# z430/keyword-spotting

Hardware: AMD Instinct MI355X
Metric: 1s 16kHz clips/sec end-to-end (wav->label) (higher is better)
Workload: dtype f32

## Files before the change

### include/kws_hip.h

```cpp
#ifndef KWS_HIP_H
#define KWS_HIP_H

#include <stddef.h>
#include <stdint.h>

#ifdef __cplusplus
extern "C" {
#endif

typedef struct kws_ctx kws_ctx;

enum {
    KWS_OK = 0,
    KWS_EINVAL = -1,
    KWS_ENOMEM = -2,
    KWS_EHIP = -3,
    KWS_ESTATE = -4,
    KWS_EUNSUPPORTED = -5
};

#define KWS_ABI_VERSION 1
int kws_abi_version(void);


int kws_create(kws_ctx** out, int device_id);
void kws_destroy(kws_ctx* ctx);

int kws_set_stream(kws_ctx* ctx, void* hip_stream, int external);

int kws_sync(kws_ctx* ctx);

const char* kws_last_error(kws_ctx* ctx);


int kws_set_frontend(kws_ctx* ctx, int sample_rate, int n_samples, int frame_len, int frame_step,
                     int nfft, int nfilt, int numcep, float preemph, int ceplifter);

#define KWS_FE_F32 0
#define KWS_FE_F64 1
int kws_set_frontend_math(kws_ctx* ctx, int math);
int kws_frontend_math(kws_ctx* ctx);

#define KWS_FE_REFINE_SPAN_DEFAULT 10.2f
int kws_set_frontend_refine(kws_ctx* ctx, float log_ratio);
int kws_frontend_stats(kws_ctx* ctx, uint64_t* frames_total, uint64_t* frames_refined, int* last_call_refined);

int kws_frontend_shape(kws_ctx* ctx, int* num_frames, int* numcep);

int kws_mfcc_i16(kws_ctx* ctx, const int16_t* d_wav, int B, float* d_out);

int kws_mfcc_f32(kws_ctx* ctx, const float* d_wav, int B, float* d_out);


int kws_load_dscnn(kws_ctx* ctx, const float* blob, size_t n_floats, int num_classes);
int kws_load_dscnn_ex(kws_ctx* ctx, const float* blob, size_t n_floats, int num_classes, int input_channels);
int kws_load_dscnn_device(kws_ctx* ctx, const float* d_blob, size_t n_floats, int num_classes, int input_channels);
int kws_dscnn_image_read(kws_ctx* ctx, uint32_t* out_words, size_t cap_words, size_t* need_words, float* scalars);

int kws_forward_f32(kws_ctx* ctx, const float* d_feat, int B, float* d_logits, int32_t* d_label);

int kws_forward_map_f32(kws_ctx* ctx, const float* d_feat, int B, int T, int F, float* d_logits, int32_t* d_label);
int kws_forward_map_debug_f32(kws_ctx* ctx, const float* d_feat, int B, int T, int F, float* d_logits, int32_t* d_label,
                              float* d_layers);


int kws_dscnn_backward_f32(kws_ctx* ctx, const float* d_feat, int B, int T, int F, const float* d_dlogits, float* d_grad);

int kws_cnn_trad_backward_f32(kws_ctx* ctx, const float* d_feat, int B, const float* d_dlogits, float* d_grad);

int kws_cnn_trad_train_debug_f32(kws_ctx* ctx, const float* d_feat, int B, float* d_conv1, int32_t* d_winner, float* d_conv2,
                                 float* d_hidden);

int kws_dsblock_forward_f32(kws_ctx* ctx, const float* d_x, int B, int C_in, int H, int W, const float* d_dw_w,
                            const float* d_dw_b, const float* d_pw_w, const float* d_pw_b, int C_out, int kernel_size,
                            int stride, int padding, float* d_out);

int kws_infer_i16(kws_ctx* ctx, const int16_t* d_wav, int B, float* d_logits, int32_t* d_label);

int kws_infer_f32(kws_ctx* ctx, const float* d_wav, int B, float* d_logits, int32_t* d_label);

int kws_infer_host_i16(kws_ctx* ctx, const int16_t* h_wav, int B, float* h_logits, int32_t* h_label);
int kws_infer_host_submit_i16(kws_ctx* ctx, const int16_t* h_wav, int B, float* h_logits, int32_t* h_label, uint64_t* ticket);
int kws_infer_host_wait(kws_ctx* ctx, uint64_t ticket);
int kws_ingest_config(kws_ctx* ctx, int chunk_clips, int n_slots, int pack_threads);

int kws_reserve(kws_ctx* ctx, int max_batch);

#define KWS_PW_F32 1
#define KWS_PW_SPLIT_BF16 4
#define KWS_PW_PAIR_F16 5
int kws_set_pointwise_math(kws_ctx* ctx, int math);

#define KWS_ACT_FLOATS_PER_CLIP (64 * (141 + 141 + 245 + 357) + 64 + 64 * 477)
int kws_forward_debug_f32(kws_ctx* ctx, const float* d_feat, int B, float* d_logits, int32_t* d_label,
                          float* d_act, int use_mfma);


int kws_stream_open(kws_ctx* ctx, int n_streams);
int kws_stream_close(kws_ctx* ctx);
int kws_stream_push_i16(kws_ctx* ctx, const int16_t* d_hop, float* d_logits, int32_t* d_label, int use_graph);
int kws_stream_cluster(kws_ctx* ctx, int workgroups_per_stream);
int kws_stream_host_results(kws_ctx* ctx, int enable);
int kws_stream_wait_host(kws_ctx* ctx, const float** h_logits, const int32_t** h_label);
int kws_stream_push_host_i16(kws_ctx* ctx, const int16_t* h_hop, const float** h_logits, const int32_t** h_label);
int kws_stream_state(kws_ctx* ctx, const float** d_feat_ring, int* hops);
int kws_stream_copy_features(kws_ctx* ctx, float* d_out);

int kws_stream_vad_f32(kws_ctx* ctx, float log_energy_threshold, int on_window, int off_window, int32_t* d_state);

int kws_load_cnn_trad(kws_ctx* ctx, const float* blob, size_t n_floats, int num_classes);
int kws_load_cnn_trad_device(kws_ctx* ctx, const float* d_blob, size_t n_floats, int num_classes);
int kws_forward_cnn_trad_f32(kws_ctx* ctx, const float* d_feat, int B, float* d_logits, int32_t* d_label);
#define KWS_CT_F16_PAIR 0
#define KWS_CT_BF16_TRIPLE 1
int kws_set_cnn_trad_math(kws_ctx* ctx, int math);
int kws_forward_cnn_trad_debug_f32(kws_ctx* ctx, const float* d_feat, int B, float* d_logits, int32_t* d_label, float* d_conv2,
                                   float* d_clip_scale);

int kws_infer_cnn_trad_i16(kws_ctx* ctx, const int16_t* d_wav, int B, float* d_logits, int32_t* d_label);


int kws_softmax_f32(kws_ctx* ctx, const float* d_logits, int B, int C, float* d_prob);

int kws_stream_smooth_f32(kws_ctx* ctx, const float* d_logits, int C, int window, float* d_smoothed, int32_t* d_label);


int kws_scan_i16(kws_ctx* ctx, const int16_t* d_pcm, int R, int n_total, int hop_frames, float* d_logits, int32_t* d_label,
                 float* d_feat_out);

int kws_scan_detect_f32(kws_ctx* ctx, const float* d_logits, int R, int W, int C, int smooth_window, int first_keyword,
                        float threshold, int refractory, float* d_smoothed, int32_t* d_event_window, int32_t* d_event_label,
                        float* d_event_score, int max_events, int32_t* d_event_count);


int kws_frames_i16(kws_ctx* ctx, const int16_t* d_pcm, int R, int n_total, float* d_feat_out);

int kws_segment_f32(kws_ctx* ctx, const float* d_feat, int R, int F_total, int n_total, float log_energy_threshold, int on_window,
                    int off_window, int pre_roll, int max_frames, int32_t* d_utt, int max_utts, int32_t* d_count);

int kws_cut_i16(kws_ctx* ctx, const int16_t* d_pcm, int R, int n_total, const int32_t* d_span, int U, int normalize_to,
                int16_t* d_clips, int n_out, int32_t* d_peak);


int kws_host_stream_utt_history(int frame_len, int frame_step, int pre_roll, int max_frames, int slack_hops, int* history_samples);

int kws_stream_utt_open(kws_ctx* ctx, float log_energy_threshold, int on_window, int off_window, int pre_roll, int max_frames,
                        int history_samples, int max_events);
int kws_stream_utt_close(kws_ctx* ctx);
int kws_stream_utt_step_i16(kws_ctx* ctx, const int16_t* d_hop, const float* d_energy);
int kws_stream_utt_flush(kws_ctx* ctx);
int kws_stream_utt_poll(kws_ctx* ctx, uint64_t* total_events, uint64_t* steps);
int kws_stream_utt_read(kws_ctx* ctx, uint64_t first_seq, int n, int64_t* out_records);
int kws_stream_utt_cut_i16(kws_ctx* ctx, uint64_t first_seq, int U, int normalize_to, int16_t* d_clips, int n_out, int32_t* d_peak);


int kws_resample_i16(kws_ctx* ctx, const int16_t* d_in, int R, int n_in, const int32_t* d_len, int rate_in, int rate_out,
                     int16_t* d_out, int n_out);
int kws_resample_f32(kws_ctx* ctx, const float* d_in, int R, int n_in, const int32_t* d_len, int rate_in, int rate_out,
                     float* d_out, int n_out);

int kws_host_stream_resample_plan(int rate_in, int rate_out, int* up, int* down, int* delay_out, int* history);
int kws_host_stream_resample_count(int rate_in, int rate_out, uint64_t samples_before, int n_in, int* n_out);
int kws_stream_resample_open(kws_ctx* ctx, int n_streams, int rate_in, int rate_out, int max_in, uint64_t first_sample);
int kws_stream_resample_close(kws_ctx* ctx);
int kws_stream_resample_i16(kws_ctx* ctx, const int16_t* d_in, int n_in, int16_t* d_out, int out_cap, int* n_out);
int kws_stream_push_rate_i16(kws_ctx* ctx, const int16_t* d_in, int n_in, float* d_logits, int32_t* d_label);
int kws_stream_push_host_rate_i16(kws_ctx* ctx, const int16_t* h_in, int n_in, const float** h_logits, const int32_t** h_label);


int kws_eval_open(kws_ctx* ctx, int num_classes, int n_bins);
int kws_eval_reset(kws_ctx* ctx);
int kws_eval_close(kws_ctx* ctx);

int kws_eval_update_f32(kws_ctx* ctx, const float* d_logits, const int32_t* d_truth, int B, float grad_scale, float* d_dlogits,
                        float* d_loss_rows);

int kws_eval_read(kws_ctx* ctx, uint64_t* counts, double* loss_sum, uint64_t* confusion, uint64_t* hist_pos, uint64_t* hist_neg);


int kws_augment_i16(kws_ctx* ctx, const int16_t* d_wav, int B, const int32_t* d_shift, const float* d_bg, int bg_len,
                    const int32_t* d_bg_off, const float* d_bg_vol, const uint8_t* d_silence, float* d_out);


#define KWS_SILENCE_INDEX 0

int kws_augment_draw(kws_ctx* ctx, uint64_t seed, uint32_t epoch, const int32_t* d_index, int B, const int32_t* d_label, int N,
                     int time_shift, const int32_t* d_bg_start, const int32_t* d_bg_len, int K, float bg_volume,
                     float bg_frequency, int use_background, int n_samples, int32_t* d_shift, int32_t* d_bg_off,
                     float* d_bg_vol, uint8_t* d_silence);

int kws_mfcc_augment_i16(kws_ctx* ctx, const int16_t* d_pcm, int N, const int32_t* d_index, int B, const int32_t* d_shift,
                         const float* d_bg, int bg_len, const int32_t* d_bg_off, const float* d_bg_vol,
                         const uint8_t* d_silence, float* d_out);

#define KWS_DSCNN_STAMPS 16
int kws_forward_stamps_f32(kws_ctx* ctx, const float* d_feat, int B, float* d_logits, uint64_t* d_stamps, int mode);


int kws_preemphasis_f32(kws_ctx* ctx, const float* d_signal, int n, float coeff, float* d_out);
int kws_framesig_f32(kws_ctx* ctx, const float* d_signal, int n, int frame_len, int frame_step,
                     const float* d_window, float* d_frames);
int kws_spec512_f32(kws_ctx* ctx, const float* d_frames, int num_frames, int frame_len, int power,
                    float* d_spec);

int kws_spec_f32(kws_ctx* ctx, const float* d_frames, int num_frames, int frame_len, int nfft, int power, float* d_spec);


enum { KWS_K_MFCC = 0, KWS_K_DSCNN = 1, KWS_K_CNNTRAD_CONV = 2, KWS_K_CNNTRAD_DENSE = 3, KWS_K_STREAM_FRAME = 4, KWS_K_MFCC_F64 = 5, KWS_K_MFCC_REFINE = 6,
       KWS_K_DSCNN_LOAD_STATS = 7, KWS_K_DSCNN_LOAD_PACK = 8, KWS_K_DSCNN_LOAD_FILL = 9,
       KWS_K_RESAMPLE = 10,
       KWS_K_COUNT = 11 };
int kws_prof_enable(kws_ctx* ctx, int on);
int kws_prof_reset(kws_ctx* ctx);
int kws_prof_read(kws_ctx* ctx, int kernel_id, double* total_ms, int* launches);
const char* kws_kernel_name(int kernel_id);


int kws_host_mel_edges(int nfilt, int nfft, int sample_rate, int* edges_out);
int kws_host_mel_dense(int nfilt, int nfft, int sample_rate, float* fb_out);
int kws_host_mel_layout(int nfilt, int nfft, int sample_rate, int* first_lane_out, int* n_lanes_out, int* lanes_used, int* row_safe);
int kws_host_dct_lifter(int nfilt, int numcep, int ceplifter, float* out);
int kws_host_dscnn_image(const float* blob, size_t n_floats, int num_classes, int input_channels, uint32_t* out_words,
                         size_t cap_words, size_t* need_words, float* scalars);
int kws_host_cnn_trad_image(const float* blob, size_t n_floats, int num_classes, uint32_t* out_words, size_t cap_words,
                            size_t* need_words, float* scalars);

int kws_host_scan_shape(int n_total, int frame_len, int frame_step, int window_frames, int hop_frames, int* frames_total,
                        int* n_windows);

int kws_host_resample_len(int n_in, int rate_in, int rate_out, int* n_out);
int kws_host_resample_design(int rate_in, int rate_out, int* up, int* down, int* half_len, int* outputs_per_workgroup,
                             double* taps, size_t cap, size_t* need);

#ifdef __cplusplus
}
#endif
#endif
```

### keyword-spotting_amd/csrc/kws_ctx.h

```cpp
#pragma once
#include <new>

#include "kws_endpoint_dev.h"
#include "kws_internal.h"

namespace kws {
struct Ingest;
void ingest_free(kws_ctx* c);
void smooth_free(kws_ctx* c);
void vad_free(kws_ctx* c);
void eval_free(kws_ctx* c);
struct ResampleCache;
void resample_free(kws_ctx* c);
struct StreamResample;
void stream_resample_free(kws_ctx* c);
struct StreamUtt;
void stream_utt_free(kws_ctx* c);
int stream_utt_push_check(kws_ctx* c, const char* fn);
int stream_utt_pushed(kws_ctx* c);
}

using kws::FrontendParams; using kws::FrontendTables; using kws::DscnnWeights; using kws::CnnTradWeights; using kws::NFFT;

struct kws_ctx {
    int device = 0;
    int n_cu = 0;
    hipStream_t own_stream = nullptr;
    hipStream_t stream = nullptr;
    hipEvent_t order_ev = nullptr;
    std::string err;

    int sample_rate = 16000, nfft = NFFT, ceplifter = 22;
    FrontendParams fp{};
    bool fe_ready = false;
    bool fe_fast_ok = false;
    int fe_math = KWS_FE_F32;
    void* d_fe = nullptr;
    FrontendTables ft{};
    double* d_spec_tw64 = nullptr;
    int spec_nfft = 0;
    float refine_span = KWS_FE_REFINE_SPAN_DEFAULT;
    int* d_refine = nullptr;
    int refine_cap = 0;
    unsigned long long frames_seen = 0;

    float* d_model = nullptr;
    DscnnWeights mw{};
    bool model_ready = false;
    size_t ds_image_words = 0;
    void* d_ds_stats = nullptr;
    int pw_math = KWS_PW_PAIR_F16;
    void* d_cnntrad = nullptr;
    CnnTradWeights tw{};
    bool cnntrad_ready = false;
    int cnntrad_math = KWS_CT_F16_PAIR;
    const float* ct_raw = nullptr;
    size_t ct_image_words = 0;
    float* d_ct_stats = nullptr;
    float* d_conv_ws = nullptr;
    size_t conv_ws_floats = 0;
    float* d_train_ws = nullptr;
    size_t train_ws_floats = 0;

    float* d_feat_ws = nullptr;
    size_t feat_ws_floats = 0;
    float* d_scan_ws = nullptr;
    size_t scan_ws_floats = 0;

    int n_streams = 0, ring_len = 0;
    int16_t* d_pcm_ring = nullptr;
    float* d_feat_ring = nullptr;
    int* d_hops = nullptr;
    int stream_cluster = 0;
    float* d_cl_part = nullptr;
    int* d_cl_count = nullptr;
    float* h_stream_logits = nullptr;
    int32_t* h_stream_label = nullptr;
    int* h_stream_flag = nullptr;
    int16_t* h_stream_hop = nullptr;
    float* d_hr_logits = nullptr;
    int32_t* d_hr_label = nullptr;
    int host_results_classes = 0;
    int pushes_enqueued = 0;
    int host_push = 0;
    bool last_push_host = false;
    hipGraphExec_t stream_graph = nullptr;
    const void* graph_key[3] = {nullptr, nullptr, nullptr};
    float* d_post_ring = nullptr;
    float* d_post_sum = nullptr;
    int* d_post_count = nullptr;
    int post_window = 0, post_classes = 0;
    unsigned long long* d_vad_bits = nullptr;
    int* d_vad_counts = nullptr;
    int vad_on = 0, vad_off = 0;

    unsigned long long* d_eval = nullptr;
    int eval_classes = 0, eval_bins = 0;
    double* d_eval_part = nullptr;
    size_t eval_part_cap = 0;

    kws::ResampleCache* resample = nullptr;
    kws::StreamResample* stream_resample = nullptr;
    kws::StreamUtt* stream_utt = nullptr;

    kws::Ingest* ingest = nullptr;

    bool prof = false;
    int prof_every = 1;
    unsigned prof_seen[KWS_K_COUNT] = {};
    struct EvPair {
        hipEvent_t a, b;
    };
    std::vector<EvPair> ev[KWS_K_COUNT];
    size_t ev_used[KWS_K_COUNT] = {};
    double ms_total[KWS_K_COUNT] = {};
    long launches[KWS_K_COUNT] = {};
};

int frames_for(int n_samples, int frame_len, int frame_step);
void set_clip_length(FrontendParams& p, int n_samples);
int ensure_refine(kws_ctx* c, int B, int num_frames);
void stream_free(kws_ctx* c);
template <typename Src>
int run_frontend(kws_ctx* c, const FrontendParams& geometry, Src src, int B, float* d_out, int refine_clips);

inline thread_local std::string g_create_err;

inline int fail(kws_ctx* c, int code, const std::string& msg) {
    if (c)
        c->err = msg;
    else
        g_create_err = msg;
    return code;
}
inline int fail_hip(kws_ctx* c, hipError_t e, const char* what) {
    return fail(c, KWS_EHIP, std::string(what) + ": " + hipGetErrorString(e));
}
inline int check_batch(kws_ctx* c, const void* in, int B, const char* fn) {
    if (!c) return KWS_EINVAL;
    if (!in) return fail(c, KWS_EINVAL, std::string(fn) + ": input pointer is NULL");
    if (B <= 0) return fail(c, KWS_EINVAL, std::string(fn) + ": B must be positive");
    return KWS_OK;
}
inline int check_endpoint_windows(kws_ctx* c, const char* fn, int on_window, int off_window) {
    const bool ok = on_window >= 1 && on_window <= off_window && off_window <= kws::EP_MAX_WINDOW;
    return ok ? KWS_OK : fail(c, KWS_EINVAL, std::string(fn) + ": need 1 <= on_window <= off_window <= 1024");
}
inline int check_append_energy(kws_ctx* c, const char* fn) {
    return c->fp.append_energy ? KWS_OK : fail(c, KWS_EUNSUPPORTED, std::string(fn) + ": needs cepstrum 0 = log frame energy (appendEnergy)");
}
inline int check_normalize_to(kws_ctx* c, const char* fn, int v) {
    return v >= 0 && v <= 32767 ? KWS_OK : fail(c, KWS_EINVAL, std::string(fn) + ": normalize_to must be in [0, 32767]");
}
#define KWS_GUARD_BEGIN try {
#define KWS_GUARD_END(c, fn)                                                          \
    }                                                                                 \
    catch (const std::bad_alloc&) { return fail(c, KWS_ENOMEM, fn ": out of host memory"); } \
    catch (...) { return fail(c, KWS_EHIP, fn ": unexpected C++ exception"); }
#define HIP_TRY(c, expr)                                   \
    do {                                                   \
        hipError_t _e = (expr);                            \
        if (_e != hipSuccess) return fail_hip(c, _e, #expr); \
    } while (0)

inline int alloc_endpoint_state(kws_ctx* c, const char* fn, size_t S, unsigned long long*& bits, int*& counts) {
    const size_t bits_b = sizeof(unsigned long long) * S * kws::EP_BIT_WORDS, counts_b = sizeof(int) * S * 4;
    if (hipMalloc(reinterpret_cast<void**>(&bits), bits_b) != hipSuccess || hipMalloc(reinterpret_cast<void**>(&counts), counts_b) != hipSuccess)
        return fail(c, KWS_ENOMEM, std::string(fn) + ": device allocation failed");
    hipError_t e = hipMemsetAsync(bits, 0, bits_b, c->stream);
    if (e == hipSuccess) e = hipMemsetAsync(counts, 0, counts_b, c->stream);
    return e == hipSuccess ? KWS_OK : fail_hip(c, e, (std::string(fn) + ": hipMemsetAsync").c_str());
}

struct ProfScope {
    kws_ctx* c;
    int id;
    hipEvent_t stop = nullptr;
    ProfScope(kws_ctx* c_, int id_) : c(c_), id(id_) {
        if (!c->prof) return;
        if (c->prof_seen[id]++ % (unsigned)c->prof_every != 0) return;
        if (c->ev_used[id] == c->ev[id].size()) {
            kws_ctx::EvPair p{};
            if (hipEventCreate(&p.a) != hipSuccess || hipEventCreate(&p.b) != hipSuccess) return;
            c->ev[id].push_back(p);
        }
        kws_ctx::EvPair& p = c->ev[id][c->ev_used[id]++];
        (void)hipEventRecord(p.a, c->stream);
        stop = p.b;
    }
    ~ProfScope() {
        if (stop) (void)hipEventRecord(stop, c->stream);
    }
};

inline void drop_stream_graph(kws_ctx* c) {
    if (c->stream_graph) (void)hipGraphExecDestroy(c->stream_graph);
    c->stream_graph = nullptr;
    c->graph_key[0] = c->graph_key[1] = c->graph_key[2] = nullptr;
}

template <class T>
int replace_device_image(kws_ctx* c, T*& slot, const void* host, size_t bytes, const char* fn) {
    HIP_TRY(c, hipStreamSynchronize(c->stream));
    void* d = nullptr;
    if (hipMalloc(&d, bytes) != hipSuccess) return fail(c, KWS_ENOMEM, std::string(fn) + ": device allocation failed");
    hipError_t e = hipMemcpy(d, host, bytes, hipMemcpyHostToDevice);
    if (e != hipSuccess) {
        (void)hipFree(d);
        return fail_hip(c, e, (std::string(fn) + ": hipMemcpy").c_str());
    }
    if (slot) (void)hipFree(slot);
    slot = static_cast<T*>(d);
    return KWS_OK;
}

template <class T>
int grow_device_buffer(kws_ctx* c, T*& buf, size_t& cap, size_t need, const char* fn, const char* what) {
    if (need <= cap) return KWS_OK;
    HIP_TRY(c, hipStreamSynchronize(c->stream));
    T* d = nullptr;
    if (hipMalloc(reinterpret_cast<void**>(&d), need * sizeof(T)) != hipSuccess)
        return fail(c, KWS_ENOMEM, std::string(fn) + ": " + what + " allocation failed");
    if (buf) (void)hipFree(buf);
    buf = d;
    cap = need;
    return KWS_OK;
}
```

### keyword-spotting_amd/csrc/kws_frontend.hip

```cpp
#include <type_traits>

#include "kws_ctx.h"
#include "kws_tables.h"

using namespace kws;

int frames_for(int n_samples, int frame_len, int frame_step) {
    if (n_samples <= frame_len) return 1;
    return 1 + (n_samples - frame_len + frame_step - 1) / frame_step;
}

void set_clip_length(FrontendParams& p, int n_samples) {
    p.n_samples = n_samples;
    p.num_frames = frames_for(n_samples, p.frame_len, p.frame_step);
    p.vec_ok = (n_samples % 8 == 0) && ((MFCC_FRAMES_PER_WG * p.frame_step) % 8 == 0);
}

int ensure_refine(kws_ctx* c, int B, int num_frames) {
    const size_t frames = (size_t)B * ((num_frames + 1) / 2);
    if (frames > 0x1fffffffu) return fail(c, KWS_EUNSUPPORTED, "refinement worklist: more than 2^29 frame pairs in one call");
    if (c->d_refine && (int)frames <= c->refine_cap) return KWS_OK;
    HIP_TRY(c, hipStreamSynchronize(c->stream));
    int* d = nullptr;
    if (hipMalloc(reinterpret_cast<void**>(&d), sizeof(int) * (8 + frames)) != hipSuccess)
        return fail(c, KWS_ENOMEM, "refinement worklist: device allocation failed");
    hipError_t e = c->d_refine ? hipMemcpy(d, c->d_refine, sizeof(int) * 8, hipMemcpyDeviceToDevice) : hipMemset(d, 0, sizeof(int) * 8);
    if (e != hipSuccess) {
        (void)hipFree(d);
        return fail_hip(c, e, "refinement worklist");
    }
    if (c->d_refine) (void)hipFree(c->d_refine);
    c->d_refine = d;
    c->refine_cap = (int)frames;
    return KWS_OK;
}

template <typename Src>
int run_frontend(kws_ctx* c, const FrontendParams& geometry, Src src, int B, float* d_out, int refine_clips) {
    HIP_TRY(c, hipSetDevice(c->device));
    FrontendParams p = geometry;
    if constexpr (std::is_same<Src, const int16_t*>::value)
        if ((reinterpret_cast<uintptr_t>(src) & 15) != 0) p.vec_ok = 0;
    if constexpr (std::is_pointer<Src>::value)
        if (c->fe_math == KWS_FE_F64 || !c->fe_fast_ok) {
            ProfScope ps(c, KWS_K_MFCC_F64);
            HIP_TRY(c, launch_mfcc_f64(c->stream, p, c->ft, src, B, d_out));
            return KWS_OK;
        }
    c->frames_seen += (unsigned long long)B * p.num_frames;
    if (p.refine_span > 0.f) {
        int rc = ensure_refine(c, B, p.num_frames);
        if (rc) return rc;
        const RefineList rl = {c->d_refine, c->d_refine + 8, c->refine_cap, 0};
        {
            ProfScope ps(c, KWS_K_MFCC);
            HIP_TRY(c, launch_mfcc(c->stream, p, c->ft, src, B, d_out, rl));
        }
        ProfScope ps(c, KWS_K_MFCC_REFINE);
        HIP_TRY(c, launch_mfcc_refine(c->stream, p, c->ft, src, d_out, rl, refine_clips));
        return KWS_OK;
    }
    ProfScope ps(c, KWS_K_MFCC);
    HIP_TRY(c, launch_mfcc(c->stream, p, c->ft, src, B, d_out, RefineList{}));
    return KWS_OK;
}
template int run_frontend(kws_ctx*, const FrontendParams&, const int16_t*, int, float*, int);
template int run_frontend(kws_ctx*, const FrontendParams&, const float*, int, float*, int);
template int run_frontend(kws_ctx*, const FrontendParams&, AugmentArgs, int, float*, int);

#pragma GCC visibility push(default)
extern "C" {

int kws_set_frontend(kws_ctx* c, int sample_rate, int n_samples, int frame_len, int frame_step, int nfft, int nfilt,
                     int numcep, float preemph, int ceplifter) {
    KWS_GUARD_BEGIN
    if (!c) return KWS_EINVAL;
    if (sample_rate <= 0 || n_samples <= 0 || frame_len <= 0 || frame_step <= 0 || nfilt <= 0 || numcep <= 0 || nfft < 2)
        return fail(c, KWS_EINVAL, "kws_set_frontend: sizes must be positive");
    if (nfilt > MAX_NFILT || numcep > MAX_NUMCEP || numcep > nfilt)
        return fail(c, KWS_EUNSUPPORTED, "kws_set_frontend: need nfilt <= 64 and numcep <= min(nfilt, 32)");
    int log2n = 0;
    if ((nfft & (nfft - 1)) == 0)
        for (int v = nfft; v > 1; v >>= 1) ++log2n;
    if (nfft > 4096 || (log2n == 0 && nfft > 2048) || (log2n > 0 && nfft < 64))
        return fail(c, KWS_EUNSUPPORTED, "kws_set_frontend: nfft must be a power of two in [64, 4096] or any value in [2, 2048]");
    FrontendImage im;
    if (!build_frontend_image(sample_rate, frame_len, nfft, nfilt, numcep, ceplifter, im))
        return fail(c, KWS_EUNSUPPORTED, "kws_set_frontend: mel edges are not monotone inside [0, nfft/2]");

    HIP_TRY(c, hipSetDevice(c->device));
    HIP_TRY(c, hipStreamSynchronize(c->stream));
    if (c->n_streams) stream_free(c);
    int rc = replace_device_image(c, c->d_fe, im.bytes.data(), im.bytes.size(), "kws_set_frontend");
    if (rc) return rc;
    c->ft = im.tables(c->d_fe);

    FrontendParams& p = c->fp;
    p.frame_len = frame_len;
    p.frame_step = frame_step;
    set_clip_length(p, n_samples);
    p.nfilt = nfilt;
    p.numcep = numcep;
    p.append_energy = 1;
    p.preemph = preemph;
    p.chunk_samples = (MFCC_FRAMES_PER_WG - 1) * frame_step + frame_len;
    p.nfft = nfft;
    p.log2_nfft = log2n;
    p.refine_span = c->refine_span;
    c->sample_rate = sample_rate;
    c->nfft = nfft;
    c->ceplifter = ceplifter;
    c->fe_fast_ok = im.fast && mfcc_tile_lds_bytes(p) <= MFCC_TILE_LDS_MAX;
    c->fe_ready = true;
    return KWS_OK;
    KWS_GUARD_END(c, "kws_set_frontend")
}

int kws_set_frontend_math(kws_ctx* c, int math) {
    if (!c) return KWS_EINVAL;
    if (math != KWS_FE_F32 && math != KWS_FE_F64) return fail(c, KWS_EINVAL, "kws_set_frontend_math: math must be KWS_FE_F32 or KWS_FE_F64");
    c->fe_math = math;
    return KWS_OK;
}

int kws_frontend_math(kws_ctx* c) {
    if (!c || !c->fe_ready) return KWS_EINVAL;
    return (c->fe_math == KWS_FE_F64 || !c->fe_fast_ok) ? KWS_FE_F64 : KWS_FE_F32;
}

int kws_set_frontend_refine(kws_ctx* c, float log_span) {
    if (!c) return KWS_EINVAL;
    if (!(log_span == log_span)) return fail(c, KWS_EINVAL, "kws_set_frontend_refine: log_span is NaN");
    c->refine_span = log_span > 0.f ? log_span : 0.f;
    c->fp.refine_span = c->refine_span;
    if (c->stream_graph) {
        HIP_TRY(c, hipStreamSynchronize(c->stream));
        drop_stream_graph(c);
    }
    return KWS_OK;
}

int kws_frontend_stats(kws_ctx* c, uint64_t* frames_total, uint64_t* frames_refined, int* last_call_refined) {
    if (!c) return KWS_EINVAL;
    int ctr[8] = {0, 0, 0, 0, 0, 0, 0, 0};
    HIP_TRY(c, hipSetDevice(c->device));
    HIP_TRY(c, hipStreamSynchronize(c->stream));
    if (c->d_refine) HIP_TRY(c, hipMemcpy(ctr, c->d_refine, sizeof ctr, hipMemcpyDeviceToHost));
    if (frames_total) *frames_total = c->frames_seen;
    if (frames_refined) *frames_refined = ((uint64_t)(uint32_t)ctr[3] << 32 | (uint32_t)ctr[2]) + (uint64_t)(uint32_t)ctr[5];
    if (last_call_refined) *last_call_refined = ctr[4];
    return KWS_OK;
}

int kws_frontend_shape(kws_ctx* c, int* num_frames, int* numcep) {
    if (!c) return KWS_EINVAL;
    if (!c->fe_ready) return fail(c, KWS_ESTATE, "front end not configured");
    if (num_frames) *num_frames = c->fp.num_frames;
    if (numcep) *numcep = c->fp.numcep;
    return KWS_OK;
}

int kws_reserve(kws_ctx* c, int max_batch) {
    if (!c) return KWS_EINVAL;
    if (max_batch <= 0) return fail(c, KWS_EINVAL, "kws_reserve: max_batch must be positive");
    if (!c->fe_ready) return fail(c, KWS_ESTATE, "front end not configured");
    if (c->refine_span > 0.f && c->fe_fast_ok) {
        int rc = ensure_refine(c, max_batch, c->fp.num_frames);
        if (rc) return rc;
    }
    const size_t need = (size_t)max_batch * c->fp.num_frames * c->fp.numcep;
    if (need <= c->feat_ws_floats) return KWS_OK;
    HIP_TRY(c, hipSetDevice(c->device));
    return grow_device_buffer(c, c->d_feat_ws, c->feat_ws_floats, need, "kws_reserve", "device");
}

int kws_mfcc_i16(kws_ctx* c, const int16_t* d_wav, int B, float* d_out) {
    int rc = check_batch(c, d_wav, B, "kws_mfcc_i16");
    if (rc) return rc;
    if (!d_out) return fail(c, KWS_EINVAL, "kws_mfcc_i16: d_out is NULL");
    if (!c->fe_ready) return fail(c, KWS_ESTATE, "kws_mfcc_i16: front end not configured");
    return run_frontend(c, c->fp, d_wav, B, d_out, B);
}

int kws_mfcc_f32(kws_ctx* c, const float* d_wav, int B, float* d_out) {
    int rc = check_batch(c, d_wav, B, "kws_mfcc_f32");
    if (rc) return rc;
    if (!d_out) return fail(c, KWS_EINVAL, "kws_mfcc_f32: d_out is NULL");
    if (!c->fe_ready) return fail(c, KWS_ESTATE, "kws_mfcc_f32: front end not configured");
    return run_frontend(c, c->fp, d_wav, B, d_out, B);
}

int kws_augment_i16(kws_ctx* c, const int16_t* d_wav, int B, const int32_t* d_shift, const float* d_bg, int bg_len,
                    const int32_t* d_bg_off, const float* d_bg_vol, const uint8_t* d_silence, float* d_out) {
    int rc = check_batch(c, d_wav, B, "kws_augment_i16");
    if (rc) return rc;
    if (!d_out) return fail(c, KWS_EINVAL, "kws_augment_i16: d_out is NULL");
    if (d_bg && (bg_len <= 0 || !d_bg_off || !d_bg_vol)) return fail(c, KWS_EINVAL, "kws_augment_i16: background pool needs length, offsets and volumes");
    if (!c->fe_ready) return fail(c, KWS_ESTATE, "kws_augment_i16: front end not configured");
    HIP_TRY(c, hipSetDevice(c->device));
    HIP_TRY(c, launch_augment(c->stream, d_wav, B, c->fp.n_samples, d_shift, d_bg, bg_len, d_bg_off, d_bg_vol, d_silence, d_out));
    return KWS_OK;
}

int kws_augment_draw(kws_ctx* c, uint64_t seed, uint32_t epoch, const int32_t* d_index, int B, const int32_t* d_label, int N,
                     int time_shift, const int32_t* d_bg_start, const int32_t* d_bg_len, int K, float bg_volume,
                     float bg_frequency, int use_background, int n_samples, int32_t* d_shift, int32_t* d_bg_off,
                     float* d_bg_vol, uint8_t* d_silence) {
    int rc = check_batch(c, d_index, B, "kws_augment_draw");
    if (rc) return rc;
    if (!d_shift || !d_bg_off || !d_bg_vol || !d_silence) return fail(c, KWS_EINVAL, "kws_augment_draw: an output pointer is NULL");
    if (K < 0 || (K > 0 && (!d_bg_start || !d_bg_len))) return fail(c, KWS_EINVAL, "kws_augment_draw: K files need their start and length tables");
    if (time_shift < 0 || time_shift > (1 << 30)) return fail(c, KWS_EINVAL, "kws_augment_draw: time_shift must be in [0, 2^30]");
    if (N < 0 || n_samples < 0) return fail(c, KWS_EINVAL, "kws_augment_draw: N and n_samples must not be negative");
    HIP_TRY(c, hipSetDevice(c->device));
    const kws::DrawArgs d = {seed, epoch, d_index, d_label, N, time_shift, d_bg_start, d_bg_len, K, bg_volume, bg_frequency,
                             use_background, n_samples, d_shift, d_bg_off, d_bg_vol, d_silence};
    HIP_TRY(c, kws::launch_augment_draw(c->stream, d, B));
    return KWS_OK;
}

int kws_mfcc_augment_i16(kws_ctx* c, const int16_t* d_pcm, int N, const int32_t* d_index, int B, const int32_t* d_shift,
                         const float* d_bg, int bg_len, const int32_t* d_bg_off, const float* d_bg_vol,
                         const uint8_t* d_silence, float* d_out) {
    int rc = check_batch(c, d_pcm, B, "kws_mfcc_augment_i16");
    if (rc) return rc;
    if (!d_index || !d_out) return fail(c, KWS_EINVAL, "kws_mfcc_augment_i16: d_index or d_out is NULL");
    if (N <= 0) return fail(c, KWS_EINVAL, "kws_mfcc_augment_i16: N must be positive");
    if (d_bg && (bg_len <= 0 || !d_bg_off || !d_bg_vol)) return fail(c, KWS_EINVAL, "kws_mfcc_augment_i16: background pool needs length, offsets and volumes");
    if (!c->fe_ready) return fail(c, KWS_ESTATE, "kws_mfcc_augment_i16: front end not configured");
    FrontendParams p = c->fp;
    if ((reinterpret_cast<uintptr_t>(d_pcm) & 15) != 0) p.vec_ok = 0;
    if (c->fe_math == KWS_FE_F64 || !c->fe_fast_ok || !kws::mfcc_wave_resident_ok(p))
        return fail(c, KWS_EUNSUPPORTED, "kws_mfcc_augment_i16: needs KWS_FE_F32 at a geometry of the wavefront-resident kernel and 16-byte "
                                         "aligned PCM; compose kws_augment_i16 and kws_mfcc_f32 instead");
    const kws::AugmentArgs a = {d_pcm, d_index, N, d_shift, d_bg, bg_len, d_bg_off, d_bg_vol, d_silence};
    return run_frontend(c, p, a, B, d_out, B);
}

int kws_preemphasis_f32(kws_ctx* c, const float* d_signal, int n, float coeff, float* d_out) {
    int rc = check_batch(c, d_signal, n, "kws_preemphasis_f32");
    if (rc) return rc;
    if (!d_out) return fail(c, KWS_EINVAL, "kws_preemphasis_f32: d_out is NULL");
    HIP_TRY(c, hipSetDevice(c->device));
    HIP_TRY(c, launch_preemphasis(c->stream, d_signal, n, coeff, d_out));
    return KWS_OK;
}

int kws_framesig_f32(kws_ctx* c, const float* d_signal, int n, int frame_len, int frame_step, const float* d_window,
                     float* d_frames) {
    int rc = check_batch(c, d_signal, n, "kws_framesig_f32");
    if (rc) return rc;
    if (!d_frames || frame_len <= 0 || frame_step <= 0) return fail(c, KWS_EINVAL, "kws_framesig_f32: bad argument");
    HIP_TRY(c, hipSetDevice(c->device));
    HIP_TRY(c, launch_framesig(c->stream, d_signal, n, frame_len, frame_step, frames_for(n, frame_len, frame_step), d_window, d_frames));
    return KWS_OK;
}

int kws_spec512_f32(kws_ctx* c, const float* d_frames, int num_frames, int frame_len, int power, float* d_spec) {
    int rc = check_batch(c, d_frames, num_frames, "kws_spec512_f32");
    if (rc) return rc;
    if (!d_spec || frame_len <= 0) return fail(c, KWS_EINVAL, "kws_spec512_f32: bad argument");
    if (!c->fe_ready) return fail(c, KWS_ESTATE, "kws_spec512_f32: front end tables not built");
    HIP_TRY(c, hipSetDevice(c->device));
    HIP_TRY(c, launch_spec512(c->stream, c->ft, d_frames, num_frames, frame_len, power, d_spec));
    return KWS_OK;
}

int kws_spec_f32(kws_ctx* c, const float* d_frames, int num_frames, int frame_len, int nfft, int power, float* d_spec) {
    KWS_GUARD_BEGIN
    int rc = check_batch(c, d_frames, num_frames, "kws_spec_f32");
    if (rc) return rc;
    if (!d_spec || frame_len <= 0 || nfft < 2) return fail(c, KWS_EINVAL, "kws_spec_f32: bad argument");
    if (nfft == NFFT) return kws_spec512_f32(c, d_frames, num_frames, frame_len, power, d_spec);
    int log2n = 0;
    if ((nfft & (nfft - 1)) == 0)
        for (int v = nfft; v > 1; v >>= 1) ++log2n;
    if (nfft > 4096 || (log2n == 0 && nfft > 2048) || (log2n > 0 && nfft < 64))
        return fail(c, KWS_EUNSUPPORTED, "kws_spec_f32: NFFT must be a power of two in [64, 4096] or any value in [2, 2048]");
    HIP_TRY(c, hipSetDevice(c->device));
    if (c->spec_nfft != nfft) {
        const std::vector<double> tw = build_twiddle64(nfft);
        rc = replace_device_image(c, c->d_spec_tw64, tw.data(), sizeof(double) * tw.size(), "kws_spec_f32");
        if (rc) return rc;
        c->spec_nfft = nfft;
    }
    HIP_TRY(c, launch_spec_f64(c->stream, c->d_spec_tw64, d_frames, num_frames, frame_len, nfft, log2n, power, d_spec));
    return KWS_OK;
    KWS_GUARD_END(c, "kws_spec_f32")
}

}
#pragma GCC visibility pop
```

### keyword-spotting_amd/csrc/kws_internal.h

```cpp
#pragma once
#include <hip/hip_runtime.h>
#include <stdint.h>

#include <string>
#include <vector>

#include "kws_hip.h"

namespace kws {

constexpr int NFFT = 512;
constexpr int NBINS = NFFT / 2 + 1;
constexpr int MEL_CHUNK = 8;
constexpr int MEL_STRIDE = 10;
#ifndef KWS_MFCC_WAVES
#define KWS_MFCC_WAVES 4
#endif
#ifndef KWS_MFCC_PAIRS_PER_WAVE
#define KWS_MFCC_PAIRS_PER_WAVE 3
#endif
constexpr int MFCC_WAVES = KWS_MFCC_WAVES;
constexpr int MFCC_THREADS = MFCC_WAVES * 64;
constexpr int MFCC_FRAMES_PER_WG = 2 * KWS_MFCC_PAIRS_PER_WAVE * MFCC_WAVES;
constexpr int MAX_NFILT = 64;
constexpr int MAX_NUMCEP = 32;

struct FrontendParams {
    int n_samples;
    int frame_len;
    int frame_step;
    int num_frames;
    int nfilt;
    int numcep;
    int append_energy;
    float preemph;
    int chunk_samples;
    int vec_ok;
    int nfft;
    int log2_nfft;
    float refine_span;
};
__host__ __device__ inline int frames_lag(int frame_len, int frame_step) { return (frame_len + frame_step - 1) / frame_step; }
__host__ __device__ inline int frames_lag(const FrontendParams& p) { return frames_lag(p.frame_len, p.frame_step); }

struct RefineList {
    int* ctr;
    int* list;
    int cap;
    int clip0;
};

struct FrontendTables {
    const float2* twiddle;
    const int* mel_k0;
    const float* mel_rw;
    const float* mel_fw;
    const uint32_t* mel_gather;
    const int* mel_slot;
    const int* mel_seg;
    const float* dct;
    const float* dct_pad;
    const double* tw64;
    const int* mel_edges;
    const double* mel_w64;
    const double* dct64;
};

template <typename K>
inline hipError_t raise_lds_limit(K kernel, size_t lds) {
    if (lds <= 64 * 1024) return hipSuccess;
    return hipFuncSetAttribute(reinterpret_cast<const void*>(kernel), hipFuncAttributeMaxDynamicSharedMemorySize, (int)lds);
}

struct AugmentArgs;
hipError_t launch_mfcc(hipStream_t s, const FrontendParams& p, const FrontendTables& t, const int16_t* d_wav, int B, float* d_out,
                       const RefineList& rl);
hipError_t launch_mfcc(hipStream_t s, const FrontendParams& p, const FrontendTables& t, const float* d_wav, int B, float* d_out,
                       const RefineList& rl);
hipError_t launch_mfcc(hipStream_t s, const FrontendParams& p, const FrontendTables& t, const AugmentArgs& a, int B, float* d_out,
                       const RefineList& rl);
hipError_t launch_mfcc_refine(hipStream_t s, const FrontendParams& p, const FrontendTables& t, const int16_t* d_wav, float* d_out,
                              const RefineList& rl, int B);
hipError_t launch_mfcc_refine(hipStream_t s, const FrontendParams& p, const FrontendTables& t, const float* d_wav, float* d_out,
                              const RefineList& rl, int B);
hipError_t launch_mfcc_refine(hipStream_t s, const FrontendParams& p, const FrontendTables& t, const AugmentArgs& a, float* d_out,
                              const RefineList& rl, int B);
hipError_t launch_mfcc_f64(hipStream_t s, const FrontendParams& p, const FrontendTables& t, const int16_t* d_wav, int B, float* d_out);
hipError_t launch_mfcc_f64(hipStream_t s, const FrontendParams& p, const FrontendTables& t, const float* d_wav, int B, float* d_out);
hipError_t launch_spec_f64(hipStream_t s, const double* d_tw64, const float* d_frames, int num_frames, int frame_len, int nfft,
                           int log2n, int power, float* d_spec);
hipError_t launch_stream_frame(hipStream_t s, const FrontendParams& p, const FrontendTables& t, const int16_t* d_hop,
                               int n_streams, int16_t* d_pcm_ring, int ring_len, float* d_feat_ring, int* d_hops, int* d_refine_ctr);
hipError_t launch_augment(hipStream_t s, const int16_t* d_wav, int B, int n, const int32_t* d_shift, const float* d_bg,
                          int bg_len, const int32_t* d_bg_off, const float* d_bg_vol, const uint8_t* d_silence,
                          float* d_out);
struct AugmentArgs {
    const int16_t* pcm;
    const int32_t* index;
    int n_rows;
    const int32_t* shift;
    const float* bg;
    int bg_len;
    const int32_t* bg_off;
    const float* bg_vol;
    const uint8_t* silence;
};
struct DrawArgs {
    unsigned long long seed;
    unsigned epoch;
    const int32_t* index;
    const int32_t* label;
    int n_rows, time_shift;
    const int32_t* bg_start;
    const int32_t* bg_len;
    int n_files;
    float bg_volume, bg_frequency;
    int use_background, n_samples;
    int32_t* shift;
    int32_t* bg_off;
    float* bg_vol;
    uint8_t* silence;
};
hipError_t launch_augment_draw(hipStream_t s, const DrawArgs& d, int B);
bool mfcc_wave_resident_ok(const FrontendParams& p);
size_t mfcc_tile_lds_bytes(const FrontendParams& p);
constexpr size_t MFCC_TILE_LDS_MAX = 160 * 1024;
hipError_t launch_preemphasis(hipStream_t s, const float* d_in, int n, float coeff, float* d_out);
hipError_t launch_framesig(hipStream_t s, const float* d_in, int n, int frame_len, int frame_step,
                           int num_frames, const float* d_window, float* d_frames);
hipError_t launch_spec512(hipStream_t s, const FrontendTables& t, const float* d_frames, int num_frames,
                          int frame_len, int power, float* d_spec);

constexpr int CH = 64;
constexpr int IN_T = 99, IN_F = 10;
constexpr int C1_K = 10, C1_H = 47, C1_W = 3;
constexpr int N_BLOCKS = 4;
constexpr int MAX_CLASSES = 64;

struct DscnnWeights {
    const float* c1_w;
    const float* c1_b;
    const float* dw_w;
    const float* pw_w;
    const float* pw_b;
    const uint32_t* pw_split;
    const uint32_t* c1_split;
    const float* fc_w;
    const float* fc_b;
    int num_classes;
    int in_channels;
    const float* c1_general;
    const float* raw;
    const uint32_t* pw_pair;
    const uint32_t* c1_pair;
    int k_c1, k_pw[4];
    float c1_abs, c1_bmax, dw_abs[4], dw_bmax[4], pw_abs[4], pw_bmax[4];
};

hipError_t dscnn_init_device();
struct ScanWindows {
    unsigned wpr;
    unsigned wpr_recip;
    unsigned row_floats;
    unsigned win_floats;
};
struct StreamPush {
    union {
        FrontendParams p;
        ScanWindows scan;
    };
    FrontendTables t;
    const int16_t* hop;
    int16_t* pcm_ring;
    int ring_len;
    int* hops;
    int* refine_ctr;
    int frames_lag;
    int cluster;
    float* cl_part;
    int* cl_count;
    float* h_logits;
    int32_t* h_label;
    int* h_flag;
};
hipError_t launch_dscnn_stream(hipStream_t s, const DscnnWeights& w, const StreamPush& sp, float* d_feat_ring, int n_streams,
                               float* d_logits, int32_t* d_label, bool pair);
hipError_t launch_dscnn(hipStream_t s, const DscnnWeights& w, const float* d_feat, int B, float* d_logits,
                        int32_t* d_label, float* d_act, int mode, unsigned long long* d_stamps = nullptr,
                        const int* d_ring_hops = nullptr, bool preconv = false, int frames_lag = 3, int n_cu = 0);
hipError_t launch_dscnn_scan(hipStream_t s, const DscnnWeights& w, const float* d_feat, int B, float* d_logits, int32_t* d_label,
                             int mode, int n_cu, const ScanWindows& sw);
hipError_t launch_conv1_general(hipStream_t s, const float* d_x, int B, int C_in, const float* d_wt, const float* d_bias, float* d_out);

struct CnnTradWeights {
    const uint32_t* c1_split;
    const float* c1_b;
    const uint32_t* c2_split;
    const float* c2_b;
    const uint32_t* lin_split;
    const float* lin_b;
    const float* dnn_w;
    const float* dnn_b;
    const float* fc_w;
    const float* fc_b;
    int num_classes;
    const uint32_t* c1_h2;
    const uint32_t* c2_h2;
    const uint32_t* lin_h2;
    float inv_sw1, inv_sw2, inv_swl;
    float w1_abs, b1_max;
    float w2_abs, b2_max;
};
hipError_t cnntrad_init_device();
hipError_t launch_cnntrad_conv(hipStream_t s, const CnnTradWeights& w, const float* d_feat, int B, float* d_conv_ws, bool f16_pair);
hipError_t launch_cnntrad_dense(hipStream_t s, const CnnTradWeights& w, const float* d_conv_ws, int B, float* d_logits,
                                int32_t* d_label, bool f16_pair);

hipError_t launch_dsblock(hipStream_t s, const float* d_x, int B, int C_in, int H, int W, const float* d_dw_w, const float* d_dw_b,
                          const float* d_pw_w, const float* d_pw_b, int C_out, int k, int stride, int pad, float* d_ws,
                          float* d_out);

hipError_t launch_conv1_any(hipStream_t s, const float* d_x, int B, int C_in, int T, int F, const float* d_wt, const float* d_bias,
                            float* d_out);
hipError_t launch_pool_fc(hipStream_t s, const float* d_x, int B, int HW, const float* d_fc_w, const float* d_fc_b, int C,
                          float* d_logits, int32_t* d_label);
struct DscnnMap {
    int H1, W1;
    DscnnMap(int T, int F) : H1((T - 6) / 2 + 1), W1((F - 6) / 2 + 1) {}
    int H(int k) const { return H1 + 2 * k; }
    int W(int k) const { return W1 + 2 * k; }
    size_t P(int k) const { return (size_t)H(k) * W(k); }
    size_t Q(int k) const { return P(k + 1); }
};
int check_dscnn_map(kws_ctx* c, const char* fn, int T, int F);
struct DscnnStages {
    float* a0;
    float* dw[N_BLOCKS];
    float* y[N_BLOCKS];
};
hipError_t launch_dscnn_composed(hipStream_t s, const DscnnWeights& w, const float* d_feat, int nb, int T, int F, const DscnnStages& st);
constexpr int COMPOSED_MAX_CLIPS = 16384;

hipError_t launch_softmax(hipStream_t s, const float* d_logits, int B, int C, float* d_prob);
hipError_t launch_smooth_posteriors(hipStream_t s, const float* d_logits, int S, int C, int window, float* d_ring,
                                    float* d_sum, int* d_count, float* d_smoothed, int32_t* d_label);
hipError_t launch_scan_detect(hipStream_t s, const float* d_logits, int R, int W, int C, int smooth_window, int first_keyword,
                              float threshold, int refractory, float* d_smoothed, int32_t* d_cand, float* d_score,
                              int32_t* d_event_window, int32_t* d_event_label, float* d_event_score, int max_events,
                              int32_t* d_event_count);

extern const char* const kKernelNames[KWS_K_COUNT];

}
```

### keyword-spotting_amd/csrc/kws_mfcc.hip

```cpp
#include <cstdlib>

#include "kws_augment_dev.h"
#include "kws_internal.h"
#include "kws_mfcc_dev.h"

namespace kws {
namespace {

template <typename T, bool TAIL6>
__device__ __forceinline__ void mfcc_body(const FrontendParams& p, const FrontendTables& t, const T* __restrict__ wav,
                                          float* __restrict__ out, const RefineList& rl) {
    extern __shared__ __attribute__((aligned(16))) unsigned char smem[];
    const int nfp = (p.nfilt + 3) & ~3;
    float* dctb = reinterpret_cast<float*>(smem);
    cf* tw2 = reinterpret_cast<cf*>(dctb + ((p.numcep * nfp + 3) & ~3));
    float* ybuf = reinterpret_cast<float*>(tw2 + 64);
    unsigned char* scr0 = reinterpret_cast<unsigned char*>(ybuf + ((p.chunk_samples + 7) & ~7));

    const int tid = threadIdx.x, lane = tid & 63, wv = tid >> 6;
    const int clip = blockIdx.y;
    const int f0 = blockIdx.x * MFCC_FRAMES_PER_WG;
    const T* __restrict__ x = wav + (size_t)clip * p.n_samples;

    const int s0 = f0 * p.frame_step;
    const float c = p.preemph;
    const int my_frames = min(MFCC_FRAMES_PER_WG, p.num_frames - f0);
    const int my_samples = (my_frames - 1) * p.frame_step + p.frame_len;
    for (int g = tid; g * 8 < my_samples; g += MFCC_THREADS) {
        const int n = s0 + g * 8;
        float y[8];
        if (sizeof(T) == 2 && p.vec_ok && n + 8 <= p.n_samples) {
            const uint4 raw = *reinterpret_cast<const uint4*>(x + n);
            float prev = (n > 0) ? to_unit(x[n - 1]) : 0.f;
            const uint32_t wd[4] = {raw.x, raw.y, raw.z, raw.w};
#pragma unroll
            for (int i = 0; i < 8; ++i) {
                const int16_t s = (int16_t)((wd[i >> 1] >> (16 * (i & 1))) & 0xffffu);
                const float cur = to_unit(s);
                y[i] = (n + i > 0) ? __fsub_rn(cur, __fmul_rn(c, prev)) : cur;
                prev = cur;
            }
        } else {
#pragma unroll
            for (int i = 0; i < 8; ++i) {
                const int m = n + i;
                float v = 0.f;
                if (m < p.n_samples) {
                    const float cur = to_unit(x[m]);
                    v = (m > 0) ? __fsub_rn(cur, __fmul_rn(c, to_unit(x[m - 1]))) : cur;
                }
                y[i] = v;
            }
        }
        float4* dst = reinterpret_cast<float4*>(ybuf + g * 8);
        dst[0] = make_float4(y[0], y[1], y[2], y[3]);
        dst[1] = make_float4(y[4], y[5], y[6], y[7]);
    }
    for (int i = tid; i < (p.numcep * nfp + 3) / 4; i += MFCC_THREADS)
        reinterpret_cast<float4*>(dctb)[i] = reinterpret_cast<const float4*>(t.dct_pad)[i];
    fill_tw2(t.twiddle, tw2, tid);

    cf t1[8];
    load_twiddles(t.twiddle, lane, t1);
    MelLane ml;
    load_mel_lane(t, lane, ml);
    unsigned char* scr = scr0 + wv * SCR_BYTES;
    zero_scratch(scr, lane);
    __syncthreads();

    const PairScratch sc = {reinterpret_cast<cf*>(scr + SCR_XBUF), reinterpret_cast<float2*>(scr + SCR_PBUF),
                            reinterpret_cast<float*>(scr + SCR_LBUF),
                            dctb, tw2, nfp};

    for (int pr = wv; pr < MFCC_FRAMES_PER_WG / 2; pr += MFCC_WAVES) {
        const int fa = f0 + 2 * pr;
        if (fa >= p.num_frames) break;
        const bool has_b = (fa + 1) < p.num_frames;
        const float* ya = ybuf + (2 * pr) * p.frame_step;
        const float* yb = ya + p.frame_step;

        cf v[8];
        uint32_t ora = 0u, orb = 0u;
        if constexpr (TAIL6) {
#pragma unroll
            for (int n1 = 0; n1 < 7; ++n1) {
                const int i = 64 * n1 + lane;
                float a = ya[i], b = yb[i];
                if (n1 == 6) {
                    const bool in = i < p.frame_len;
                    a = in ? a : 0.f, b = in ? b : 0.f;
                }
                v[n1] = cf{a, b};
                ora |= __builtin_bit_cast(uint32_t, a);
                orb |= __builtin_bit_cast(uint32_t, b);
            }
            v[7] = cf{0.f, 0.f};
            if (!has_b) {
#pragma unroll
                for (int n1 = 0; n1 < 7; ++n1) v[n1].y = 0.f;
                orb = 0u;
            }
        } else {
#pragma unroll
            for (int n1 = 0; n1 < 8; ++n1) {
                const int i = 64 * n1 + lane;
                const bool in = i < p.frame_len;
                const float la = ya[i], lb = yb[i];
                const float a = in ? la : 0.f, b = (in && has_b) ? lb : 0.f;
                v[n1] = cf{a, b};
                ora |= __builtin_bit_cast(uint32_t, a);
                orb |= __builtin_bit_cast(uint32_t, b);
            }
        }
        const bool nza = __any((ora << 1) != 0u);
        const bool nzb = __any((orb << 1) != 0u);
        const uint32_t flags = mfcc_pair(v, nza, nzb, has_b, p, sc, t1, ml, lane,
                                         out + ((size_t)clip * p.num_frames + fa) * p.numcep,
                                         out + ((size_t)clip * p.num_frames + fa + 1) * p.numcep);
        if (flags && rl.ctr && lane == 0) {
            const unsigned long long old = atomicAdd(reinterpret_cast<unsigned long long*>(rl.ctr), 1ull | ((unsigned long long)__builtin_popcount(flags) << 32));
            const int at = (int)(unsigned)old;
            if (at < rl.cap) rl.list[at] = (int)((((unsigned)(rl.clip0 + clip) * (unsigned)((p.num_frames + 1) / 2) + (unsigned)(fa >> 1)) << 2) | flags);
        }
        wave_lds_order();
    }
}

#ifndef KWS_MFCC_EU
#define KWS_MFCC_EU 4
#endif
__global__ __launch_bounds__(MFCC_THREADS) __attribute__((amdgpu_waves_per_eu(KWS_MFCC_EU, KWS_MFCC_EU))) void kws_mfcc_i16_tile_kernel(FrontendParams p, FrontendTables t,
                                                                    const int16_t* __restrict__ wav,
                                                                    float* __restrict__ out, RefineList rl) {
    mfcc_body<int16_t, true>(p, t, wav, out, rl);
}
__global__ __launch_bounds__(MFCC_THREADS) __attribute__((amdgpu_waves_per_eu(KWS_MFCC_EU, KWS_MFCC_EU))) void kws_mfcc_f32_kernel(FrontendParams p, FrontendTables t,
                                                                    const float* __restrict__ wav,
                                                                    float* __restrict__ out, RefineList rl) {
    mfcc_body<float, true>(p, t, wav, out, rl);
}
__global__ __launch_bounds__(MFCC_THREADS) __attribute__((amdgpu_waves_per_eu(KWS_MFCC_EU, KWS_MFCC_EU))) void kws_mfcc_i16_any_kernel(FrontendParams p, FrontendTables t,
                                                                    const int16_t* __restrict__ wav,
                                                                    float* __restrict__ out, RefineList rl) {
    mfcc_body<int16_t, false>(p, t, wav, out, rl);
}
__global__ __launch_bounds__(MFCC_THREADS) __attribute__((amdgpu_waves_per_eu(KWS_MFCC_EU, KWS_MFCC_EU))) void kws_mfcc_f32_any_kernel(FrontendParams p, FrontendTables t,
                                                                    const float* __restrict__ wav,
                                                                    float* __restrict__ out, RefineList rl) {
    mfcc_body<float, false>(p, t, wav, out, rl);
}

constexpr int WR_PAIRS = 2, WR_FRAMES = 2 * WR_PAIRS;
constexpr int WR_SPAN = 1024;
constexpr int WR_WAVE_BYTES = WR_SPAN * 4 + SCR_BYTES;

typedef float float4_a4 __attribute__((ext_vector_type(4), aligned(4)));
__device__ __forceinline__ void aug_vec8(const AugClip& c, int n0, int n, float (&a)[8]) {
    if (n0 + 8 > n) {
#pragma unroll
        for (int i = 0; i < 8; ++i) a[i] = 0.f;
        return;
    }
    const int r = uniform_i(-c.shift & 7);
    const int base = n0 - c.shift - r;
    uint4 lo = make_uint4(0, 0, 0, 0), hi = lo;
    if (!c.silence) {
        if (base >= 0 && base + 8 <= n) lo = *reinterpret_cast<const uint4*>(c.x + base);
        if (base + 8 >= 0 && base + 16 <= n) hi = *reinterpret_cast<const uint4*>(c.x + base + 8);
    }
    const uint32_t w[8] = {lo.x, lo.y, lo.z, lo.w, hi.x, hi.y, hi.z, hi.w};
    const uint32_t m2 = (r & 4) ? ~0u : 0u, m1 = (r & 2) ? ~0u : 0u;
    uint32_t u[6], v[5];
#pragma unroll
    for (int k = 0; k < 6; ++k) u[k] = (w[k + 2] & m2) | (w[k] & ~m2);
#pragma unroll
    for (int k = 0; k < 5; ++k) v[k] = (u[k + 1] & m1) | (u[k] & ~m1);
#pragma unroll
    for (int k = 0; k < 4; ++k) {
        const uint32_t wd = (r & 1) ? __builtin_amdgcn_alignbyte(v[k + 1], v[k], 2) : v[k];
        a[2 * k] = pcm_unit((int16_t)(wd & 0xffffu));
        a[2 * k + 1] = pcm_unit((int16_t)(wd >> 16));
    }
    if (c.bg) {
        const int k0 = c.off + n0;
        float g[8];
        if (k0 >= 0 && k0 + 8 <= c.bg_len) {
            const float4_a4 g0 = *reinterpret_cast<const float4_a4*>(c.bg + k0);
            const float4_a4 g1 = *reinterpret_cast<const float4_a4*>(c.bg + k0 + 4);
            g[0] = g0.x, g[1] = g0.y, g[2] = g0.z, g[3] = g0.w, g[4] = g1.x, g[5] = g1.y, g[6] = g1.z, g[7] = g1.w;
        } else {
#pragma unroll
            for (int i = 0; i < 8; ++i) {
                const int k = c.off + n0 + i;
                g[i] = (k >= 0 && k < c.bg_len) ? c.bg[k] : 0.f;
            }
        }
#pragma unroll
        for (int i = 0; i < 8; ++i) a[i] = __fadd_rn(a[i], __fmul_rn(g[i], c.vol));
    }
}

__host__ __device__ inline size_t mfcc_wr_lds_bytes(const FrontendParams& p) {
    const int nfp = (p.nfilt + 3) & ~3;
    return sizeof(float) * (size_t)(((p.numcep * nfp + 3) & ~3) + 2 * 64) + (size_t)MFCC_WAVES * WR_WAVE_BYTES;
}

template <bool AUG>
__device__ __forceinline__ void mfcc_wr_body(FrontendParams p, FrontendTables t, const int16_t* __restrict__ wav,
                                             float* __restrict__ out, RefineList rl, int B, int chunks_per_wave,
                                             AugmentArgs aug) {
    extern __shared__ __attribute__((aligned(16))) unsigned char smem[];
    const int nfp = (p.nfilt + 3) & ~3;
    float* dctb = reinterpret_cast<float*>(smem);
    cf* tw2 = reinterpret_cast<cf*>(dctb + ((p.numcep * nfp + 3) & ~3));
    const int tid = threadIdx.x, lane = tid & 63, wv = tid >> 6;
    unsigned char* mine = reinterpret_cast<unsigned char*>(tw2 + 64) + wv * WR_WAVE_BYTES;
    float* ybuf = reinterpret_cast<float*>(mine);
    unsigned char* scr = mine + WR_SPAN * 4;

    for (int i = tid; i < (p.numcep * nfp + 3) / 4; i += MFCC_THREADS)
        reinterpret_cast<float4*>(dctb)[i] = reinterpret_cast<const float4*>(t.dct_pad)[i];
    fill_tw2(t.twiddle, tw2, tid);
    cf t1[8];
    load_twiddles(t.twiddle, lane, t1);
    MelLane ml;
    load_mel_lane(t, lane, ml);
    zero_scratch(scr, lane);

    const int n_chunks = (p.num_frames + WR_FRAMES - 1) / WR_FRAMES;
    const int waves_per_clip = (n_chunks + chunks_per_wave - 1) / chunks_per_wave;
    const int gw = blockIdx.x * MFCC_WAVES + wv;
    const int clip = gw / waves_per_clip, part = gw - clip * waves_per_clip;
    int c = part * chunks_per_wave;
    const int c_end = min(n_chunks, c + chunks_per_wave);
    const bool active = clip < B && c < c_end;
    const int16_t* __restrict__ x = AUG ? nullptr : wav + (size_t)(active ? clip : 0) * p.n_samples;
    AugClip ac{};
    if constexpr (AUG) ac = aug_clip(aug, active ? clip : 0, p.n_samples);
    const int chunk_step = WR_FRAMES * p.frame_step;

    uint4 v0 = make_uint4(0, 0, 0, 0), v1 = v0;
    int16_t before = 0;
    auto fetch = [&](int cc) {
        const int s0 = cc * chunk_step;
        const int n0 = s0 + 8 * lane, n1 = n0 + 512;
        v0 = n0 + 8 <= p.n_samples ? *reinterpret_cast<const uint4*>(x + n0) : make_uint4(0, 0, 0, 0);
        v1 = n1 + 8 <= p.n_samples ? *reinterpret_cast<const uint4*>(x + n1) : make_uint4(0, 0, 0, 0);
        before = s0 > 0 ? x[s0 - 1] : (int16_t)0;
    };
    __syncthreads();
    if (!active) return;

    const PairScratch sc = {reinterpret_cast<cf*>(scr + SCR_XBUF), reinterpret_cast<float2*>(scr + SCR_PBUF),
                            reinterpret_cast<float*>(scr + SCR_LBUF), dctb, tw2, nfp};
    const float pre = p.preemph;
    uint32_t fmask = 0u;
    int pair0 = 2 * c;
#define KWS_FLUSH_FLAGS()                                                                                                          \
    if (fmask && rl.ctr) {                                                                                                          \
        const int lane = (int)__builtin_amdgcn_mbcnt_hi(~0u, __builtin_amdgcn_mbcnt_lo(~0u, 0u));  \
        const uint32_t fk = lane < 16 ? (fmask >> (2 * lane)) & 3u : 0u;                                                            \
        const uint32_t has = (uint32_t)__ballot(fk != 0u);                                                                          \
        unsigned long long old = 0ull;                                                                                              \
        if (lane == 0)                                                                                                              \
            old = atomicAdd(reinterpret_cast<unsigned long long*>(rl.ctr),                                                          \
                            (unsigned long long)__builtin_popcount(has) | ((unsigned long long)__builtin_popcount(fmask) << 32));   \
        const int at = __builtin_amdgcn_readfirstlane((int)(unsigned)old) + __builtin_popcount(has & ((1u << (lane & 31)) - 1u));   \
        if (fk != 0u && at < rl.cap)                                                                                                \
            rl.list[at] = (int)((((unsigned)(rl.clip0 + clip) * (unsigned)((p.num_frames + 1) / 2) + (unsigned)(pair0 + lane)) << 2) | fk); \
    }
    for (; c < c_end; ++c) {
        if constexpr (!AUG) fetch(c);
        if constexpr (AUG) {
            const int s0 = c * chunk_step;
            float a0[8], a1[8];
            aug_vec8(ac, s0 + 8 * lane, p.n_samples, a0);
            aug_vec8(ac, s0 + 512 + 8 * lane, p.n_samples, a1);
            const float w0 = __int_as_float(__builtin_amdgcn_update_dpp(0, __float_as_int(a0[7]), 0x138, 0xf, 0xf, false));
            const float w1 = __int_as_float(__builtin_amdgcn_update_dpp(0, __float_as_int(a1[7]), 0x138, 0xf, 0xf, false));
            const float last0 = __int_as_float(__builtin_amdgcn_readlane(__float_as_int(a0[7]), 63));
            const float before_a = s0 > 0 ? aug_sample(ac, s0 - 1, p.n_samples) : 0.f;
            auto emphasise = [&](const float (&a)[8], float prev, int n, float* dst) {
                float y[8];
#pragma unroll
                for (int i = 0; i < 8; ++i) {
                    y[i] = __fsub_rn(a[i], __fmul_rn(pre, prev));
                    prev = a[i];
                }
                if (n == 0) y[0] = a[0];
                if (n + 8 > p.n_samples) {
#pragma unroll
                    for (int i = 0; i < 8; ++i) y[i] = 0.f;
                }
                reinterpret_cast<float4*>(dst)[0] = make_float4(y[0], y[1], y[2], y[3]);
                reinterpret_cast<float4*>(dst)[1] = make_float4(y[4], y[5], y[6], y[7]);
            };
            emphasise(a0, lane == 0 ? before_a : w0, s0 + 8 * lane, ybuf + 8 * lane);
            emphasise(a1, lane == 0 ? last0 : w1, s0 + 512 + 8 * lane, ybuf + 512 + 8 * lane);
        } else {
            const int s0 = c * chunk_step;
            const uint32_t w0 = (uint32_t)__builtin_amdgcn_update_dpp(0, (int)v0.w, 0x138, 0xf, 0xf, false);
            const uint32_t w1 = (uint32_t)__builtin_amdgcn_update_dpp(0, (int)v1.w, 0x138, 0xf, 0xf, false);
            const uint32_t last0 = (uint32_t)__builtin_amdgcn_readlane((int)v0.w, 63);
            float prev0 = lane == 0 ? to_unit(before) : to_unit((int16_t)(w0 >> 16));
            float prev1 = lane == 0 ? to_unit((int16_t)(last0 >> 16)) : to_unit((int16_t)(w1 >> 16));
            auto convert = [&](const uint4& raw, float prev, int n, float* dst) {
                const uint32_t wd[4] = {raw.x, raw.y, raw.z, raw.w};
                float y[8];
#pragma unroll
                for (int i = 0; i < 8; ++i) {
                    const float cur = to_unit((int16_t)((wd[i >> 1] >> (16 * (i & 1))) & 0xffffu));
                    y[i] = __fsub_rn(cur, __fmul_rn(pre, prev));
                    prev = cur;
                }
                if (n == 0) y[0] = to_unit((int16_t)(wd[0] & 0xffffu));
                if (n + 8 > p.n_samples) {
#pragma unroll
                    for (int i = 0; i < 8; ++i) y[i] = 0.f;
                }
                reinterpret_cast<float4*>(dst)[0] = make_float4(y[0], y[1], y[2], y[3]);
                reinterpret_cast<float4*>(dst)[1] = make_float4(y[4], y[5], y[6], y[7]);
            };
            convert(v0, prev0, s0 + 8 * lane, ybuf + 8 * lane);
            convert(v1, prev1, s0 + 512 + 8 * lane, ybuf + 512 + 8 * lane);
        }
        wave_lds_order();
#pragma unroll 1
        for (int pr = 0; pr < WR_PAIRS; ++pr) {
            const int fa = WR_FRAMES * c + 2 * pr;
            if (fa >= p.num_frames) break;
            const bool has_b = fa + 1 < p.num_frames;
            const float* ya = ybuf + (2 * pr) * p.frame_step;
            const float* yb = ya + p.frame_step;
            cf v[8];
            uint32_t ora = 0u, orb = 0u;
#pragma unroll
            for (int n1 = 0; n1 < 7; ++n1) {
                const int i = 64 * n1 + lane;
                float a = ya[i], b = yb[i];
                if (n1 == 6) {
                    const bool in = i < p.frame_len;
                    a = in ? a : 0.f, b = in ? b : 0.f;
                }
                v[n1] = cf{a, b};
                ora |= __builtin_bit_cast(uint32_t, a);
                orb |= __builtin_bit_cast(uint32_t, b);
            }
            v[7] = cf{0.f, 0.f};
            if (!has_b) {
#pragma unroll
                for (int n1 = 0; n1 < 7; ++n1) v[n1].y = 0.f;
                orb = 0u;
            }
            const bool nza = __any((ora << 1) != 0u);
            const bool nzb = __any((orb << 1) != 0u);
            const uint32_t flags = mfcc_pair(v, nza, nzb, has_b, p, sc, t1, ml, lane,
                                             out + ((size_t)clip * p.num_frames + fa) * p.numcep,
                                             out + ((size_t)clip * p.num_frames + fa + 1) * p.numcep);
            fmask |= flags << (2 * ((fa >> 1) - pair0));
            wave_lds_order();
        }
        if (2 * (c + 1) - pair0 >= 16) {
            KWS_FLUSH_FLAGS()
            fmask = 0u;
            pair0 = 2 * (c + 1);
        }
    }
    KWS_FLUSH_FLAGS()
#undef KWS_FLUSH_FLAGS
}

__global__ __launch_bounds__(MFCC_THREADS) __attribute__((amdgpu_waves_per_eu(KWS_MFCC_EU, KWS_MFCC_EU))) void kws_mfcc_i16_kernel(
    FrontendParams p, FrontendTables t, const int16_t* __restrict__ wav, float* __restrict__ out, RefineList rl, int B, int chunks_per_wave) {
    mfcc_wr_body<false>(p, t, wav, out, rl, B, chunks_per_wave, AugmentArgs{});
}
#ifndef KWS_MFCC_AUG_EU
#define KWS_MFCC_AUG_EU 4
#endif
__global__ __launch_bounds__(MFCC_THREADS) __attribute__((amdgpu_waves_per_eu(KWS_MFCC_AUG_EU, KWS_MFCC_AUG_EU))) void kws_mfcc_augment_i16_kernel(
    FrontendParams p, FrontendTables t, AugmentArgs aug, float* __restrict__ out, RefineList rl, int B, int chunks_per_wave) {
    mfcc_wr_body<true>(p, t, nullptr, out, rl, B, chunks_per_wave, aug);
}

__global__ __launch_bounds__(64) void kws_spec512_f32_kernel(FrontendTables t, const float* __restrict__ frames,
                                                             int num_frames, int frame_len, int power,
                                                             float* __restrict__ spec) {
    __shared__ __attribute__((aligned(16))) unsigned char smem[SCR_BYTES + 512];
    cf* xbuf = reinterpret_cast<cf*>(smem + SCR_XBUF);
    float2* pbuf = reinterpret_cast<float2*>(smem + SCR_PBUF);
    cf* tw2 = reinterpret_cast<cf*>(smem + SCR_BYTES);
    const int lane = threadIdx.x;
    const int fa = 2 * blockIdx.x;
    const bool has_b = fa + 1 < num_frames;
    cf t1[8];
    load_twiddles(t.twiddle, lane, t1);
    fill_tw2(t.twiddle, tw2, lane);
    wave_lds_order();
    const float* ya = frames + (size_t)fa * frame_len;
    const float* yb = ya + frame_len;
    cf v[8];
    bool nza = false, nzb = false;
#pragma unroll
    for (int n1 = 0; n1 < 8; ++n1) {
        const int i = 64 * n1 + lane;
        const bool in = i < frame_len;
        v[n1].x = in ? ya[i] : 0.f;
        v[n1].y = (in && has_b) ? yb[i] : 0.f;
        nza |= v[n1].x != 0.f;
        nzb |= v[n1].y != 0.f;
    }
    nza = __any(nza);
    nzb = __any(nzb);
    const PairLevel lv = equalise_levels(v);
    fft512(v, xbuf, t1, tw2, lane);
    float ea, eb;
    const int ident[4] = {lane, lane + 64, lane + 128, lane + 192};
    split_power(v, xbuf, pbuf, lane, power, nza, nzb, ident, 256, lv, ea, eb);
    for (int k = lane; k < NBINS; k += 64) {
        const float2 pw = pbuf[k];
        spec[(size_t)fa * NBINS + k] = pw.x;
        if (has_b) spec[(size_t)(fa + 1) * NBINS + k] = pw.y;
    }
}

__global__ __launch_bounds__(64) void kws_stream_frame_kernel(FrontendParams p, FrontendTables t,
                                                              const int16_t* __restrict__ hop, int n_streams,
                                                              int16_t* __restrict__ pcm_ring, int ring_len,
                                                              float* __restrict__ feat_ring,
                                                              int* __restrict__ hops_ptr, int* refine_ctr) {
    extern __shared__ __attribute__((aligned(16))) unsigned char smem[];
    const int lane = threadIdx.x;
    const int sa = 2 * blockIdx.x, sb = sa + 1;
    const int hops = *hops_ptr;
    stream_frame_wave(p, t, hop, sa, sb, sb < n_streams, pcm_ring, ring_len, feat_ring, hops, smem, lane, nullptr, refine_ctr);
    if (lane == 0) {
        if (atomicAdd(&hops_ptr[1], 1) == (int)gridDim.x - 1) {
            hops_ptr[1] = 0;
            hops_ptr[0] = hops + 1;
        }
    }
}

}

size_t mfcc_tile_lds_bytes(const FrontendParams& p) {
    const int nfp = (p.nfilt + 3) & ~3;
    return sizeof(float) * (size_t)(((p.numcep * nfp + 3) & ~3) + 2 * 64 + ((p.chunk_samples + 7) & ~7)) +
           (size_t)MFCC_WAVES * SCR_BYTES;
}

template <typename T, typename K>
static hipError_t launch_mfcc_t(K kernel, hipStream_t s, const FrontendParams& p, const FrontendTables& t, const T* d_wav,
                                int B, float* d_out, RefineList rl) {
    dim3 grid((p.num_frames + MFCC_FRAMES_PER_WG - 1) / MFCC_FRAMES_PER_WG, B);
    const size_t lds = mfcc_tile_lds_bytes(p);
    hipError_t e = raise_lds_limit(kernel, lds);
    if (e != hipSuccess) return e;
    for (int b0 = 0; b0 < B; b0 += 65535) {
        const int nb = (B - b0 < 65535) ? (B - b0) : 65535;
        grid.y = nb;
        rl.clip0 = b0;
        hipLaunchKernelGGL(kernel, grid, dim3(MFCC_THREADS), lds, s, p, t, d_wav + (size_t)b0 * p.n_samples,
                           d_out + (size_t)b0 * p.num_frames * p.numcep, rl);
    }
    return hipGetLastError();
}

static bool mfcc_tail6(const FrontendParams& p) { return p.frame_len > 384 && p.frame_len <= 448; }

bool mfcc_wave_resident_ok(const FrontendParams& p) {
    return mfcc_tail6(p) && p.vec_ok && (WR_FRAMES * p.frame_step) % 8 == 0 && (WR_FRAMES - 1) * p.frame_step + 448 <= WR_SPAN;
}

static int mfcc_wr_chunks_per_wave(int nb, int n_chunks) {
    int wpc = (n_chunks + 2) / 5;
    wpc = wpc < 1 ? 1 : wpc;
    int cpw = (n_chunks + wpc - 1) / wpc;
    const int fill = (int)(((long)nb * n_chunks + 4095) / 4096);
    cpw = cpw > fill ? (fill < 1 ? 1 : fill) : cpw;
    static const int cpw_env = [] {
        const char* e = getenv("KWS_X_MFCC_CPW");
        return e ? atoi(e) : 0;
    }();
    if (cpw_env > 0) cpw = cpw_env > 16 ? 16 : cpw_env;
    return cpw;
}

static const int16_t* clips_from(const int16_t* d_wav, int b0, const FrontendParams& p) { return d_wav + (size_t)b0 * p.n_samples; }
static AugmentArgs clips_from(AugmentArgs a, int b0, const FrontendParams&) {
    a.index += b0;
    if (a.shift) a.shift += b0;
    if (a.bg_off) a.bg_off += b0;
    if (a.bg_vol) a.bg_vol += b0;
    if (a.silence) a.silence += b0;
    return a;
}

template <typename K, typename Src>
static hipError_t launch_mfcc_wr(K kernel, hipStream_t s, const FrontendParams& p, const FrontendTables& t, const Src& src, int B,
                                 float* d_out, RefineList rl) {
    const size_t lds = mfcc_wr_lds_bytes(p);
    const int n_chunks = (p.num_frames + WR_FRAMES - 1) / WR_FRAMES;
    for (int b0 = 0; b0 < B; b0 += (1 << 20)) {
        const int nb = B - b0 < (1 << 20) ? B - b0 : (1 << 20);
        const int cpw = mfcc_wr_chunks_per_wave(nb, n_chunks);
        const int waves_per_clip = (n_chunks + cpw - 1) / cpw;
        const long waves = (long)nb * waves_per_clip;
        rl.clip0 = b0;
        hipLaunchKernelGGL(kernel, dim3((unsigned)((waves + MFCC_WAVES - 1) / MFCC_WAVES)), dim3(MFCC_THREADS), lds, s, p, t,
                           clips_from(src, b0, p), d_out + (size_t)b0 * p.num_frames * p.numcep, rl, nb, cpw);
    }
    return hipGetLastError();
}

hipError_t launch_mfcc(hipStream_t s, const FrontendParams& p, const FrontendTables& t, const int16_t* d_wav, int B, float* d_out,
                       const RefineList& rl) {
#ifndef KWS_X_MFCC_TILE_KERNEL
    if (mfcc_wave_resident_ok(p)) return launch_mfcc_wr(kws_mfcc_i16_kernel, s, p, t, d_wav, B, d_out, rl);
#endif
    return launch_mfcc_t(mfcc_tail6(p) ? kws_mfcc_i16_tile_kernel : kws_mfcc_i16_any_kernel, s, p, t, d_wav, B, d_out, rl);
}
hipError_t launch_mfcc(hipStream_t s, const FrontendParams& p, const FrontendTables& t, const float* d_wav, int B, float* d_out,
                       const RefineList& rl) {
    return launch_mfcc_t(mfcc_tail6(p) ? kws_mfcc_f32_kernel : kws_mfcc_f32_any_kernel, s, p, t, d_wav, B, d_out, rl);
}
hipError_t launch_mfcc(hipStream_t s, const FrontendParams& p, const FrontendTables& t, const AugmentArgs& a, int B, float* d_out,
                       const RefineList& rl) {
    if (!mfcc_wave_resident_ok(p)) return hipErrorInvalidValue;
    return launch_mfcc_wr(kws_mfcc_augment_i16_kernel, s, p, t, a, B, d_out, rl);
}

hipError_t launch_stream_frame(hipStream_t s, const FrontendParams& p, const FrontendTables& t, const int16_t* d_hop,
                               int n_streams, int16_t* d_pcm_ring, int ring_len, float* d_feat_ring, int* d_hops, int* d_refine_ctr) {
    const size_t lds = stream_frame_lds_bytes(p);
    hipLaunchKernelGGL(kws_stream_frame_kernel, dim3((n_streams + 1) / 2), dim3(64), lds, s, p, t, d_hop, n_streams,
                       d_pcm_ring, ring_len, d_feat_ring, d_hops, d_refine_ctr);
    return hipGetLastError();
}

hipError_t launch_spec512(hipStream_t s, const FrontendTables& t, const float* d_frames, int num_frames, int frame_len,
                          int power, float* d_spec) {
    hipLaunchKernelGGL(kws_spec512_f32_kernel, dim3((num_frames + 1) / 2), dim3(64), 0, s, t, d_frames, num_frames,
                       frame_len, power, d_spec);
    return hipGetLastError();
}

}
```

### keyword-spotting_amd/csrc/kws_mfcc_dev.h

```cpp
#pragma once
#include "kws_internal.h"
#include "kws_mfcc_f64_dev.h"

namespace kws {
namespace {

typedef float cf __attribute__((ext_vector_type(2)));

__device__ __forceinline__ cf cadd(cf a, cf b) { return a + b; }
__device__ __forceinline__ cf csub(cf a, cf b) { return a - b; }
__device__ __forceinline__ cf cmul(cf a, cf b) {
    cf t, r;
    asm("v_pk_mul_f32 %0, %1, %2 op_sel:[1,1] op_sel_hi:[1,0] neg_lo:[0,1]" : "=v"(t) : "v"(a), "v"(b));
    asm("v_pk_fma_f32 %0, %1, %2, %3 op_sel_hi:[0,1,1]" : "=v"(r) : "v"(a), "v"(b), "v"(t));
    return r;
}
__device__ __forceinline__ cf add_mi(cf a, cf b) {
    cf r;
    asm("v_pk_add_f32 %0, %1, %2 op_sel:[0,1] op_sel_hi:[1,0] neg_hi:[0,1]" : "=v"(r) : "v"(a), "v"(b));
    return r;
}
__device__ __forceinline__ cf sub_mi(cf a, cf b) {
    cf r;
    asm("v_pk_add_f32 %0, %1, %2 op_sel:[0,1] op_sel_hi:[1,0] neg_lo:[0,1]" : "=v"(r) : "v"(a), "v"(b));
    return r;
}

__device__ __forceinline__ void dft8(cf (&v)[8]) {
    constexpr float R = 0.70710678118654752440f;
    const cf b0 = cadd(v[0], v[4]), b4 = csub(v[0], v[4]);
    const cf b1 = cadd(v[1], v[5]), c5 = csub(v[1], v[5]);
    const cf b2 = cadd(v[2], v[6]), b6 = csub(v[2], v[6]);
    const cf b3 = cadd(v[3], v[7]), c7 = csub(v[3], v[7]);
    const cf b5 = add_mi(c5, c5) * R;
    const cf b7 = sub_mi(c7, c7) * -R;
    const cf d0 = cadd(b0, b2), d1 = csub(b0, b2), d2 = cadd(b1, b3), d3 = csub(b1, b3);
    v[0] = cadd(d0, d2);
    v[4] = csub(d0, d2);
    v[2] = add_mi(d1, d3);
    v[6] = sub_mi(d1, d3);
    const cf e0 = add_mi(b4, b6), e1 = sub_mi(b4, b6), e2 = cadd(b5, b7), e3 = csub(b5, b7);
    v[1] = cadd(e0, e2);
    v[5] = csub(e0, e2);
    v[3] = add_mi(e1, e3);
    v[7] = sub_mi(e1, e3);
}

constexpr int XROW = 72;

constexpr int SCR_XBUF = 0, SCR_PBUF = 0, SCR_LBUF = 4608, SCR_BYTES = 4608 + 512;
static_assert(64 * MEL_STRIDE * 8 <= SCR_BYTES, "the power buffer (64 chunks of MEL_STRIDE float2) may run over the log-mel vectors, which are written after its last read, but not out of the wavefront's scratch");
static_assert(KWS_MFCC_WAVES * SCR_BYTES >= NFFT * 4, "frame loads may run up to NFFT floats past the staged span, into the scratch");

typedef float floatx2 __attribute__((ext_vector_type(2)));
__device__ __forceinline__ uint32_t lds_addr(const void* p) {
    return (uint32_t)(uintptr_t)(__attribute__((address_space(3))) const void*)p;
}

__device__ __forceinline__ void wave_lds_order() {
    __builtin_amdgcn_fence(__ATOMIC_ACQ_REL, "wavefront");
    __builtin_amdgcn_wave_barrier();
}

__device__ __forceinline__ int zswz(int k) { return k ^ ((k >> 3) & 7); }

__device__ __forceinline__ void fft512(cf (&v)[8], cf* xbuf, const cf (&t1)[8], const cf* tw2, int lane) {
    const int k1 = lane >> 3, q = lane & 7;
    dft8(v);
#pragma unroll
    for (int i = 1; i < 8; ++i) v[i] = cmul(v[i], t1[i]);
#ifdef KWS_MFCC_XCHG_PERMLANE
    {
        uint32_t r[8][2];
#pragma unroll
        for (int i = 0; i < 8; ++i) {
            r[i][0] = __builtin_bit_cast(uint32_t, (float)v[i].x);
            r[i][1] = __builtin_bit_cast(uint32_t, (float)v[i].y);
        }
#pragma unroll
        for (int i = 0; i < 4; ++i)
#pragma unroll
            for (int h = 0; h < 2; ++h) asm volatile("v_permlane32_swap_b32 %0, %1" : "+v"(r[i][h]), "+v"(r[i + 4][h]));
#pragma unroll
        for (int i = 0; i < 8; ++i)
            if (!(i & 2))
#pragma unroll
                for (int h = 0; h < 2; ++h) asm volatile("v_permlane16_swap_b32 %0, %1" : "+v"(r[i][h]), "+v"(r[i + 2][h]));
        const bool up = (lane & 8) != 0;
#pragma unroll
        for (int i = 0; i < 8; i += 2)
#pragma unroll
            for (int h = 0; h < 2; ++h) {
                const uint32_t send = up ? r[i][h] : r[i + 1][h];
                const uint32_t got = (uint32_t)__builtin_amdgcn_update_dpp(0, (int)send, 0x128 , 0xf, 0xf, false);
                r[i][h] = up ? got : r[i][h];
                r[i + 1][h] = up ? r[i + 1][h] : got;
            }
#pragma unroll
        for (int i = 0; i < 8; ++i) v[i] = cf{__builtin_bit_cast(float, r[i][0]), __builtin_bit_cast(float, r[i][1])};
    }
#else
#pragma unroll
    for (int i = 0; i < 8; ++i) xbuf[i * XROW + lane] = v[i];
    wave_lds_order();
    {
        floatx2 r0, r1, r2, r3, r4, r5, r6, r7;
        asm volatile(
            "ds_read_b64 %0, %8\n\t"
            "ds_read_b64 %1, %8 offset:64\n\t"
            "ds_read_b64 %2, %8 offset:128\n\t"
            "ds_read_b64 %3, %8 offset:192\n\t"
            "ds_read_b64 %4, %8 offset:256\n\t"
            "ds_read_b64 %5, %8 offset:320\n\t"
            "ds_read_b64 %6, %8 offset:384\n\t"
            "ds_read_b64 %7, %8 offset:448\n\t"
            "s_waitcnt lgkmcnt(0)"
            : "=&v"(r0), "=&v"(r1), "=&v"(r2), "=&v"(r3), "=&v"(r4), "=&v"(r5), "=&v"(r6), "=&v"(r7)
            : "v"(lds_addr(xbuf + k1 * XROW + q))
            : "memory");
        v[0] = {r0.x, r0.y}; v[1] = {r1.x, r1.y}; v[2] = {r2.x, r2.y}; v[3] = {r3.x, r3.y};
        v[4] = {r4.x, r4.y}; v[5] = {r5.x, r5.y}; v[6] = {r6.x, r6.y}; v[7] = {r7.x, r7.y};
    }
    wave_lds_order();
#endif
    dft8(v);
#pragma unroll
    for (int i = 1; i < 8; ++i) v[i] = cmul(v[i], tw2[i * 8 + q]);
    const int sw = k1 & 3;
#pragma unroll
    for (int c = 0; c < 8; ++c) xbuf[k1 * XROW + 8 * c + (q ^ (2 * sw))] = v[c];
    wave_lds_order();
    {
        const float4* row4 = reinterpret_cast<const float4*>(xbuf + k1 * XROW + 8 * q);
#pragma unroll
        for (int pr = 0; pr < 4; ++pr) {
            const float4 f = row4[pr ^ sw];
            v[2 * pr] = {f.x, f.y};
            v[2 * pr + 1] = {f.z, f.w};
        }
    }
    wave_lds_order();
    dft8(v);
}

template <int CTRL, int ROW_MASK>
__device__ __forceinline__ float dpp_shift_add(float v) {
    const float o = __builtin_bit_cast(float, __builtin_amdgcn_update_dpp(0, __builtin_bit_cast(int, v), CTRL, ROW_MASK, 0xf, true));
    return v + o;
}
__device__ __forceinline__ float wave_sum(float v) {
    v = dpp_shift_add<0x111, 0xf>(v);
    v = dpp_shift_add<0x112, 0xf>(v);
    v = dpp_shift_add<0x114, 0xf>(v);
    v = dpp_shift_add<0x118, 0xf>(v);
    v = dpp_shift_add<0x142, 0xa>(v);
    v = dpp_shift_add<0x143, 0xc>(v);
    return __builtin_bit_cast(float, __builtin_amdgcn_readlane(__builtin_bit_cast(int, v), 63));
}

__device__ __forceinline__ void wave_sum2(float& a, float& b) {
#define KWS_DPP_STEP(ctrl)                                                      \
    "v_add_f32_dpp %0, %0, %0 " ctrl "\n\t"                                      \
    "v_add_f32_dpp %1, %1, %1 " ctrl "\n\t"                                      \
    "s_nop 0\n\t"
    asm("s_nop 1\n\t"
        KWS_DPP_STEP("row_shr:1 row_mask:0xf bank_mask:0xf bound_ctrl:1")
        KWS_DPP_STEP("row_shr:2 row_mask:0xf bank_mask:0xf bound_ctrl:1")
        KWS_DPP_STEP("row_shr:4 row_mask:0xf bank_mask:0xf bound_ctrl:1")
        KWS_DPP_STEP("row_shr:8 row_mask:0xf bank_mask:0xf bound_ctrl:1")
        KWS_DPP_STEP("row_bcast:15 row_mask:0xa bank_mask:0xf")
        KWS_DPP_STEP("row_bcast:31 row_mask:0xc bank_mask:0xf")
        : "+v"(a), "+v"(b));
#undef KWS_DPP_STEP
    a = __builtin_bit_cast(float, __builtin_amdgcn_readlane(__builtin_bit_cast(int, a), 63));
    b = __builtin_bit_cast(float, __builtin_amdgcn_readlane(__builtin_bit_cast(int, b), 63));
}


struct PairLevel {
    float pow_a, pow_b;
};
__device__ __forceinline__ PairLevel equalise_levels(cf (&v)[8]) {
    cf e2 = {0.f, 0.f};
#pragma unroll
    for (int i = 0; i < 8; ++i) asm("v_pk_fma_f32 %0, %1, %1, %0" : "+v"(e2) : "v"(v[i]));
    float ea = e2.x, eb = e2.y;
    wave_sum2(ea, eb);
    auto shift_of = [](float e) -> int {
        const int ex = (int)((__builtin_bit_cast(uint32_t, e) >> 23) & 0xffu);
        if (ex == 0 || ex == 255) return 0;
        const int s = (ex - 127) >> 1;
        return s < -30 ? -30 : (s > 30 ? 30 : s);
    };
    const int sa = shift_of(ea), sb = shift_of(eb);
    if (sa == sb) return {1.0f, 1.0f};
    const cf down = {__builtin_bit_cast(float, (uint32_t)(127 - sa) << 23), __builtin_bit_cast(float, (uint32_t)(127 - sb) << 23)};
#pragma unroll
    for (int i = 0; i < 8; ++i) v[i] = v[i] * down;
    return {__builtin_bit_cast(float, (uint32_t)(127 + 2 * sa) << 23), __builtin_bit_cast(float, (uint32_t)(127 + 2 * sb) << 23)};
}

__device__ __forceinline__ void load_twiddles(const float2* __restrict__ tw, int lane, cf (&t1)[8]) {
#pragma unroll
    for (int i = 0; i < 8; ++i) {
        const float2 a = tw[(lane * i) & 511];
        t1[i] = {a.x, a.y};
    }
}
__device__ __forceinline__ void fill_tw2(const float2* __restrict__ tw, cf* tw2, int idx) {
    if (idx < 64) {
        const float2 a = tw[(8 * (idx >> 3) * (idx & 7)) & 511];
        tw2[idx] = {a.x, a.y};
    }
}

__device__ __forceinline__ void split_power(const cf (&v)[8], cf* zbuf, float2* pbuf, int lane, int power, bool nza,
                                            bool nzb, const int (&pslot)[4], int slot256, const PairLevel& lv, float& ea,
                                            float& eb, float* pk_a = nullptr, float* pk_b = nullptr) {
    const int k1 = lane >> 3, q = lane & 7;
#pragma unroll
    for (int d = 0; d < 8; ++d) zbuf[zswz(k1 + 8 * q + 64 * d)] = v[d];
    wave_lds_order();
    cf z[4], w[4];
#pragma unroll
    for (int j = 0; j < 4; ++j) {
        const int k = lane + 64 * j;
        z[j] = zbuf[zswz(k)];
        w[j] = zbuf[zswz((NFFT - k) & (NFFT - 1))];
    }
    wave_lds_order();
    const float scale = power ? (1.0f / (4.0f * NFFT)) : 0.25f;
    const float scale_a = scale * lv.pow_a, scale_b = scale * lv.pow_b;
    float pa[4], pb[4];
#pragma unroll
    for (int j = 0; j < 4; ++j) {
        const float ar = z[j].x + w[j].x, ai = z[j].y - w[j].y;
        const float br = z[j].y + w[j].y, bi = z[j].x - w[j].x;
        pa[j] = fmaf(ar, ar, ai * ai) * scale_a;
        pb[j] = fmaf(br, br, bi * bi) * scale_b;
        if (!power) {
            pa[j] = sqrtf(pa[j]);
            pb[j] = sqrtf(pb[j]);
        }
    }
    if (!(nza && nzb)) {
        asm volatile("" ::: "memory");
#pragma unroll
        for (int j = 0; j < 4; ++j) {
            pa[j] = nza ? pa[j] : 0.f;
            pb[j] = nzb ? pb[j] : 0.f;
        }
    }
    if (pk_a) {
        asm("v_max3_f32 %0, %1, %2, %3" : "=v"(*pk_a) : "v"(pa[0]), "v"(pa[1]), "v"(pa[2]));
        asm("v_max3_f32 %0, %1, %2, %3" : "=v"(*pk_b) : "v"(pb[0]), "v"(pb[1]), "v"(pb[2]));
        asm("v_max_f32 %0, %0, %1" : "+v"(*pk_a) : "v"(pa[3]));
        asm("v_max_f32 %0, %0, %1" : "+v"(*pk_b) : "v"(pb[3]));
    }
    ea = 0.f;
    eb = 0.f;
#pragma unroll
    for (int j = 0; j < 4; ++j) {
        pbuf[pslot[j]] = make_float2(pa[j], pb[j]);
        ea += pa[j];
        eb += pb[j];
    }
    if (lane == 0) {
        float pa = (2.f * v[4].x) * (2.f * v[4].x) * scale_a, pb = (2.f * v[4].y) * (2.f * v[4].y) * scale_b;
        if (!power) {
            pa = sqrtf(pa);
            pb = sqrtf(pb);
        }
        pa = nza ? pa : 0.f;
        pb = nzb ? pb : 0.f;
        if (slot256 >= 0) pbuf[slot256] = make_float2(pa, pb);
        ea += pa;
        eb += pb;
        if (pk_a) {
            asm("v_max_f32 %0, %0, %1" : "+v"(*pk_a) : "v"(pa));
            asm("v_max_f32 %0, %0, %1" : "+v"(*pk_b) : "v"(pb));
        }
    }
    wave_lds_order();
}

constexpr float PSF_EPS = 2.220446049250313e-16f;

__device__ __forceinline__ float to_unit(int16_t s) { return (float)s * (1.0f / 32768.0f); }
__device__ __forceinline__ float to_unit(float s) { return s; }

struct PairScratch {
    cf* xbuf;
    float2* pbuf;
    float* lbuf;
    const float* dctb;
    const cf* tw2;
    int nfp;
};

struct MelLane {
    float rw[MEL_CHUNK], fw[MEL_CHUNK];
    int pslot[4];
    uint32_t gth;
    float m1, m2, m4;
    bool deep;
};
__device__ __forceinline__ void load_mel_lane(const FrontendTables& t, int lane, MelLane& m) {
#pragma unroll
    for (int i = 0; i < MEL_CHUNK; ++i) {
        m.rw[i] = t.mel_rw[i * 64 + lane];
        m.fw[i] = t.mel_fw[i * 64 + lane];
    }
#pragma unroll
    for (int j = 0; j < 4; ++j) m.pslot[j] = t.mel_slot[lane + 64 * j];
    m.gth = t.mel_gather[lane];
    const int seg = t.mel_seg[lane];
    m.m1 = (seg & 1) ? 1.f : 0.f;
    m.m2 = (seg & 2) ? 1.f : 0.f;
    m.m4 = (seg & 4) ? 1.f : 0.f;
    m.deep = __any((seg & 128) != 0);
}

__device__ __forceinline__ void zero_scratch(unsigned char* scr, int lane) {
    static_assert(SCR_BYTES % (64 * 16) == 0, "one 16-byte store per lane and round");
#pragma unroll
    for (int i = 0; i < SCR_BYTES / (64 * 16); ++i)
        reinterpret_cast<float4*>(scr)[i * 64 + lane] = make_float4(0.f, 0.f, 0.f, 0.f);
}

__device__ __forceinline__ void segment_suffix_sums(float& a, float& b, float& c, float& d, const MelLane& m) {
    asm("s_nop 1\n\t"
        "v_fmac_f32_dpp %0, %0, %4 row_shl:1 row_mask:0xf bank_mask:0xf bound_ctrl:1\n\t"
        "v_fmac_f32_dpp %1, %1, %4 row_shl:1 row_mask:0xf bank_mask:0xf bound_ctrl:1\n\t"
        "v_fmac_f32_dpp %2, %2, %4 row_shl:1 row_mask:0xf bank_mask:0xf bound_ctrl:1\n\t"
        "v_fmac_f32_dpp %3, %3, %4 row_shl:1 row_mask:0xf bank_mask:0xf bound_ctrl:1\n\t"
        "v_fmac_f32_dpp %0, %0, %5 row_shl:2 row_mask:0xf bank_mask:0xf bound_ctrl:1\n\t"
        "v_fmac_f32_dpp %1, %1, %5 row_shl:2 row_mask:0xf bank_mask:0xf bound_ctrl:1\n\t"
        "v_fmac_f32_dpp %2, %2, %5 row_shl:2 row_mask:0xf bank_mask:0xf bound_ctrl:1\n\t"
        "v_fmac_f32_dpp %3, %3, %5 row_shl:2 row_mask:0xf bank_mask:0xf bound_ctrl:1"
        : "+v"(a), "+v"(b), "+v"(c), "+v"(d)
        : "v"(m.m1), "v"(m.m2));
    if (m.deep)
        asm("s_nop 1\n\t"
            "v_fmac_f32_dpp %0, %0, %4 row_shl:4 row_mask:0xf bank_mask:0xf bound_ctrl:1\n\t"
            "v_fmac_f32_dpp %1, %1, %4 row_shl:4 row_mask:0xf bank_mask:0xf bound_ctrl:1\n\t"
            "v_fmac_f32_dpp %2, %2, %4 row_shl:4 row_mask:0xf bank_mask:0xf bound_ctrl:1\n\t"
            "v_fmac_f32_dpp %3, %3, %4 row_shl:4 row_mask:0xf bank_mask:0xf bound_ctrl:1"
            : "+v"(a), "+v"(b), "+v"(c), "+v"(d)
            : "v"(m.m4));
}

__device__ __forceinline__ void wave_sum2_max2(float& a, float& b, float& ma, float& mb) {
#define KWS_DPP_STEP(ctrl)                                                      \
    "v_add_f32_dpp %0, %0, %0 " ctrl "\n\t"                                      \
    "v_add_f32_dpp %1, %1, %1 " ctrl "\n\t"                                      \
    "v_max_f32_dpp %2, %2, %2 " ctrl "\n\t"                                      \
    "v_max_f32_dpp %3, %3, %3 " ctrl "\n\t"
    asm("s_nop 1\n\t"
        KWS_DPP_STEP("row_shr:1 row_mask:0xf bank_mask:0xf bound_ctrl:1")
        KWS_DPP_STEP("row_shr:2 row_mask:0xf bank_mask:0xf bound_ctrl:1")
        KWS_DPP_STEP("row_shr:4 row_mask:0xf bank_mask:0xf bound_ctrl:1")
        KWS_DPP_STEP("row_shr:8 row_mask:0xf bank_mask:0xf bound_ctrl:1")
        KWS_DPP_STEP("row_bcast:15 row_mask:0xa bank_mask:0xf")
        KWS_DPP_STEP("row_bcast:31 row_mask:0xc bank_mask:0xf")
        "s_nop 0"
        : "+v"(a), "+v"(b), "+v"(ma), "+v"(mb));
#undef KWS_DPP_STEP
    a = __builtin_bit_cast(float, __builtin_amdgcn_readlane(__builtin_bit_cast(int, a), 63));
    b = __builtin_bit_cast(float, __builtin_amdgcn_readlane(__builtin_bit_cast(int, b), 63));
    ma = __builtin_bit_cast(float, __builtin_amdgcn_readlane(__builtin_bit_cast(int, ma), 63));
    mb = __builtin_bit_cast(float, __builtin_amdgcn_readlane(__builtin_bit_cast(int, mb), 63));
}

template <bool FULL>
__device__ __forceinline__ unsigned long long peak_over(float v, float lim) {
    float mn = v;
#define KWS_MM_STEP(ctrl)                                      \
    "v_min_f32_dpp %0, %0, %0 " ctrl "\n\t"                    \
    "s_nop 1\n\t"
    asm("s_nop 1\n\t"
        KWS_MM_STEP("row_shr:1 row_mask:0xf bank_mask:0xf")
        KWS_MM_STEP("row_shr:2 row_mask:0xf bank_mask:0xf")
        KWS_MM_STEP("row_shr:4 row_mask:0xf bank_mask:0xf")
        KWS_MM_STEP("row_shr:8 row_mask:0xf bank_mask:0xf")
        "v_min_f32_dpp %0, %0, %0 row_bcast:15 row_mask:0xa bank_mask:0xf"
        : "+v"(mn));
    if constexpr (FULL)
        asm("s_nop 1\n\t"
            "v_min_f32_dpp %0, %0, %0 row_bcast:31 row_mask:0xc bank_mask:0xf"
            : "+v"(mn));
#undef KWS_MM_STEP
    return __ballot(mn < lim);
}
__device__ __forceinline__ void peak_over2(float va, float vb, float lim_a, float lim_b, bool& over_a, bool& over_b) {
    float a = va, b = vb;
#define KWS_MM_STEP(ctrl)                                      \
    "v_min_f32_dpp %0, %0, %0 " ctrl "\n\t"                    \
    "v_min_f32_dpp %1, %1, %1 " ctrl "\n\t"                    \
    "s_nop 0\n\t"
    asm("s_nop 1\n\t"
        KWS_MM_STEP("row_shr:1 row_mask:0xf bank_mask:0xf")
        KWS_MM_STEP("row_shr:2 row_mask:0xf bank_mask:0xf")
        KWS_MM_STEP("row_shr:4 row_mask:0xf bank_mask:0xf")
        KWS_MM_STEP("row_shr:8 row_mask:0xf bank_mask:0xf")
        KWS_MM_STEP("row_bcast:15 row_mask:0xa bank_mask:0xf")
        KWS_MM_STEP("row_bcast:31 row_mask:0xc bank_mask:0xf")
        : "+v"(a), "+v"(b));
#undef KWS_MM_STEP
    over_a = (__ballot(a < lim_a) >> 63) & 1ull;
    over_b = (__ballot(b < lim_b) >> 63) & 1ull;
}

__device__ __forceinline__ uint32_t mfcc_pair(cf (&v)[8], bool nza, bool nzb, bool has_b, const FrontendParams& p,
                                          const PairScratch& sc, const cf (&t1)[8], const MelLane& ml, int lane,
                                          float* __restrict__ out_a, float* __restrict__ out_b,
                                          float* lds_out_a = nullptr) {
    cf* xbuf = sc.xbuf;
    float2* pbuf = sc.pbuf;
    float* lbuf = sc.lbuf;
    const float* dctb = sc.dctb;
    const cf* tw2 = sc.tw2;
    const uint32_t gth = ml.gth;
    const int nfp = sc.nfp;
    const PairLevel lv = equalise_levels(v);
#if !defined(KWS_X_MFCC_STOP) || KWS_X_MFCC_STOP >= 1
    fft512(v, xbuf, t1, tw2, lane);
#endif
#if defined(KWS_X_MFCC_STOP) && KWS_X_MFCC_STOP <= 1
    if (lane < p.numcep) out_a[lane] = v[0].x + v[1].y + v[2].x + v[3].y + v[4].x + v[5].y + v[6].x + v[7].y + lv.pow_a;
    return 0u;
#endif

    float ea, eb, pka = 0.f, pkb = 0.f;
    if (p.refine_span > 0.f) {
        split_power(v, xbuf, pbuf, lane, 1, nza, nzb, ml.pslot, -1, lv, ea, eb, &pka, &pkb);
        wave_sum2_max2(ea, eb, pka, pkb);
    } else {
        split_power(v, xbuf, pbuf, lane, 1, nza, nzb, ml.pslot, -1, lv, ea, eb);
        wave_sum2(ea, eb);
    }
#if defined(KWS_X_MFCC_STOP) && KWS_X_MFCC_STOP == 2
    if (lane < p.numcep) out_a[lane] = ea + eb + pbuf[lane].x;
    return 0u;
#endif

    float ra = 0.f, fa_ = 0.f, rb = 0.f, fb_ = 0.f;
    {
        const float4* pc = reinterpret_cast<const float4*>(pbuf + lane * MEL_STRIDE);
#pragma unroll
        for (int h = 0; h < MEL_CHUNK / 2; ++h) {
            const float4 pw = pc[h];
            ra = fmaf(ml.rw[2 * h], pw.x, ra);
            fa_ = fmaf(ml.fw[2 * h], pw.x, fa_);
            rb = fmaf(ml.rw[2 * h], pw.y, rb);
            fb_ = fmaf(ml.fw[2 * h], pw.y, fb_);
            ra = fmaf(ml.rw[2 * h + 1], pw.z, ra);
            fa_ = fmaf(ml.fw[2 * h + 1], pw.z, fa_);
            rb = fmaf(ml.rw[2 * h + 1], pw.w, rb);
            fb_ = fmaf(ml.fw[2 * h + 1], pw.w, fb_);
        }
    }
    segment_suffix_sums(ra, fa_, rb, fb_, ml);
    float ma, mb;
    uint32_t flags = 0u;
    {
        const int r0 = gth & 255, nr = (gth >> 8) & 255, q0 = (gth >> 16) & 255, nq = gth >> 24;
        const float gra = __builtin_bit_cast(float, __builtin_amdgcn_ds_bpermute(4 * r0, __builtin_bit_cast(int, ra)));
        const float grb = __builtin_bit_cast(float, __builtin_amdgcn_ds_bpermute(4 * r0, __builtin_bit_cast(int, rb)));
        const float gfa = __builtin_bit_cast(float, __builtin_amdgcn_ds_bpermute(4 * q0, __builtin_bit_cast(int, fa_)));
        const float gfb = __builtin_bit_cast(float, __builtin_amdgcn_ds_bpermute(4 * q0, __builtin_bit_cast(int, fb_)));
        const float sa = (nr ? gra : 0.f) + (nq ? gfa : 0.f);
        const float sb = (nr ? grb : 0.f) + (nq ? gfb : 0.f);
        if (p.nfilt <= 32) {
            const auto sw = __builtin_amdgcn_permlane32_swap(__builtin_bit_cast(unsigned, sa), __builtin_bit_cast(unsigned, sb), false, false);
            const float s = __builtin_bit_cast(float, (unsigned)sw[0]);
            const float l = logf(s == 0.f ? PSF_EPS : s);
            ma = __builtin_bit_cast(float, __builtin_amdgcn_readlane(__builtin_bit_cast(int, l), 0));
            mb = __builtin_bit_cast(float, __builtin_amdgcn_readlane(__builtin_bit_cast(int, l), 32));
#if defined(KWS_X_MFCC_STOP) && KWS_X_MFCC_STOP == 3
            if (lane < p.numcep) out_a[lane] = l + ea + eb;
            return 0u;
#endif
            const int f = lane >> 5, j = lane & 31;
            const float cv = j < p.nfilt ? l - (f ? mb : ma) : 0.f;
            lbuf[64 * f + j] = cv;
            if (p.refine_span > 0.f) {
                const float lim = 0.6931471806f * __builtin_amdgcn_logf(f ? pkb : pka) - (f ? mb : ma) - p.refine_span;
                const unsigned long long over = peak_over<false>(cv, lim);
                flags = (uint32_t)((over >> 31) & 1u) | ((uint32_t)((over >> 63) & 1u) << 1);
            }
        } else {
            const float la = logf(sa == 0.f ? PSF_EPS : sa), lb = logf(sb == 0.f ? PSF_EPS : sb);
            ma = __builtin_bit_cast(float, __builtin_amdgcn_readfirstlane(__builtin_bit_cast(int, la)));
            mb = __builtin_bit_cast(float, __builtin_amdgcn_readfirstlane(__builtin_bit_cast(int, lb)));
            const float cva = lane < p.nfilt ? la - ma : 0.f, cvb = lane < p.nfilt ? lb - mb : 0.f;
            lbuf[lane] = cva;
            lbuf[64 + lane] = cvb;
            if (p.refine_span > 0.f) {
                bool oa, ob;
                peak_over2(cva, cvb, 0.6931471806f * __builtin_amdgcn_logf(pka) - ma - p.refine_span, 0.6931471806f * __builtin_amdgcn_logf(pkb) - mb - p.refine_span, oa, ob);
                flags = (uint32_t)oa | ((uint32_t)ob << 1);
            }
        }
    }
    wave_lds_order();

    {
        const int f = lane >> 5, i = lane & 31;
        if (i < p.numcep && (f == 0 || has_b)) {
            const float4* L4 = reinterpret_cast<const float4*>(lbuf + 64 * f);
            const float4* D4 = reinterpret_cast<const float4*>(dctb + i * nfp);
            float acc = 0.f;
            if (nfp == 28) {
#pragma unroll
                for (int j0 = 0; j0 < 7; j0 += 4) {
                    float4 d[4], l[4];
#pragma unroll
                    for (int j = 0; j < 4; ++j)
                        if (j0 + j < 7) d[j] = D4[j0 + j], l[j] = L4[j0 + j];
#pragma unroll
                    for (int j = 0; j < 4; ++j)
                        if (j0 + j < 7) {
                            acc = fmaf(d[j].x, l[j].x, acc);
                            acc = fmaf(d[j].y, l[j].y, acc);
                            acc = fmaf(d[j].z, l[j].z, acc);
                            acc = fmaf(d[j].w, l[j].w, acc);
                        }
                    __builtin_amdgcn_sched_barrier(0);
                }
            } else {
                for (int j = 0; j < nfp / 4; ++j) {
                    const float4 d = D4[j], l = L4[j];
                    acc = fmaf(d.x, l.x, acc);
                    acc = fmaf(d.y, l.y, acc);
                    acc = fmaf(d.z, l.z, acc);
                    acc = fmaf(d.w, l.w, acc);
                }
            }
            if (i == 0) {
                if (p.append_energy) {
                    const float e = f ? eb : ea;
                    acc = logf(e == 0.f ? PSF_EPS : e);
                } else {
                    float dsum = 0.f;
                    for (int j = 0; j < p.nfilt; ++j) dsum += dctb[j];
                    acc = fmaf(f ? mb : ma, dsum, acc);
                }
            }
            (f ? out_b : out_a)[i] = acc;
            if (lds_out_a && f == 0) lds_out_a[i] = acc;
        }
    }
    wave_lds_order();
    return has_b ? flags : (flags & 1u);
}


constexpr int STREAM_F64_BYTES = 16 * NFFT + 8 * 128;
__host__ __device__ __forceinline__ size_t stream_frame_lds_bytes(const FrontendParams& p) {
    const int nfp = (p.nfilt + 3) & ~3;
    return sizeof(float) * (size_t)(((p.numcep * nfp + 3) & ~3) + 2 * 64) + SCR_BYTES + STREAM_F64_BYTES;
}

template <typename F>
__device__ __forceinline__ void f64_redo_frame(const FrontendParams& p, const FrontendTables& t, d2* X, double* L, F&& get,
                                               float* __restrict__ out, float* lds_out, int lane) {
    bool nz = false;
#pragma unroll
    for (int n1 = 0; n1 < 8; ++n1) {
        const int i = 64 * n1 + lane;
        const float y = i < p.frame_len ? get(i) : 0.f;
        nz |= y != 0.f;
        X[sw512(i)] = d2{(double)y, 0.0};
    }
    nz = __any(nz);
    wave_order();
    spectrum_pair<true, NFFT>(X, X, reinterpret_cast<const d2*>(t.tw64), NFFT, 9, p.frame_len, 1.0 / (double)NFFT, lane);
    const F64Tabs tb = {reinterpret_cast<const d2*>(t.tw64), t.mel_w64, t.dct64, t.mel_edges};
    f64_tail<NBINS>(p, tb, NBINS, X, L, nz, false, false, out, out, lds_out, lane);
}
__device__ __forceinline__ long stream_frame_wave(const FrontendParams& p, const FrontendTables& t,
                                                  const int16_t* __restrict__ hop, int sa, int sb, bool has_b,
                                                  int16_t* __restrict__ pcm_ring, int ring_len,
                                                  float* __restrict__ feat_ring, int hops, unsigned char* smem, int lane,
                                                  float* lds_out_a, int* refine_ctr = nullptr) {
    const int nfp = (p.nfilt + 3) & ~3;
    float* dctb = reinterpret_cast<float*>(smem);
    cf* tw2 = reinterpret_cast<cf*>(dctb + ((p.numcep * nfp + 3) & ~3));
    unsigned char* scr = reinterpret_cast<unsigned char*>(tw2 + 64);
    const int step = p.frame_step;
    const long base = (long)step * hops;

    {
        const int n4 = (p.numcep * nfp + 3) / 4;
        const float4* src = reinterpret_cast<const float4*>(t.dct_pad);
        for (int i0 = 0; i0 < n4; i0 += 128) {
            const int i = i0 + lane, j = i + 64;
            const float4 a = i < n4 ? src[i] : make_float4(0.f, 0.f, 0.f, 0.f);
            const float4 b = j < n4 ? src[j] : make_float4(0.f, 0.f, 0.f, 0.f);
            if (i < n4) reinterpret_cast<float4*>(dctb)[i] = a;
            if (j < n4) reinterpret_cast<float4*>(dctb)[j] = b;
        }
    }
    fill_tw2(t.twiddle, tw2, lane);
    zero_scratch(scr, lane);
    cf t1[8];
    load_twiddles(t.twiddle, lane, t1);
    MelLane ml;
    load_mel_lane(t, lane, ml);

    const long f_start = base + step - ((p.frame_len + step - 1) / step) * step;
    const bool frame_ok = f_start >= 0;
    const long fidx = f_start / step;
    const int base_mod = (int)(base % ring_len);
    const int d0 = (int)(f_start - base);
    const int first_d = base < (long)ring_len ? -(int)base : -ring_len;
    auto sample = [&](int s, int d) -> float {
        int r = base_mod + d;
        r += r < 0 ? ring_len : 0;
        const int dc = d < first_d ? first_d : d;
        const int16_t* ptr = d >= 0 ? hop + (size_t)s * step + d : pcm_ring + (size_t)s * ring_len + (dc == d ? r : 0);
        const float x = to_unit(*ptr);
        return d < first_d ? 0.f : x;
    };
    cf v[8];
    bool nza = false, nzb = false;
    float carry_a = 0.f, carry_b = 0.f;
    int16_t app_a[8], app_b[8];
#pragma unroll
    for (int j = 0; j < 8; ++j) {
        app_a[j] = 0;
        app_b[j] = 0;
        if (64 * j < step) {
            const int i = 64 * j + lane;
            if (i < step) {
                app_a[j] = hop[(size_t)sa * step + i];
                if (has_b) app_b[j] = hop[(size_t)sb * step + i];
            }
        }
    }
    if (frame_ok) {
        carry_a = sample(sa, d0 - 1);
        if (has_b) carry_b = sample(sb, d0 - 1);
    }
#pragma unroll
    for (int n1 = 0; n1 < 8; ++n1) {
        const int i = 64 * n1 + lane;
        float ya = 0.f, yb = 0.f;
        if (frame_ok && 64 * n1 < p.frame_len) {
            const bool in = i < p.frame_len;
            const int d = d0 + (in ? i : 0);
            const bool first = f_start + i == 0;
            const float ca = sample(sa, d);
            float pa = __builtin_bit_cast(float, __builtin_amdgcn_update_dpp(0, __builtin_bit_cast(int, ca), 0x138, 0xf, 0xf, false));
            pa = lane == 0 ? carry_a : pa;
            carry_a = __builtin_bit_cast(float, __builtin_amdgcn_readlane(__builtin_bit_cast(int, ca), 63));
            ya = in ? (first ? ca : __fsub_rn(ca, __fmul_rn(p.preemph, pa))) : 0.f;
            if (has_b) {
                const float cb = sample(sb, d);
                float pb = __builtin_bit_cast(float, __builtin_amdgcn_update_dpp(0, __builtin_bit_cast(int, cb), 0x138, 0xf, 0xf, false));
                pb = lane == 0 ? carry_b : pb;
                carry_b = __builtin_bit_cast(float, __builtin_amdgcn_readlane(__builtin_bit_cast(int, cb), 63));
                yb = in ? (first ? cb : __fsub_rn(cb, __fmul_rn(p.preemph, pb))) : 0.f;
            }
        }
        v[n1].x = ya;
        v[n1].y = yb;
        nza |= ya != 0.f;
        nzb |= yb != 0.f;
    }
    nza = __any(nza);
    nzb = __any(nzb);
#pragma unroll
    for (int j = 0; j < 8; ++j) {
        const int i = 64 * j + lane;
        if (64 * j < step && i < step) {
            int pos = base_mod + i;
            pos -= pos >= ring_len ? ring_len : 0;
            pcm_ring[(size_t)sa * ring_len + pos] = app_a[j];
            if (has_b) pcm_ring[(size_t)sb * ring_len + pos] = app_b[j];
        }
    }
    wave_lds_order();
    if (frame_ok) {
        const PairScratch sc = {reinterpret_cast<cf*>(scr + SCR_XBUF), reinterpret_cast<float2*>(scr + SCR_PBUF),
                                reinterpret_cast<float*>(scr + SCR_LBUF),
                                dctb, tw2, nfp};
        const int row = (int)(fidx % p.num_frames);
        float* out_a = feat_ring + ((size_t)sa * p.num_frames + row) * p.numcep;
        float* out_b = feat_ring + ((size_t)sb * p.num_frames + row) * p.numcep;
        const uint32_t flags = mfcc_pair(v, nza, nzb, has_b, p, sc, t1, ml, lane, out_a, out_b, lds_out_a);
        if (flags) {
            d2* X = reinterpret_cast<d2*>(scr + SCR_BYTES);
            double* L = reinterpret_cast<double*>(scr + SCR_BYTES + 16 * NFFT);
            auto frame_of = [&](int s) {
                return [&, s](int i) -> float {
                    const float cur = sample(s, d0 + i);
                    return f_start + i == 0 ? cur : __fsub_rn(cur, __fmul_rn(p.preemph, sample(s, d0 + i - 1)));
                };
            };
            if (flags & 1u) f64_redo_frame(p, t, X, L, frame_of(sa), out_a, lds_out_a, lane);
            if (flags & 2u) f64_redo_frame(p, t, X, L, frame_of(sb), out_b, nullptr, lane);
            if (refine_ctr && lane == 0) atomicAdd(refine_ctr + 5, (int)__builtin_popcount(flags));
        }
    }
    return frame_ok ? fidx : -1;
}

}
}
```

### keyword-spotting_amd/kws/_native/__init__.py

```python
from __future__ import annotations

import ctypes as C
import os
import threading

import numpy as np

from kws.common.errors import AudioProcessingError, KWSError, ModelError

LIB_PATH = os.environ.get("KWS_HIP_LIB") or os.path.join(os.path.dirname(os.path.abspath(__file__)), "libkws_hip.so")

KWS_OK, KWS_EINVAL, KWS_ENOMEM, KWS_EHIP, KWS_ESTATE, KWS_EUNSUPPORTED = 0, -1, -2, -3, -4, -5
KWS_CT_F16_PAIR, KWS_CT_BF16_TRIPLE = 0, 1
KWS_K_MFCC, KWS_K_DSCNN, KWS_K_CNNTRAD_CONV, KWS_K_CNNTRAD_DENSE, KWS_K_STREAM_FRAME, KWS_K_MFCC_F64, KWS_K_MFCC_REFINE = 0, 1, 2, 3, 4, 5, 6
KWS_K_DSCNN_LOAD_STATS, KWS_K_DSCNN_LOAD_PACK, KWS_K_DSCNN_LOAD_FILL = 7, 8, 9
KWS_K_RESAMPLE = 10
FE_REFINE_SPAN_DEFAULT = 10.2
FE_F32, FE_F64 = 0, 1
ACT_FLOATS_PER_CLIP = 64 * (141 + 141 + 245 + 357) + 64 + 64 * 477
PW_F32 = 1
PW_SPLIT_BF16 = 4
PW_PAIR_F16 = 5
PW_DEFAULT = PW_PAIR_F16

_c_ctx = C.c_void_p
_i16p, _f32p, _i32p = C.c_void_p, C.c_void_p, C.c_void_p

SIGNATURES = {
    "kws_abi_version": (C.c_int, []),
    "kws_create": (C.c_int, [C.POINTER(_c_ctx), C.c_int]),
    "kws_destroy": (None, [_c_ctx]),
    "kws_set_stream": (C.c_int, [_c_ctx, C.c_void_p, C.c_int]),
    "kws_sync": (C.c_int, [_c_ctx]),
    "kws_last_error": (C.c_char_p, [_c_ctx]),
    "kws_set_frontend": (C.c_int, [_c_ctx] + [C.c_int] * 7 + [C.c_float, C.c_int]),
    "kws_set_frontend_math": (C.c_int, [_c_ctx, C.c_int]),
    "kws_frontend_math": (C.c_int, [_c_ctx]),
    "kws_set_frontend_refine": (C.c_int, [_c_ctx, C.c_float]),
    "kws_frontend_stats": (C.c_int, [_c_ctx, C.POINTER(C.c_uint64), C.POINTER(C.c_uint64), C.POINTER(C.c_int)]),
    "kws_spec_f32": (C.c_int, [_c_ctx, _f32p, C.c_int, C.c_int, C.c_int, C.c_int, _f32p]),
    "kws_frontend_shape": (C.c_int, [_c_ctx, C.POINTER(C.c_int), C.POINTER(C.c_int)]),
    "kws_mfcc_i16": (C.c_int, [_c_ctx, _i16p, C.c_int, _f32p]),
    "kws_mfcc_f32": (C.c_int, [_c_ctx, _f32p, C.c_int, _f32p]),
    "kws_load_dscnn": (C.c_int, [_c_ctx, C.POINTER(C.c_float), C.c_size_t, C.c_int]),
    "kws_load_dscnn_ex": (C.c_int, [_c_ctx, C.POINTER(C.c_float), C.c_size_t, C.c_int, C.c_int]),
    "kws_load_dscnn_device": (C.c_int, [_c_ctx, _f32p, C.c_size_t, C.c_int, C.c_int]),
    "kws_dscnn_image_read": (C.c_int, [_c_ctx, C.POINTER(C.c_uint32), C.c_size_t, C.POINTER(C.c_size_t), C.POINTER(C.c_float)]),
    "kws_forward_f32": (C.c_int, [_c_ctx, _f32p, C.c_int, _f32p, _i32p]),
    "kws_forward_map_f32": (C.c_int, [_c_ctx, _f32p, C.c_int, C.c_int, C.c_int, _f32p, _i32p]),
    "kws_forward_map_debug_f32": (C.c_int, [_c_ctx, _f32p, C.c_int, C.c_int, C.c_int, _f32p, _i32p, _f32p]),
    "kws_infer_i16": (C.c_int, [_c_ctx, _i16p, C.c_int, _f32p, _i32p]),
    "kws_dscnn_backward_f32": (C.c_int, [_c_ctx, _f32p, C.c_int, C.c_int, C.c_int, _f32p, _f32p]),
    "kws_dsblock_forward_f32": (C.c_int, [_c_ctx, _f32p, C.c_int, C.c_int, C.c_int, C.c_int, _f32p, _f32p, _f32p, _f32p, C.c_int, C.c_int,
                                          C.c_int, C.c_int, _f32p]),
    "kws_infer_f32": (C.c_int, [_c_ctx, _f32p, C.c_int, _f32p, _i32p]),
    "kws_infer_host_i16": (C.c_int, [_c_ctx, C.c_void_p, C.c_int, C.c_void_p, C.c_void_p]),
    "kws_infer_host_submit_i16": (C.c_int, [_c_ctx, C.c_void_p, C.c_int, C.c_void_p, C.c_void_p, C.POINTER(C.c_uint64)]),
    "kws_infer_host_wait": (C.c_int, [_c_ctx, C.c_uint64]),
    "kws_ingest_config": (C.c_int, [_c_ctx, C.c_int, C.c_int, C.c_int]),
    "kws_reserve": (C.c_int, [_c_ctx, C.c_int]),
    "kws_set_pointwise_math": (C.c_int, [_c_ctx, C.c_int]),
    "kws_forward_debug_f32": (C.c_int, [_c_ctx, _f32p, C.c_int, _f32p, _i32p, _f32p, C.c_int]),
    "kws_stream_open": (C.c_int, [_c_ctx, C.c_int]),
    "kws_stream_close": (C.c_int, [_c_ctx]),
    "kws_stream_cluster": (C.c_int, [_c_ctx, C.c_int]),
    "kws_stream_host_results": (C.c_int, [_c_ctx, C.c_int]),
    "kws_stream_wait_host": (C.c_int, [_c_ctx, C.POINTER(C.c_void_p), C.POINTER(C.c_void_p)]),
    "kws_stream_push_host_i16": (C.c_int, [_c_ctx, C.c_void_p, C.POINTER(C.c_void_p), C.POINTER(C.c_void_p)]),
    "kws_stream_push_i16": (C.c_int, [_c_ctx, _i16p, _f32p, _i32p, C.c_int]),
    "kws_stream_state": (C.c_int, [_c_ctx, C.POINTER(C.c_void_p), C.POINTER(C.c_int)]),
    "kws_stream_copy_features": (C.c_int, [_c_ctx, _f32p]),
    "kws_load_cnn_trad": (C.c_int, [_c_ctx, C.POINTER(C.c_float), C.c_size_t, C.c_int]),
    "kws_load_cnn_trad_device": (C.c_int, [_c_ctx, _f32p, C.c_size_t, C.c_int]),
    "kws_cnn_trad_backward_f32": (C.c_int, [_c_ctx, _f32p, C.c_int, _f32p, _f32p]),
    "kws_cnn_trad_train_debug_f32": (C.c_int, [_c_ctx, _f32p, C.c_int, _f32p, _i32p, _f32p, _f32p]),
    "kws_stream_vad_f32": (C.c_int, [_c_ctx, C.c_float, C.c_int, C.c_int, _i32p]),
    "kws_forward_cnn_trad_f32": (C.c_int, [_c_ctx, _f32p, C.c_int, _f32p, _i32p]),
    "kws_forward_cnn_trad_debug_f32": (C.c_int, [_c_ctx, _f32p, C.c_int, _f32p, _i32p, _f32p, _f32p]),
    "kws_set_cnn_trad_math": (C.c_int, [_c_ctx, C.c_int]),
    "kws_infer_cnn_trad_i16": (C.c_int, [_c_ctx, _i16p, C.c_int, _f32p, _i32p]),
    "kws_softmax_f32": (C.c_int, [_c_ctx, _f32p, C.c_int, C.c_int, _f32p]),
    "kws_stream_smooth_f32": (C.c_int, [_c_ctx, _f32p, C.c_int, C.c_int, _f32p, _i32p]),
    "kws_scan_i16": (C.c_int, [_c_ctx, _i16p, C.c_int, C.c_int, C.c_int, _f32p, _i32p, _f32p]),
    "kws_scan_detect_f32": (C.c_int, [_c_ctx, _f32p, C.c_int, C.c_int, C.c_int, C.c_int, C.c_int, C.c_float, C.c_int, _f32p, _i32p, _i32p,
                                      _f32p, C.c_int, _i32p]),
    "kws_frames_i16": (C.c_int, [_c_ctx, _i16p, C.c_int, C.c_int, _f32p]),
    "kws_segment_f32": (C.c_int, [_c_ctx, _f32p, C.c_int, C.c_int, C.c_int, C.c_float, C.c_int, C.c_int, C.c_int, C.c_int, _i32p, C.c_int,
                                  _i32p]),
    "kws_cut_i16": (C.c_int, [_c_ctx, _i16p, C.c_int, C.c_int, _i32p, C.c_int, C.c_int, _i16p, C.c_int, _i32p]),
    "kws_host_stream_utt_history": (C.c_int, [C.c_int] * 5 + [C.POINTER(C.c_int)]),
    "kws_stream_utt_open": (C.c_int, [_c_ctx, C.c_float] + [C.c_int] * 6),
    "kws_stream_utt_close": (C.c_int, [_c_ctx]),
    "kws_stream_utt_step_i16": (C.c_int, [_c_ctx, _i16p, _f32p]),
    "kws_stream_utt_flush": (C.c_int, [_c_ctx]),
    "kws_stream_utt_poll": (C.c_int, [_c_ctx, C.POINTER(C.c_uint64), C.POINTER(C.c_uint64)]),
    "kws_stream_utt_read": (C.c_int, [_c_ctx, C.c_uint64, C.c_int, C.POINTER(C.c_int64)]),
    "kws_stream_utt_cut_i16": (C.c_int, [_c_ctx, C.c_uint64, C.c_int, C.c_int, _i16p, C.c_int, _i32p]),
    "kws_resample_i16": (C.c_int, [_c_ctx, _i16p, C.c_int, C.c_int, _i32p, C.c_int, C.c_int, _i16p, C.c_int]),
    "kws_resample_f32": (C.c_int, [_c_ctx, _f32p, C.c_int, C.c_int, _i32p, C.c_int, C.c_int, _f32p, C.c_int]),
    "kws_host_stream_resample_plan": (C.c_int, [C.c_int, C.c_int] + [C.POINTER(C.c_int)] * 4),
    "kws_host_stream_resample_count": (C.c_int, [C.c_int, C.c_int, C.c_uint64, C.c_int, C.POINTER(C.c_int)]),
    "kws_stream_resample_open": (C.c_int, [_c_ctx, C.c_int, C.c_int, C.c_int, C.c_int, C.c_uint64]),
    "kws_stream_resample_close": (C.c_int, [_c_ctx]),
    "kws_stream_resample_i16": (C.c_int, [_c_ctx, _i16p, C.c_int, _i16p, C.c_int, C.POINTER(C.c_int)]),
    "kws_stream_push_rate_i16": (C.c_int, [_c_ctx, _i16p, C.c_int, _f32p, _i32p]),
    "kws_stream_push_host_rate_i16": (C.c_int, [_c_ctx, C.c_void_p, C.c_int, C.POINTER(C.c_void_p), C.POINTER(C.c_void_p)]),
    "kws_eval_open": (C.c_int, [_c_ctx, C.c_int, C.c_int]),
    "kws_eval_reset": (C.c_int, [_c_ctx]),
    "kws_eval_close": (C.c_int, [_c_ctx]),
    "kws_eval_update_f32": (C.c_int, [_c_ctx, _f32p, _i32p, C.c_int, C.c_float, _f32p, _f32p]),
    "kws_eval_read": (C.c_int, [_c_ctx, C.POINTER(C.c_uint64), C.POINTER(C.c_double), C.POINTER(C.c_uint64), C.POINTER(C.c_uint64),
                                C.POINTER(C.c_uint64)]),
    "kws_augment_i16": (C.c_int, [_c_ctx, _i16p, C.c_int, C.c_void_p, _f32p, C.c_int, C.c_void_p, _f32p, C.c_void_p, _f32p]),
    "kws_augment_draw": (C.c_int, [_c_ctx, C.c_uint64, C.c_uint32, _i32p, C.c_int, _i32p, C.c_int, C.c_int, _i32p, _i32p, C.c_int, C.c_float,
                                   C.c_float, C.c_int, C.c_int, _i32p, _i32p, _f32p, C.c_void_p]),
    "kws_mfcc_augment_i16": (C.c_int, [_c_ctx, _i16p, C.c_int, _i32p, C.c_int, C.c_void_p, _f32p, C.c_int, C.c_void_p, _f32p, C.c_void_p,
                                       _f32p]),
    "kws_forward_stamps_f32": (C.c_int, [_c_ctx, _f32p, C.c_int, _f32p, C.c_void_p, C.c_int]),
    "kws_preemphasis_f32": (C.c_int, [_c_ctx, _f32p, C.c_int, C.c_float, _f32p]),
    "kws_framesig_f32": (C.c_int, [_c_ctx, _f32p, C.c_int, C.c_int, C.c_int, _f32p, _f32p]),
    "kws_spec512_f32": (C.c_int, [_c_ctx, _f32p, C.c_int, C.c_int, C.c_int, _f32p]),
    "kws_prof_enable": (C.c_int, [_c_ctx, C.c_int]),
    "kws_prof_reset": (C.c_int, [_c_ctx]),
    "kws_prof_read": (C.c_int, [_c_ctx, C.c_int, C.POINTER(C.c_double), C.POINTER(C.c_int)]),
    "kws_kernel_name": (C.c_char_p, [C.c_int]),
    "kws_host_mel_edges": (C.c_int, [C.c_int, C.c_int, C.c_int, C.POINTER(C.c_int)]),
    "kws_host_mel_dense": (C.c_int, [C.c_int, C.c_int, C.c_int, C.POINTER(C.c_float)]),
    "kws_host_mel_layout": (C.c_int, [C.c_int, C.c_int, C.c_int, C.POINTER(C.c_int), C.POINTER(C.c_int), C.POINTER(C.c_int),
                                      C.POINTER(C.c_int)]),
    "kws_host_dct_lifter": (C.c_int, [C.c_int, C.c_int, C.c_int, C.POINTER(C.c_float)]),
    "kws_host_dscnn_image": (C.c_int, [C.POINTER(C.c_float), C.c_size_t, C.c_int, C.c_int, C.POINTER(C.c_uint32), C.c_size_t,
                                       C.POINTER(C.c_size_t), C.POINTER(C.c_float)]),
    "kws_host_cnn_trad_image": (C.c_int, [C.POINTER(C.c_float), C.c_size_t, C.c_int, C.POINTER(C.c_uint32), C.c_size_t,
                                          C.POINTER(C.c_size_t), C.POINTER(C.c_float)]),
    "kws_host_scan_shape": (C.c_int, [C.c_int] * 5 + [C.POINTER(C.c_int), C.POINTER(C.c_int)]),
    "kws_host_resample_len": (C.c_int, [C.c_int, C.c_int, C.c_int, C.POINTER(C.c_int)]),
    "kws_host_resample_design": (C.c_int, [C.c_int, C.c_int] + [C.POINTER(C.c_int)] * 4 + [C.POINTER(C.c_double), C.c_size_t,
                                           C.POINTER(C.c_size_t)]),
}

_lib = None
_lock = threading.Lock()


def lib() -> C.CDLL:
    global _lib
    if _lib is not None:
        return _lib
    with _lock:
        if _lib is None:
            if not os.path.exists(LIB_PATH):
                raise KWSError(
                    f"native library missing: {LIB_PATH} (build it with `python -c 'import __graft_entry__ as g; g.build()'` "
                    "or `make -C keyword-spotting_amd/csrc`); there is no CPU fallback"
                )
            try:
                h = C.CDLL(LIB_PATH)
            except OSError as e:
                raise KWSError(f"cannot load {LIB_PATH}: {e}") from e
            for name, (res, args) in SIGNATURES.items():
                fn = getattr(h, name)
                fn.restype = res
                fn.argtypes = args
            _lib = h
    return _lib


def _ptr(t) -> int:
    return int(t.data_ptr())


class Context:

    def __init__(self, device: int = 0, error_cls=KWSError):
        self._h = _c_ctx()
        self._lib = lib()
        rc = self._lib.kws_create(C.byref(self._h), int(device))
        if rc != KWS_OK:
            msg = self._lib.kws_last_error(None).decode()
            self._h = _c_ctx()
            raise error_cls(f"kws_create failed ({rc}): {msg}")
        self.device = int(device)
        self.num_classes = None

    def close(self):
        if getattr(self, "_h", None) and self._h.value:
            self._lib.kws_destroy(self._h)
            self._h = _c_ctx()

    def __del__(self):
        try:
            self.close()
        except Exception:
            pass

    def _check(self, rc: int, error_cls=KWSError):
        if rc != KWS_OK:
            raise error_cls(f"{self._lib.kws_last_error(self._h).decode()} (code {rc})")

    def use_torch_stream(self):
        import torch

        self._check(self._lib.kws_set_stream(self._h, C.c_void_p(torch.cuda.current_stream(self.device).cuda_stream), 1))

    def use_own_stream(self):
        self._check(self._lib.kws_set_stream(self._h, None, 0))

    def sync(self):
        self._check(self._lib.kws_sync(self._h))

    def set_frontend(self, sample_rate=16000, n_samples=16000, frame_len=400, frame_step=160, nfft=512, nfilt=26,
                     numcep=10, preemph=0.97, ceplifter=22):
        self._check(
            self._lib.kws_set_frontend(self._h, sample_rate, n_samples, frame_len, frame_step, nfft, nfilt, numcep,
                                       float(preemph), ceplifter),
            AudioProcessingError,
        )

    def set_frontend_math(self, math: int):
        self._check(self._lib.kws_set_frontend_math(self._h, int(math)), AudioProcessingError)

    def frontend_math(self) -> int:
        return int(self._lib.kws_frontend_math(self._h))

    def set_frontend_refine(self, log_span: float = FE_REFINE_SPAN_DEFAULT):
        self._check(self._lib.kws_set_frontend_refine(self._h, float(log_span)), AudioProcessingError)

    def frontend_stats(self):
        total, refined, last = C.c_uint64(), C.c_uint64(), C.c_int()
        self._check(self._lib.kws_frontend_stats(self._h, C.byref(total), C.byref(refined), C.byref(last)), AudioProcessingError)
        return int(total.value), int(refined.value), int(last.value)

    def frontend_shape(self):
        nf, nc = C.c_int(), C.c_int()
        self._check(self._lib.kws_frontend_shape(self._h, C.byref(nf), C.byref(nc)), AudioProcessingError)
        return nf.value, nc.value

    def mfcc_i16(self, wav, out):
        self._check(self._lib.kws_mfcc_i16(self._h, _ptr(wav), int(wav.shape[0]), _ptr(out)), AudioProcessingError)

    def mfcc_f32(self, wav, out):
        self._check(self._lib.kws_mfcc_f32(self._h, _ptr(wav), int(wav.shape[0]), _ptr(out)), AudioProcessingError)

    def load_dscnn(self, blob: np.ndarray, num_classes: int, input_channels: int = 1):
        blob = np.ascontiguousarray(blob, dtype=np.float32)
        self._check(
            self._lib.kws_load_dscnn_ex(self._h, blob.ctypes.data_as(C.POINTER(C.c_float)), blob.size, int(num_classes),
                                        int(input_channels)),
            ModelError,
        )
        self.num_classes = int(num_classes)

    def load_dscnn_device(self, blob, num_classes: int, input_channels: int = 1):
        self._check(self._lib.kws_load_dscnn_device(self._h, _ptr(blob), int(blob.numel()), int(num_classes), int(input_channels)),
                    ModelError)
        self.num_classes = int(num_classes)

    def dscnn_image(self):
        need = C.c_size_t(0)
        self._check(self._lib.kws_dscnn_image_read(self._h, None, 0, C.byref(need), None), ModelError)
        words, scalars = np.empty(need.value, np.uint32), np.empty(23, np.float32)
        self._check(self._lib.kws_dscnn_image_read(self._h, words.ctypes.data_as(C.POINTER(C.c_uint32)), words.size, None,
                                                   scalars.ctypes.data_as(C.POINTER(C.c_float))), ModelError)
        return words, scalars

    def forward_f32(self, feat, logits, label=None):
        self._check(
            self._lib.kws_forward_f32(self._h, _ptr(feat), int(feat.shape[0]), _ptr(logits), _ptr(label) if label is not None else None),
            ModelError,
        )

    def forward_map_f32(self, feat, logits, label=None, layers=None):
        B, _, T, F = (int(v) for v in feat.shape)
        lab = _ptr(label) if label is not None else None
        if layers is None:
            self._check(self._lib.kws_forward_map_f32(self._h, _ptr(feat), B, T, F, _ptr(logits), lab), ModelError)
        else:
            self._check(self._lib.kws_forward_map_debug_f32(self._h, _ptr(feat), B, T, F, _ptr(logits), lab, _ptr(layers)), ModelError)

    def dscnn_backward_f32(self, feat, T, F, dlogits, grad):
        self._check(self._lib.kws_dscnn_backward_f32(self._h, _ptr(feat), int(feat.shape[0]), int(T), int(F), _ptr(dlogits), _ptr(grad)),
                    ModelError)

    def load_cnn_trad(self, blob: np.ndarray, num_classes: int):
        blob = np.ascontiguousarray(blob, dtype=np.float32)
        self._check(self._lib.kws_load_cnn_trad(self._h, blob.ctypes.data_as(C.POINTER(C.c_float)), blob.size, int(num_classes)),
                    ModelError)

    def load_cnn_trad_device(self, blob, num_classes: int):
        self._check(self._lib.kws_load_cnn_trad_device(self._h, _ptr(blob), int(blob.numel()), int(num_classes)), ModelError)

    def cnn_trad_backward_f32(self, feat, dlogits, grad):
        self._check(self._lib.kws_cnn_trad_backward_f32(self._h, _ptr(feat), int(feat.shape[0]), _ptr(dlogits), _ptr(grad)), ModelError)

    def cnn_trad_train_debug_f32(self, feat, conv1, winner, conv2, hidden):
        self._check(self._lib.kws_cnn_trad_train_debug_f32(self._h, _ptr(feat), int(feat.shape[0]), _ptr(conv1), _ptr(winner), _ptr(conv2),
                                                           _ptr(hidden)), ModelError)

    def set_cnn_trad_math(self, math: int):
        self._check(self._lib.kws_set_cnn_trad_math(self._h, int(math)), ModelError)

    def forward_cnn_trad_f32(self, feat, logits, label=None):
        self._check(self._lib.kws_forward_cnn_trad_f32(self._h, _ptr(feat), int(feat.shape[0]), _ptr(logits),
                                                       _ptr(label) if label is not None else None), ModelError)

    def forward_cnn_trad_debug_f32(self, feat, logits, label, conv2, clip_scale=None):
        self._check(self._lib.kws_forward_cnn_trad_debug_f32(self._h, _ptr(feat), int(feat.shape[0]), _ptr(logits),
                                                             _ptr(label) if label is not None else None, _ptr(conv2),
                                                             _ptr(clip_scale) if clip_scale is not None else None), ModelError)

    def infer_cnn_trad_i16(self, wav, logits, label=None):
        self._check(self._lib.kws_infer_cnn_trad_i16(self._h, _ptr(wav), int(wav.shape[0]), _ptr(logits),
                                                     _ptr(label) if label is not None else None), ModelError)

    def softmax_f32(self, logits, prob):
        self._check(self._lib.kws_softmax_f32(self._h, _ptr(logits), int(logits.shape[0]), int(logits.shape[1]), _ptr(prob)),
                    ModelError)

    def stream_smooth_f32(self, logits, window, smoothed, label=None):
        self._check(self._lib.kws_stream_smooth_f32(self._h, _ptr(logits), int(logits.shape[1]), int(window), _ptr(smoothed),
                                                    _ptr(label) if label is not None else None), ModelError)

    def stream_vad_f32(self, threshold, on_window, off_window, state):
        self._check(self._lib.kws_stream_vad_f32(self._h, float(threshold), int(on_window), int(off_window), _ptr(state)), ModelError)

    def set_pointwise_math(self, math):
        self._check(self._lib.kws_set_pointwise_math(self._h, int(math)), ModelError)

    def forward_debug_f32(self, feat, logits, label, act, use_mfma=PW_SPLIT_BF16):
        self._check(
            self._lib.kws_forward_debug_f32(self._h, _ptr(feat), int(feat.shape[0]), _ptr(logits),
                                            _ptr(label) if label is not None else None,
                                            _ptr(act) if act is not None else None, int(use_mfma)),
            ModelError,
        )

    def forward_stamps_f32(self, feat, logits, stamps, mode=PW_SPLIT_BF16):
        self._check(self._lib.kws_forward_stamps_f32(self._h, _ptr(feat), int(feat.shape[0]), _ptr(logits), _ptr(stamps), int(mode)), ModelError)

    def infer_i16(self, wav, logits, label=None):
        self._check(
            self._lib.kws_infer_i16(self._h, _ptr(wav), int(wav.shape[0]), _ptr(logits), _ptr(label) if label is not None else None),
            ModelError,
        )

    def dsblock_forward_f32(self, x, dw_w, dw_b, pw_w, pw_b, kernel_size, stride, padding, out):
        B, c_in, H, W = (int(v) for v in x.shape)
        self._check(self._lib.kws_dsblock_forward_f32(self._h, _ptr(x), B, c_in, H, W, _ptr(dw_w), _ptr(dw_b), _ptr(pw_w), _ptr(pw_b),
                                                      int(pw_w.shape[0]), int(kernel_size), int(stride), int(padding), _ptr(out)), ModelError)

    def infer_host_i16(self, wav: np.ndarray, logits: np.ndarray = None, label: np.ndarray = None):
        logits, label, ticket, _keep = self.infer_host_submit_i16(wav, logits, label)
        self.infer_host_wait(ticket)
        return logits, label

    def infer_host_wait(self, ticket: int = 0):
        self._check(self._lib.kws_infer_host_wait(self._h, C.c_uint64(int(ticket))), ModelError)

    def infer_host_submit_i16(self, wav: np.ndarray, logits: np.ndarray = None, label: np.ndarray = None):
        if self.num_classes is None:
            raise ModelError("no model loaded (kws_load_dscnn)")
        if hasattr(wav, "data_ptr"):
            if wav.is_cuda or wav.dtype.__str__() != "torch.int16" or not wav.is_contiguous() or wav.dim() != 2:
                raise ModelError("infer_host_i16 expects a contiguous CPU int16 tensor [B, n_samples]")
            src, B = int(wav.data_ptr()), int(wav.shape[0])
        else:
            wav = np.ascontiguousarray(wav, dtype=np.int16)
            if wav.ndim != 2:
                raise ModelError("infer_host_i16 expects int16 [B, n_samples]")
            src, B = wav.ctypes.data, int(wav.shape[0])
        if logits is None:
            logits = np.empty((B, self.num_classes), np.float32)
        if label is None:
            label = np.empty((B,), np.int32)
        assert logits.dtype == np.float32 and logits.flags.c_contiguous and logits.shape == (B, self.num_classes)
        assert label.dtype == np.int32 and label.flags.c_contiguous and label.shape == (B,)
        ticket = C.c_uint64(0)
        self._check(self._lib.kws_infer_host_submit_i16(self._h, C.c_void_p(src), B, C.c_void_p(logits.ctypes.data),
                                                        C.c_void_p(label.ctypes.data), C.byref(ticket)), ModelError)
        return logits, label, int(ticket.value), wav

    def ingest_config(self, chunk_clips: int = 0, n_slots: int = 0, pack_threads: int = 0):
        self._check(self._lib.kws_ingest_config(self._h, int(chunk_clips), int(n_slots), int(pack_threads)), ModelError)

    def infer_f32(self, wav, logits, label=None):
        self._check(
            self._lib.kws_infer_f32(self._h, _ptr(wav), int(wav.shape[0]), _ptr(logits), _ptr(label) if label is not None else None),
            ModelError,
        )

    def scan_i16(self, pcm, hop_frames, logits, label=None, feat=None):
        p = lambda t: _ptr(t) if t is not None else None
        self._check(self._lib.kws_scan_i16(self._h, _ptr(pcm), int(pcm.shape[0]), int(pcm.shape[1]), int(hop_frames), _ptr(logits),
                                           p(label), p(feat)), ModelError)

    def scan_detect_f32(self, logits, smooth_window, first_keyword, threshold, refractory, event_count, event_window=None,
                        event_label=None, event_score=None, max_events=0, smoothed=None):
        p = lambda t: _ptr(t) if t is not None else None
        R, W, Cn = (int(v) for v in logits.shape)
        self._check(self._lib.kws_scan_detect_f32(self._h, _ptr(logits), R, W, Cn, int(smooth_window), int(first_keyword), float(threshold),
                                                  int(refractory), p(smoothed), p(event_window), p(event_label), p(event_score),
                                                  int(max_events), _ptr(event_count)), ModelError)

    def frames_i16(self, pcm, feat):
        self._check(self._lib.kws_frames_i16(self._h, _ptr(pcm), int(pcm.shape[0]), int(pcm.shape[1]), _ptr(feat)), AudioProcessingError)

    def segment_f32(self, feat, n_total, threshold, count, utt=None, max_utts=0, on_window=40, off_window=80, pre_roll=60,
                    max_frames=1000):
        self._check(self._lib.kws_segment_f32(self._h, _ptr(feat), int(feat.shape[0]), int(feat.shape[1]), int(n_total), float(threshold),
                                              int(on_window), int(off_window), int(pre_roll), int(max_frames),
                                              _ptr(utt) if utt is not None else None, int(max_utts), _ptr(count)), ModelError)

    def cut_i16(self, pcm, span, clips, normalize_to=16384, peak=None):
        self._check(self._lib.kws_cut_i16(self._h, _ptr(pcm), int(pcm.shape[0]), int(pcm.shape[1]), _ptr(span), int(span.shape[0]),
                                          int(normalize_to), _ptr(clips), int(clips.shape[1]), _ptr(peak) if peak is not None else None),
                    AudioProcessingError)

    def stream_utt_open(self, threshold, on_window, off_window, pre_roll, max_frames, history_samples, max_events):
        self._check(self._lib.kws_stream_utt_open(self._h, float(threshold), int(on_window), int(off_window), int(pre_roll),
                                                  int(max_frames), int(history_samples), int(max_events)), ModelError)

    def stream_utt_close(self):
        self._check(self._lib.kws_stream_utt_close(self._h), ModelError)

    def stream_utt_step_i16(self, hop=None, energy=None):
        p = lambda t: None if t is None else (int(t) if isinstance(t, int) else _ptr(t))
        self._check(self._lib.kws_stream_utt_step_i16(self._h, p(hop), p(energy)), ModelError)

    def stream_utt_flush(self):
        self._check(self._lib.kws_stream_utt_flush(self._h), ModelError)

    def stream_utt_poll(self):
        total, steps = C.c_uint64(0), C.c_uint64(0)
        self._check(self._lib.kws_stream_utt_poll(self._h, C.byref(total), C.byref(steps)), ModelError)
        return int(total.value), int(steps.value)

    def stream_utt_read(self, first_seq: int, n: int) -> np.ndarray:
        out = np.empty((max(int(n), 0), 6), np.int64)
        self._check(self._lib.kws_stream_utt_read(self._h, C.c_uint64(int(first_seq)), int(n), out.ctypes.data_as(C.POINTER(C.c_int64))),
                    ModelError)
        return out

    def stream_utt_cut_i16(self, first_seq: int, clips, normalize_to=16384, peak=None):
        self._check(self._lib.kws_stream_utt_cut_i16(self._h, C.c_uint64(int(first_seq)), int(clips.shape[0]), int(normalize_to), _ptr(clips),
                                                     int(clips.shape[1]), _ptr(peak) if peak is not None else None), AudioProcessingError)

    def _resample(self, fn, x, rate_in, rate_out, out, lengths):
        self._check(fn(self._h, _ptr(x), int(x.shape[0]), int(x.shape[1]), _ptr(lengths) if lengths is not None else None, int(rate_in),
                       int(rate_out), _ptr(out), int(out.shape[1])), AudioProcessingError)

    def resample_i16(self, pcm, rate_in, rate_out, out, lengths=None):
        self._resample(self._lib.kws_resample_i16, pcm, rate_in, rate_out, out, lengths)

    def resample_f32(self, signal, rate_in, rate_out, out, lengths=None):
        self._resample(self._lib.kws_resample_f32, signal, rate_in, rate_out, out, lengths)

    @staticmethod
    def host_stream_resample_plan(rate_in, rate_out):
        return host_stream_resample_plan(rate_in, rate_out)

    @staticmethod
    def host_stream_resample_count(rate_in, rate_out, samples_before, n_in) -> int:
        return host_stream_resample_count(rate_in, rate_out, samples_before, n_in)

    def stream_resample_open(self, n_streams: int, rate_in: int, rate_out: int, max_in: int, first_sample: int = 0):
        self._check(self._lib.kws_stream_resample_open(self._h, int(n_streams), int(rate_in), int(rate_out), int(max_in),
                                                       C.c_uint64(int(first_sample))), AudioProcessingError)

    def stream_resample_close(self):
        self._check(self._lib.kws_stream_resample_close(self._h), AudioProcessingError)

    def stream_resample_i16(self, pcm, out) -> int:
        n = C.c_int(0)
        self._check(self._lib.kws_stream_resample_i16(self._h, _ptr(pcm), int(pcm.shape[1]), _ptr(out), int(out.shape[1]), C.byref(n)),
                    AudioProcessingError)
        return n.value

    def stream_push_rate_i16(self, pcm, logits=None, label=None):
        self._check(self._lib.kws_stream_push_rate_i16(self._h, _ptr(pcm), int(pcm.shape[1]), _ptr(logits) if logits is not None else None,
                                                       _ptr(label) if label is not None else None), ModelError)

    def stream_push_host_rate_i16(self, pcm: np.ndarray, n_streams: int):
        if pcm.dtype != np.int16 or not pcm.flags.c_contiguous or pcm.ndim != 2 or pcm.shape[0] != n_streams:
            raise ModelError("stream_push_host_rate_i16 expects a C-contiguous int16 array [n_streams, n_in]")
        pl, py = C.c_void_p(), C.c_void_p()
        self._check(self._lib.kws_stream_push_host_rate_i16(self._h, pcm.ctypes.data, int(pcm.shape[1]), C.byref(pl), C.byref(py)), ModelError)
        return self._host_views_of(pl, py, n_streams)

    def eval_open(self, num_classes: int, n_bins: int = 256):
        self._check(self._lib.kws_eval_open(self._h, int(num_classes), int(n_bins)), ModelError)
        self._eval_shape = (int(num_classes), int(n_bins))

    def eval_reset(self):
        self._check(self._lib.kws_eval_reset(self._h), ModelError)

    def eval_close(self):
        self._check(self._lib.kws_eval_close(self._h), ModelError)
        self._eval_shape = None

    def eval_update_f32(self, logits, truth, grad_scale: float = 0.0, dlogits=None, loss_rows=None):
        p = lambda t: _ptr(t) if t is not None else None
        self._check(self._lib.kws_eval_update_f32(self._h, _ptr(logits), _ptr(truth), int(logits.shape[0]), float(grad_scale), p(dlogits),
                                                  p(loss_rows)), ModelError)

    def eval_read(self):
        shape = getattr(self, "_eval_shape", None)
        if shape is None:
            raise ModelError("eval_read: call eval_open first")
        Cn, K = shape
        u64 = C.POINTER(C.c_uint64)
        counts, loss = np.zeros(4, np.uint64), C.c_double(0.0)
        confusion = np.zeros((Cn, Cn), np.uint64)
        pos, neg = np.zeros((Cn, K), np.uint64), np.zeros((Cn, K), np.uint64)
        self._check(self._lib.kws_eval_read(self._h, counts.ctypes.data_as(u64), C.byref(loss), confusion.ctypes.data_as(u64),
                                            pos.ctypes.data_as(u64) if K else None, neg.ctypes.data_as(u64) if K else None), ModelError)
        return counts, float(loss.value), confusion, pos, neg

    def stream_open(self, n_streams: int):
        self._check(self._lib.kws_stream_open(self._h, int(n_streams)), AudioProcessingError)

    def stream_cluster(self, workgroups_per_stream: int = 0):
        self._check(self._lib.kws_stream_cluster(self._h, int(workgroups_per_stream)), ModelError)

    def stream_host_results(self, enable: bool = True):
        self._check(self._lib.kws_stream_host_results(self._h, 1 if enable else 0), ModelError)
        self._host_views = None

    def stream_push_host_i16(self, hop: np.ndarray, n_streams: int):
        if hop.dtype != np.int16 or not hop.flags.c_contiguous:
            raise ModelError("stream_push_host_i16 expects a C-contiguous int16 array")
        pl, py = C.c_void_p(), C.c_void_p()
        self._check(self._lib.kws_stream_push_host_i16(self._h, hop.ctypes.data, C.byref(pl), C.byref(py)), ModelError)
        return self._host_views_of(pl, py, n_streams)

    def stream_wait_host(self, n_streams: int):
        pl, py = C.c_void_p(), C.c_void_p()
        self._check(self._lib.kws_stream_wait_host(self._h, C.byref(pl), C.byref(py)), ModelError)
        return self._host_views_of(pl, py, n_streams)

    def _host_views_of(self, pl, py, n_streams):
        if getattr(self, "_host_views", None) is None or self._host_views[0] != (pl.value, py.value, n_streams):
            lg = np.ctypeslib.as_array(C.cast(pl, C.POINTER(C.c_float)), shape=(n_streams, self.num_classes))
            lb = np.ctypeslib.as_array(C.cast(py, C.POINTER(C.c_int32)), shape=(n_streams,))
            self._host_views = ((pl.value, py.value, n_streams), lg, lb)
        return self._host_views[1], self._host_views[2]

    def stream_close(self):
        self._check(self._lib.kws_stream_close(self._h))

    def stream_push_i16(self, hop, logits=None, label=None, use_graph=False):
        self._check(
            self._lib.kws_stream_push_i16(self._h, _ptr(hop), _ptr(logits) if logits is not None else None,
                                          _ptr(label) if label is not None else None, 1 if use_graph else 0),
            ModelError,
        )

    def stream_state(self):
        ring, hops = C.c_void_p(), C.c_int()
        self._check(self._lib.kws_stream_state(self._h, C.byref(ring), C.byref(hops)))
        return ring.value, hops.value

    def stream_copy_features(self, out):
        self._check(self._lib.kws_stream_copy_features(self._h, _ptr(out)))

    def augment_i16(self, wav, out, shift=None, bg=None, bg_off=None, bg_vol=None, silence=None):
        p = lambda t: _ptr(t) if t is not None else None
        self._check(
            self._lib.kws_augment_i16(self._h, _ptr(wav), int(wav.shape[0]), p(shift), p(bg), int(bg.numel()) if bg is not None else 0,
                                      p(bg_off), p(bg_vol), p(silence), _ptr(out)),
            AudioProcessingError,
        )

    def augment_draw(self, seed, epoch, index, shift, bg_off, bg_vol, silence, labels=None, time_shift=0, bg_start=None, bg_len=None,
                     bg_volume=0.0, bg_frequency=0.0, use_background=True, n_samples=16000):
        p = lambda t: _ptr(t) if t is not None else None
        self._check(
            self._lib.kws_augment_draw(self._h, int(seed) & 0xFFFFFFFFFFFFFFFF, int(epoch) & 0xFFFFFFFF, _ptr(index), int(index.numel()),
                                       p(labels), int(labels.numel()) if labels is not None else 0, int(time_shift), p(bg_start),
                                       p(bg_len), int(bg_start.numel()) if bg_start is not None else 0, float(bg_volume),
                                       float(bg_frequency), int(bool(use_background)), int(n_samples), _ptr(shift), _ptr(bg_off),
                                       _ptr(bg_vol), _ptr(silence)),
            AudioProcessingError,
        )

    def mfcc_augment_i16(self, pcm, index, out, shift=None, bg=None, bg_off=None, bg_vol=None, silence=None) -> int:
        p = lambda t: _ptr(t) if t is not None else None
        rc = self._lib.kws_mfcc_augment_i16(self._h, _ptr(pcm), int(pcm.shape[0]), _ptr(index), int(index.numel()), p(shift), p(bg),
                                            int(bg.numel()) if bg is not None else 0, p(bg_off), p(bg_vol), p(silence), _ptr(out))
        if rc != KWS_EUNSUPPORTED:
            self._check(rc, AudioProcessingError)
        return rc

    def reserve(self, max_batch: int):
        self._check(self._lib.kws_reserve(self._h, int(max_batch)))

    def preemphasis_f32(self, sig, coeff, out):
        self._check(self._lib.kws_preemphasis_f32(self._h, _ptr(sig), int(sig.numel()), float(coeff), _ptr(out)), AudioProcessingError)

    def framesig_f32(self, sig, frame_len, frame_step, window, frames):
        self._check(
            self._lib.kws_framesig_f32(self._h, _ptr(sig), int(sig.numel()), int(frame_len), int(frame_step),
                                       _ptr(window) if window is not None else None, _ptr(frames)),
            AudioProcessingError,
        )

    def spec_f32(self, frames, nfft, power, spec):
        self._check(
            self._lib.kws_spec_f32(self._h, _ptr(frames), int(frames.shape[0]), int(frames.shape[1]), int(nfft), 1 if power else 0, _ptr(spec)),
            AudioProcessingError,
        )

    def spec512_f32(self, frames, power, spec):
        self._check(
            self._lib.kws_spec512_f32(self._h, _ptr(frames), int(frames.shape[0]), int(frames.shape[1]), 1 if power else 0, _ptr(spec)),
            AudioProcessingError,
        )

    def prof_enable(self, on=True):
        self._check(self._lib.kws_prof_enable(self._h, int(on)))

    def prof_reset(self):
        self._check(self._lib.kws_prof_reset(self._h))

    def prof_read(self, kernel_id: int):
        ms, n = C.c_double(), C.c_int()
        self._check(self._lib.kws_prof_read(self._h, int(kernel_id), C.byref(ms), C.byref(n)))
        return ms.value, n.value


def kernel_name(kernel_id: int) -> str:
    return lib().kws_kernel_name(int(kernel_id)).decode()


def host_mel_edges(nfilt=26, nfft=512, sample_rate=16000) -> np.ndarray:
    out = (C.c_int * (nfilt + 2))()
    rc = lib().kws_host_mel_edges(nfilt, nfft, sample_rate, out)
    if rc != KWS_OK:
        raise KWSError(f"kws_host_mel_edges failed ({rc})")
    return np.array(out[:], dtype=np.int64)


def host_mel_dense(nfilt=26, nfft=512, sample_rate=16000) -> np.ndarray:
    out = np.zeros((nfilt, nfft // 2 + 1), np.float32)
    rc = lib().kws_host_mel_dense(nfilt, nfft, sample_rate, out.ctypes.data_as(C.POINTER(C.c_float)))
    if rc != KWS_OK:
        raise KWSError(f"kws_host_mel_dense failed ({rc})")
    return out


def host_mel_layout(nfilt=26, nfft=512, sample_rate=16000):
    first = (C.c_int * (nfilt + 1))()
    count = (C.c_int * (nfilt + 1))()
    used, safe = C.c_int(0), C.c_int(0)
    rc = lib().kws_host_mel_layout(nfilt, nfft, sample_rate, first, count, C.byref(used), C.byref(safe))
    if rc != KWS_OK:
        raise KWSError(f"kws_host_mel_layout failed ({rc})")
    return np.array(first[:], dtype=np.int64), np.array(count[:], dtype=np.int64), int(used.value), bool(safe.value)


def host_dct_lifter(nfilt=26, numcep=10, ceplifter=22) -> np.ndarray:
    out = np.zeros((numcep, nfilt), np.float32)
    rc = lib().kws_host_dct_lifter(nfilt, numcep, ceplifter, out.ctypes.data_as(C.POINTER(C.c_float)))
    if rc != KWS_OK:
        raise KWSError(f"kws_host_dct_lifter failed ({rc})")
    return out


def host_scan_shape(n_total, frame_len=400, frame_step=160, window_frames=99, hop_frames=1):
    frames, windows = C.c_int(0), C.c_int(0)
    rc = lib().kws_host_scan_shape(int(n_total), int(frame_len), int(frame_step), int(window_frames), int(hop_frames),
                                   C.byref(frames), C.byref(windows))
    if rc != KWS_OK:
        raise KWSError(f"kws_host_scan_shape failed ({rc}): sizes must be positive")
    return int(frames.value), int(windows.value)


def host_stream_utt_history(frame_len=400, frame_step=160, pre_roll=60, max_frames=1000, slack_hops=8) -> int:
    n = C.c_int(0)
    rc = lib().kws_host_stream_utt_history(int(frame_len), int(frame_step), int(pre_roll), int(max_frames), int(slack_hops), C.byref(n))
    if rc != KWS_OK:
        raise ModelError(f"kws_host_stream_utt_history({frame_len}, {frame_step}, {pre_roll}, {max_frames}, {slack_hops}) failed (code {rc})")
    return int(n.value)


def host_resample_len(n_in, rate_in, rate_out) -> int:
    n = C.c_int(0)
    rc = lib().kws_host_resample_len(int(n_in), int(rate_in), int(rate_out), C.byref(n))
    if rc != KWS_OK:
        raise AudioProcessingError(f"kws_host_resample_len({n_in}, {rate_in}, {rate_out}) failed (code {rc})")
    return int(n.value)


def host_stream_resample_plan(rate_in, rate_out):
    v = [C.c_int(0) for _ in range(4)]
    rc = lib().kws_host_stream_resample_plan(int(rate_in), int(rate_out), *(C.byref(x) for x in v))
    if rc != KWS_OK:
        raise AudioProcessingError(f"kws_host_stream_resample_plan({rate_in}, {rate_out}) failed (code {rc})")
    return tuple(x.value for x in v)


def host_stream_resample_count(rate_in, rate_out, samples_before, n_in) -> int:
    n = C.c_int(0)
    rc = lib().kws_host_stream_resample_count(int(rate_in), int(rate_out), C.c_uint64(int(samples_before)), int(n_in), C.byref(n))
    if rc != KWS_OK:
        raise AudioProcessingError(f"kws_host_stream_resample_count({rate_in}, {rate_out}, {samples_before}, {n_in}) failed (code {rc})")
    return n.value


def host_resample_design(rate_in, rate_out):
    up, down, half, tile, need = C.c_int(0), C.c_int(0), C.c_int(0), C.c_int(0), C.c_size_t(0)
    fn = lib().kws_host_resample_design
    rc = fn(int(rate_in), int(rate_out), C.byref(up), C.byref(down), C.byref(half), C.byref(tile), None, 0, C.byref(need))
    if rc == KWS_OK:
        taps = np.empty(need.value, np.float64)
        rc = fn(int(rate_in), int(rate_out), None, None, None, None, taps.ctypes.data_as(C.POINTER(C.c_double)), taps.size, None)
    if rc != KWS_OK:
        raise AudioProcessingError(f"{lib().kws_last_error(None).decode()} (code {rc})")
    return int(up.value), int(down.value), int(half.value), int(tile.value), taps


def _host_image(fn, n_scalars, blob, *dims):
    blob = np.ascontiguousarray(blob, dtype=np.float32)
    bp, need = blob.ctypes.data_as(C.POINTER(C.c_float)), C.c_size_t(0)
    rc = fn(bp, blob.size, *dims, None, 0, C.byref(need), None)
    if rc != KWS_OK:
        raise ModelError(f"{lib().kws_last_error(None).decode()} (code {rc})")
    words, scalars = np.empty(need.value, np.uint32), np.empty(n_scalars, np.float32)
    rc = fn(bp, blob.size, *dims, words.ctypes.data_as(C.POINTER(C.c_uint32)), words.size, None,
            scalars.ctypes.data_as(C.POINTER(C.c_float)))
    if rc != KWS_OK:
        raise ModelError(f"{lib().kws_last_error(None).decode()} (code {rc})")
    return words, scalars


def host_dscnn_image(blob: np.ndarray, num_classes: int, input_channels: int = 1):
    return _host_image(lib().kws_host_dscnn_image, 23, blob, int(num_classes), int(input_channels))


def host_cnn_trad_image(blob: np.ndarray, num_classes: int):
    return _host_image(lib().kws_host_cnn_trad_image, 7, blob, int(num_classes))


_contexts: dict = {}


def default_context(device: int = 0) -> Context:
    ctx = _contexts.get(device)
    if ctx is None:
        ctx = _contexts[device] = Context(device)
    return ctx
```

Baseline: 7.034 million.

## Add compile-time specialized MFCC kernel for the reference frontend geometry

Adds a GeomRef template path for the MFCC wave-resident kernel, used when the frontend matches the reference frame length, step, filter and cepstrum counts. Constants are baked in, LDS frame reads become inline ds_read2 assembly, the mel accumulation uses packed FMA, and the per-frame zero/nonzero checks and some bookkeeping are dropped. A no-flag variant leaves out the refine flag logic. The aim is fewer instructions and less register pressure on the common path, at the cost of more code and a route switch (auto or generic) that lets users fall back to the generic kernel.

```diff
diff --git a/include/kws_hip.h b/include/kws_hip.h
--- a/include/kws_hip.h
+++ b/include/kws_hip.h
@@ -40,6 +40,10 @@
 #define KWS_FE_F64 1
 int kws_set_frontend_math(kws_ctx* ctx, int math);
 int kws_frontend_math(kws_ctx* ctx);
+
+#define KWS_FE_ROUTE_AUTO 0
+#define KWS_FE_ROUTE_GENERIC 1
+int kws_set_frontend_route(kws_ctx* ctx, int route);
 
 #define KWS_FE_REFINE_SPAN_DEFAULT 10.2f
 int kws_set_frontend_refine(kws_ctx* ctx, float log_ratio);
diff --git a/keyword-spotting_amd/csrc/kws_ctx.h b/keyword-spotting_amd/csrc/kws_ctx.h
--- a/keyword-spotting_amd/csrc/kws_ctx.h
+++ b/keyword-spotting_amd/csrc/kws_ctx.h
@@ -34,6 +34,8 @@
     FrontendParams fp{};
     bool fe_ready = false;
     bool fe_fast_ok = false;
+    bool fe_ref_geometry = false;
+    int fe_route = KWS_FE_ROUTE_AUTO;
     int fe_math = KWS_FE_F32;
     void* d_fe = nullptr;
     FrontendTables ft{};
diff --git a/keyword-spotting_amd/csrc/kws_frontend.hip b/keyword-spotting_amd/csrc/kws_frontend.hip
--- a/keyword-spotting_amd/csrc/kws_frontend.hip
+++ b/keyword-spotting_amd/csrc/kws_frontend.hip
@@ -48,20 +48,21 @@
             return KWS_OK;
         }
     c->frames_seen += (unsigned long long)B * p.num_frames;
+    const bool ref_route = c->fe_ref_geometry && c->fe_route == KWS_FE_ROUTE_AUTO;
     if (p.refine_span > 0.f) {
         int rc = ensure_refine(c, B, p.num_frames);
         if (rc) return rc;
         const RefineList rl = {c->d_refine, c->d_refine + 8, c->refine_cap, 0};
         {
             ProfScope ps(c, KWS_K_MFCC);
-            HIP_TRY(c, launch_mfcc(c->stream, p, c->ft, src, B, d_out, rl));
+            HIP_TRY(c, launch_mfcc(c->stream, p, c->ft, src, B, d_out, rl, ref_route));
         }
         ProfScope ps(c, KWS_K_MFCC_REFINE);
         HIP_TRY(c, launch_mfcc_refine(c->stream, p, c->ft, src, d_out, rl, refine_clips));
         return KWS_OK;
     }
     ProfScope ps(c, KWS_K_MFCC);
-    HIP_TRY(c, launch_mfcc(c->stream, p, c->ft, src, B, d_out, RefineList{}));
+    HIP_TRY(c, launch_mfcc(c->stream, p, c->ft, src, B, d_out, RefineList{}, ref_route));
     return KWS_OK;
 }
 template int run_frontend(kws_ctx*, const FrontendParams&, const int16_t*, int, float*, int);
@@ -111,6 +112,7 @@
     c->nfft = nfft;
     c->ceplifter = ceplifter;
     c->fe_fast_ok = im.fast && mfcc_tile_lds_bytes(p) <= MFCC_TILE_LDS_MAX;
+    c->fe_ref_geometry = c->fe_fast_ok && mfcc_reference_geometry(p);
     c->fe_ready = true;
     return KWS_OK;
     KWS_GUARD_END(c, "kws_set_frontend")
@@ -120,6 +122,14 @@
     if (!c) return KWS_EINVAL;
     if (math != KWS_FE_F32 && math != KWS_FE_F64) return fail(c, KWS_EINVAL, "kws_set_frontend_math: math must be KWS_FE_F32 or KWS_FE_F64");
     c->fe_math = math;
+    return KWS_OK;
+}
+
+int kws_set_frontend_route(kws_ctx* c, int route) {
+    if (!c) return KWS_EINVAL;
+    if (route != KWS_FE_ROUTE_AUTO && route != KWS_FE_ROUTE_GENERIC)
+        return fail(c, KWS_EINVAL, "kws_set_frontend_route: route must be KWS_FE_ROUTE_AUTO or KWS_FE_ROUTE_GENERIC");
+    c->fe_route = route;
     return KWS_OK;
 }
 
diff --git a/keyword-spotting_amd/csrc/kws_internal.h b/keyword-spotting_amd/csrc/kws_internal.h
--- a/keyword-spotting_amd/csrc/kws_internal.h
+++ b/keyword-spotting_amd/csrc/kws_internal.h
@@ -74,11 +74,11 @@
 
 struct AugmentArgs;
 hipError_t launch_mfcc(hipStream_t s, const FrontendParams& p, const FrontendTables& t, const int16_t* d_wav, int B, float* d_out,
-                       const RefineList& rl);
+                       const RefineList& rl, bool ref_route);
 hipError_t launch_mfcc(hipStream_t s, const FrontendParams& p, const FrontendTables& t, const float* d_wav, int B, float* d_out,
-                       const RefineList& rl);
+                       const RefineList& rl, bool ref_route);
 hipError_t launch_mfcc(hipStream_t s, const FrontendParams& p, const FrontendTables& t, const AugmentArgs& a, int B, float* d_out,
-                       const RefineList& rl);
+                       const RefineList& rl, bool ref_route);
 hipError_t launch_mfcc_refine(hipStream_t s, const FrontendParams& p, const FrontendTables& t, const int16_t* d_wav, float* d_out,
                               const RefineList& rl, int B);
 hipError_t launch_mfcc_refine(hipStream_t s, const FrontendParams& p, const FrontendTables& t, const float* d_wav, float* d_out,
@@ -123,6 +123,7 @@
 };
 hipError_t launch_augment_draw(hipStream_t s, const DrawArgs& d, int B);
 bool mfcc_wave_resident_ok(const FrontendParams& p);
+bool mfcc_reference_geometry(const FrontendParams& p);
 size_t mfcc_tile_lds_bytes(const FrontendParams& p);
 constexpr size_t MFCC_TILE_LDS_MAX = 160 * 1024;
 hipError_t launch_preemphasis(hipStream_t s, const float* d_in, int n, float coeff, float* d_out);
diff --git a/keyword-spotting_amd/csrc/kws_mfcc.hip b/keyword-spotting_amd/csrc/kws_mfcc.hip
--- a/keyword-spotting_amd/csrc/kws_mfcc.hip
+++ b/keyword-spotting_amd/csrc/kws_mfcc.hip
@@ -205,20 +205,22 @@
     return sizeof(float) * (size_t)(((p.numcep * nfp + 3) & ~3) + 2 * 64) + (size_t)MFCC_WAVES * WR_WAVE_BYTES;
 }
 
-template <bool AUG>
+template <bool AUG, class G = GeomAny>
 __device__ __forceinline__ void mfcc_wr_body(FrontendParams p, FrontendTables t, const int16_t* __restrict__ wav,
                                              float* __restrict__ out, RefineList rl, int B, int chunks_per_wave,
                                              AugmentArgs aug) {
     extern __shared__ __attribute__((aligned(16))) unsigned char smem[];
-    const int nfp = (p.nfilt + 3) & ~3;
+    static_assert(!(AUG && G::REF), "the fused loader keeps the generic geometry");
+    const int nfp = (G::nfilt(p) + 3) & ~3;
+    const int numcep = G::numcep(p), frame_step = G::frame_step(p);
     float* dctb = reinterpret_cast<float*>(smem);
-    cf* tw2 = reinterpret_cast<cf*>(dctb + ((p.numcep * nfp + 3) & ~3));
-    const int tid = threadIdx.x, lane = tid & 63, wv = tid >> 6;
+    cf* tw2 = reinterpret_cast<cf*>(dctb + ((numcep * nfp + 3) & ~3));
+    const int tid = threadIdx.x, lane = tid & 63, wv = G::REF ? uniform_i(tid >> 6) : tid >> 6;
     unsigned char* mine = reinterpret_cast<unsigned char*>(tw2 + 64) + wv * WR_WAVE_BYTES;
     float* ybuf = reinterpret_cast<float*>(mine);
     unsigned char* scr = mine + WR_SPAN * 4;
 
-    for (int i = tid; i < (p.numcep * nfp + 3) / 4; i += MFCC_THREADS)
+    for (int i = tid; i < (numcep * nfp + 3) / 4; i += MFCC_THREADS)
         reinterpret_cast<float4*>(dctb)[i] = reinterpret_cast<const float4*>(t.dct_pad)[i];
     fill_tw2(t.twiddle, tw2, tid);
     cf t1[8];
@@ -237,11 +239,11 @@
     const int16_t* __restrict__ x = AUG ? nullptr : wav + (size_t)(active ? clip : 0) * p.n_samples;
     AugClip ac{};
     if constexpr (AUG) ac = aug_clip(aug, active ? clip : 0, p.n_samples);
-    const int chunk_step = WR_FRAMES * p.frame_step;
+    const int chunk_step = WR_FRAMES * frame_step;
 
     uint4 v0 = make_uint4(0, 0, 0, 0), v1 = v0;
     int16_t before = 0;
-    auto fetch = [&](int cc) {
+    auto fetch = [&](int cc, int lane) {
         const int s0 = cc * chunk_step;
         const int n0 = s0 + 8 * lane, n1 = n0 + 512;
         v0 = n0 + 8 <= p.n_samples ? *reinterpret_cast<const uint4*>(x + n0) : make_uint4(0, 0, 0, 0);
@@ -256,8 +258,9 @@
     const float pre = p.preemph;
     uint32_t fmask = 0u;
     int pair0 = 2 * c;
+    float* orow = G::REF ? out + ((size_t)clip * p.num_frames + WR_FRAMES * c) * REF_NUMCEP : nullptr;
 #define KWS_FLUSH_FLAGS()                                                                                                          \
-    if (fmask && rl.ctr) {                                                                                                          \
+    if (fmask && (G::REF || rl.ctr)) {                                                                                              \
         const int lane = (int)__builtin_amdgcn_mbcnt_hi(~0u, __builtin_amdgcn_mbcnt_lo(~0u, 0u));  \
         const uint32_t fk = lane < 16 ? (fmask >> (2 * lane)) & 3u : 0u;                                                            \
         const uint32_t has = (uint32_t)__ballot(fk != 0u);                                                                          \
@@ -270,7 +273,7 @@
             rl.list[at] = (int)((((unsigned)(rl.clip0 + clip) * (unsigned)((p.num_frames + 1) / 2) + (unsigned)(pair0 + lane)) << 2) | fk); \
     }
     for (; c < c_end; ++c) {
-        if constexpr (!AUG) fetch(c);
+        if constexpr (!AUG) fetch(c, lane);
         if constexpr (AUG) {
             const int s0 = c * chunk_step;
             float a0[8], a1[8];
@@ -313,10 +316,17 @@
                     y[i] = __fsub_rn(cur, __fmul_rn(pre, prev));
                     prev = cur;
                 }
-                if (n == 0) y[0] = to_unit((int16_t)(wd[0] & 0xffffu));
-                if (n + 8 > p.n_samples) {
-#pragma unroll
-                    for (int i = 0; i < 8; ++i) y[i] = 0.f;
+#ifdef KWS_X_MFCC_NO_BOOKKEEPING
+                if constexpr (!G::REF)
+#endif
+                {
+                    if (n == 0) y[0] = to_unit((int16_t)(wd[0] & 0xffffu));
+                    if constexpr (G::REF) {
+                        if (n + 8 > p.n_samples) y[0] = 0.f;
+                    } else if (n + 8 > p.n_samples) {
+#pragma unroll
+                        for (int i = 0; i < 8; ++i) y[i] = 0.f;
+                    }
                 }
                 reinterpret_cast<float4*>(dst)[0] = make_float4(y[0], y[1], y[2], y[3]);
                 reinterpret_cast<float4*>(dst)[1] = make_float4(y[4], y[5], y[6], y[7]);
@@ -325,54 +335,110 @@
             convert(v1, prev1, s0 + 512 + 8 * lane, ybuf + 512 + 8 * lane);
         }
         wave_lds_order();
+        if constexpr (G::REF) {
+            const float* ya = ybuf;
 #pragma unroll 1
-        for (int pr = 0; pr < WR_PAIRS; ++pr) {
-            const int fa = WR_FRAMES * c + 2 * pr;
-            if (fa >= p.num_frames) break;
-            const bool has_b = fa + 1 < p.num_frames;
-            const float* ya = ybuf + (2 * pr) * p.frame_step;
-            const float* yb = ya + p.frame_step;
-            cf v[8];
-            uint32_t ora = 0u, orb = 0u;
-#pragma unroll
-            for (int n1 = 0; n1 < 7; ++n1) {
-                const int i = 64 * n1 + lane;
-                float a = ya[i], b = yb[i];
-                if (n1 == 6) {
-                    const bool in = i < p.frame_len;
-                    a = in ? a : 0.f, b = in ? b : 0.f;
-                }
-                v[n1] = cf{a, b};
-                ora |= __builtin_bit_cast(uint32_t, a);
-                orb |= __builtin_bit_cast(uint32_t, b);
-            }
-            v[7] = cf{0.f, 0.f};
-            if (!has_b) {
-#pragma unroll
-                for (int n1 = 0; n1 < 7; ++n1) v[n1].y = 0.f;
-                orb = 0u;
-            }
-            const bool nza = __any((ora << 1) != 0u);
-            const bool nzb = __any((orb << 1) != 0u);
-            const uint32_t flags = mfcc_pair(v, nza, nzb, has_b, p, sc, t1, ml, lane,
-                                             out + ((size_t)clip * p.num_frames + fa) * p.numcep,
-                                             out + ((size_t)clip * p.num_frames + fa + 1) * p.numcep);
-            fmask |= flags << (2 * ((fa >> 1) - pair0));
-            wave_lds_order();
+            for (int pr = 0; pr < WR_PAIRS; ++pr, ya += 2 * REF_FRAME_STEP, orow += 2 * REF_NUMCEP) {
+                const int fa = WR_FRAMES * c + 2 * pr;
+                if (fa >= p.num_frames) break;
+                const bool has_b = fa + 1 < p.num_frames;
+                [[maybe_unused]] const float* yb = ya + REF_FRAME_STEP;
+                cf v[8];
+#ifdef KWS_X_MFCC_NO_BOOKKEEPING
+#pragma unroll
+                for (int n1 = 0; n1 < 7; ++n1) v[n1] = cf{ya[64 * n1 + lane], yb[64 * n1 + lane]};
+                v[7] = cf{0.f, 0.f};
+                const bool nza = true, nzb = true;
+#else
+                static_assert(REF_FRAME_STEP == 160 && REF_FRAME_LEN > 384 && REF_FRAME_LEN <= 448, "the offsets below");
+                {
+                    const uint32_t a0 = lds_addr(ya + lane);
+                    asm volatile(
+                        "ds_read2_b32 %0, %7 offset1:160\n\t"
+                        "ds_read2_b32 %1, %7 offset0:64 offset1:224\n\t"
+                        "ds_read2_b32 %2, %8 offset1:160\n\t"
+                        "ds_read2_b32 %3, %8 offset0:64 offset1:224\n\t"
+                        "ds_read2_b32 %4, %9 offset1:160\n\t"
+                        "ds_read2_b32 %5, %9 offset0:64 offset1:224\n\t"
+                        "ds_read2_b32 %6, %10 offset1:160\n\t"
+                        "s_waitcnt lgkmcnt(0)"
+                        : "=&v"(v[0]), "=&v"(v[1]), "=&v"(v[2]), "=&v"(v[3]), "=&v"(v[4]), "=&v"(v[5]), "=&v"(v[6])
+                        : "v"(a0), "v"(a0 + 512u), "v"(a0 + 1024u), "v"(a0 + 1536u)
+                        : "memory");
+                }
+                const bool in6 = lane < REF_FRAME_LEN - 384;
+                v[6] = cf{in6 ? v[6].x : 0.f, in6 ? v[6].y : 0.f};
+                v[7] = cf{0.f, 0.f};
+                if (!has_b) {
+                    asm volatile("" ::: "memory");
+#pragma unroll
+                    for (int n1 = 0; n1 < 7; ++n1) v[n1].y = 0.f;
+                }
+                const bool nza = true, nzb = true;
+#endif
+                const uint32_t flags = mfcc_pair<G>(v, nza, nzb, has_b, p, sc, t1, ml, lane, orow, orow + REF_NUMCEP, nullptr, t.mel_seg);
+                if constexpr (G::FLAGS) fmask |= flags << (2 * ((fa >> 1) - pair0));
+                wave_lds_order();
+            }
+        } else {
+#pragma unroll 1
+            for (int pr = 0; pr < WR_PAIRS; ++pr) {
+                const int fa = WR_FRAMES * c + 2 * pr;
+                if (fa >= p.num_frames) break;
+                const bool has_b = fa + 1 < p.num_frames;
+                const float* ya = ybuf + (2 * pr) * p.frame_step;
+                const float* yb = ya + p.frame_step;
+                cf v[8];
+                uint32_t ora = 0u, orb = 0u;
+#pragma unroll
+                for (int n1 = 0; n1 < 7; ++n1) {
+                    const int i = 64 * n1 + lane;
+                    float a = ya[i], b = yb[i];
+                    if (n1 == 6) {
+                        const bool in = i < p.frame_len;
+                        a = in ? a : 0.f, b = in ? b : 0.f;
+                    }
+                    v[n1] = cf{a, b};
+                    ora |= __builtin_bit_cast(uint32_t, a);
+                    orb |= __builtin_bit_cast(uint32_t, b);
+                }
+                v[7] = cf{0.f, 0.f};
+                if (!has_b) {
+#pragma unroll
+                    for (int n1 = 0; n1 < 7; ++n1) v[n1].y = 0.f;
+                    orb = 0u;
+                }
+                const bool nza = __any((ora << 1) != 0u);
+                const bool nzb = __any((orb << 1) != 0u);
+                const uint32_t flags = mfcc_pair(v, nza, nzb, has_b, p, sc, t1, ml, lane,
+                                                 out + ((size_t)clip * p.num_frames + fa) * p.numcep,
+                                                 out + ((size_t)clip * p.num_frames + fa + 1) * p.numcep);
+                fmask |= flags << (2 * ((fa >> 1) - pair0));
+                wave_lds_order();
+            }
         }
-        if (2 * (c + 1) - pair0 >= 16) {
-            KWS_FLUSH_FLAGS()
-            fmask = 0u;
-            pair0 = 2 * (c + 1);
-        }
-    }
-    KWS_FLUSH_FLAGS()
+        if constexpr (G::FLAGS)
+            if (2 * (c + 1) - pair0 >= 16) {
+                KWS_FLUSH_FLAGS()
+                fmask = 0u;
+                pair0 = 2 * (c + 1);
+            }
+    }
+    if constexpr (G::FLAGS) KWS_FLUSH_FLAGS()
 #undef KWS_FLUSH_FLAGS
 }
 
 __global__ __launch_bounds__(MFCC_THREADS) __attribute__((amdgpu_waves_per_eu(KWS_MFCC_EU, KWS_MFCC_EU))) void kws_mfcc_i16_kernel(
     FrontendParams p, FrontendTables t, const int16_t* __restrict__ wav, float* __restrict__ out, RefineList rl, int B, int chunks_per_wave) {
     mfcc_wr_body<false>(p, t, wav, out, rl, B, chunks_per_wave, AugmentArgs{});
+}
+__global__ __launch_bounds__(MFCC_THREADS) __attribute__((amdgpu_waves_per_eu(KWS_MFCC_EU, KWS_MFCC_EU))) void kws_mfcc_i16_ref_kernel(
+    FrontendParams p, FrontendTables t, const int16_t* __restrict__ wav, float* __restrict__ out, RefineList rl, int B, int chunks_per_wave) {
+    mfcc_wr_body<false, GeomRef<true>>(p, t, wav, out, rl, B, chunks_per_wave, AugmentArgs{});
+}
+__global__ __launch_bounds__(MFCC_THREADS) __attribute__((amdgpu_waves_per_eu(KWS_MFCC_EU, KWS_MFCC_EU))) void kws_mfcc_i16_ref_noflag_kernel(
+    FrontendParams p, FrontendTables t, const int16_t* __restrict__ wav, float* __restrict__ out, RefineList rl, int B, int chunks_per_wave) {
+    mfcc_wr_body<false, GeomRef<false>>(p, t, wav, out, rl, B, chunks_per_wave, AugmentArgs{});
 }
 #ifndef KWS_MFCC_AUG_EU
 #define KWS_MFCC_AUG_EU 4
@@ -472,6 +538,11 @@
     return mfcc_tail6(p) && p.vec_ok && (WR_FRAMES * p.frame_step) % 8 == 0 && (WR_FRAMES - 1) * p.frame_step + 448 <= WR_SPAN;
 }
 
+bool mfcc_reference_geometry(const FrontendParams& p) {
+    return p.frame_len == REF_FRAME_LEN && p.frame_step == REF_FRAME_STEP && p.nfilt == REF_NFILT && p.numcep == REF_NUMCEP &&
+           p.append_energy != 0;
+}
+
 static int mfcc_wr_chunks_per_wave(int nb, int n_chunks) {
     int wpc = (n_chunks + 2) / 5;
     wpc = wpc < 1 ? 1 : wpc;
@@ -514,18 +585,23 @@
 }
 
 hipError_t launch_mfcc(hipStream_t s, const FrontendParams& p, const FrontendTables& t, const int16_t* d_wav, int B, float* d_out,
-                       const RefineList& rl) {
+                       const RefineList& rl, bool ref_route) {
 #ifndef KWS_X_MFCC_TILE_KERNEL
-    if (mfcc_wave_resident_ok(p)) return launch_mfcc_wr(kws_mfcc_i16_kernel, s, p, t, d_wav, B, d_out, rl);
+    if (mfcc_wave_resident_ok(p)) {
+        if (ref_route && mfcc_reference_geometry(p))
+            return launch_mfcc_wr(rl.ctr && p.refine_span > 0.f ? kws_mfcc_i16_ref_kernel : kws_mfcc_i16_ref_noflag_kernel, s, p, t,
+                                  d_wav, B, d_out, rl);
+        return launch_mfcc_wr(kws_mfcc_i16_kernel, s, p, t, d_wav, B, d_out, rl);
+    }
 #endif
     return launch_mfcc_t(mfcc_tail6(p) ? kws_mfcc_i16_tile_kernel : kws_mfcc_i16_any_kernel, s, p, t, d_wav, B, d_out, rl);
 }
 hipError_t launch_mfcc(hipStream_t s, const FrontendParams& p, const FrontendTables& t, const float* d_wav, int B, float* d_out,
-                       const RefineList& rl) {
+                       const RefineList& rl, bool) {
     return launch_mfcc_t(mfcc_tail6(p) ? kws_mfcc_f32_kernel : kws_mfcc_f32_any_kernel, s, p, t, d_wav, B, d_out, rl);
 }
 hipError_t launch_mfcc(hipStream_t s, const FrontendParams& p, const FrontendTables& t, const AugmentArgs& a, int B, float* d_out,
-                       const RefineList& rl) {
+                       const RefineList& rl, bool) {
     if (!mfcc_wave_resident_ok(p)) return hipErrorInvalidValue;
     return launch_mfcc_wr(kws_mfcc_augment_i16_kernel, s, p, t, a, B, d_out, rl);
 }
diff --git a/keyword-spotting_amd/csrc/kws_mfcc_dev.h b/keyword-spotting_amd/csrc/kws_mfcc_dev.h
--- a/keyword-spotting_amd/csrc/kws_mfcc_dev.h
+++ b/keyword-spotting_amd/csrc/kws_mfcc_dev.h
@@ -180,12 +180,14 @@
 struct PairLevel {
     float pow_a, pow_b;
 };
-__device__ __forceinline__ PairLevel equalise_levels(cf (&v)[8]) {
+template <int NV = 8>
+__device__ __forceinline__ PairLevel equalise_levels(cf (&v)[8], float* e_out = nullptr) {
     cf e2 = {0.f, 0.f};
 #pragma unroll
-    for (int i = 0; i < 8; ++i) asm("v_pk_fma_f32 %0, %1, %1, %0" : "+v"(e2) : "v"(v[i]));
+    for (int i = 0; i < NV; ++i) asm("v_pk_fma_f32 %0, %1, %1, %0" : "+v"(e2) : "v"(v[i]));
     float ea = e2.x, eb = e2.y;
     wave_sum2(ea, eb);
+    if (e_out) e_out[0] = ea, e_out[1] = eb;
     auto shift_of = [](float e) -> int {
         const int ex = (int)((__builtin_bit_cast(uint32_t, e) >> 23) & 0xffu);
         if (ex == 0 || ex == 255) return 0;
@@ -196,7 +198,7 @@
     if (sa == sb) return {1.0f, 1.0f};
     const cf down = {__builtin_bit_cast(float, (uint32_t)(127 - sa) << 23), __builtin_bit_cast(float, (uint32_t)(127 - sb) << 23)};
 #pragma unroll
-    for (int i = 0; i < 8; ++i) v[i] = v[i] * down;
+    for (int i = 0; i < NV; ++i) v[i] = v[i] * down;
     return {__builtin_bit_cast(float, (uint32_t)(127 + 2 * sa) << 23), __builtin_bit_cast(float, (uint32_t)(127 + 2 * sb) << 23)};
 }
 
@@ -284,6 +286,58 @@
     wave_lds_order();
 }
 
+template <bool PEAK>
+__device__ __forceinline__ void split_power_packed(const cf (&v)[8], cf* zbuf, float2* pbuf, int lane, bool nza, bool nzb,
+                                                   const int (&pslot)[4], const PairLevel& lv, float& ea, float& eb,
+                                                   float& pk_a, float& pk_b) {
+    const int k1 = lane >> 3, q = lane & 7;
+#pragma unroll
+    for (int d = 0; d < 8; ++d) zbuf[zswz(k1 + 8 * q + 64 * d)] = v[d];
+    wave_lds_order();
+    cf z[4], w[4];
+#pragma unroll
+    for (int j = 0; j < 4; ++j) {
+        const int k = lane + 64 * j;
+        z[j] = zbuf[zswz(k)];
+        w[j] = zbuf[zswz((NFFT - k) & (NFFT - 1))];
+    }
+    wave_lds_order();
+    constexpr float scale = 1.0f / (4.0f * NFFT);
+    const cf sc = {nza ? scale * lv.pow_a : 0.f, nzb ? scale * lv.pow_b : 0.f};
+    cf pw[4], e = {0.f, 0.f};
+#pragma unroll
+    for (int j = 0; j < 4; ++j) {
+        const cf s = z[j] + w[j], d = z[j] - w[j];
+        const cf t = d * d;
+        cf r;
+        asm("v_pk_fma_f32 %0, %1, %1, %2 op_sel:[0,0,1] op_sel_hi:[1,1,0]" : "=v"(r) : "v"(s), "v"(t));
+        pw[j] = r * sc;
+    }
+    if constexpr (PEAK) {
+        asm("v_max3_f32 %0, %1, %2, %3" : "=v"(pk_a) : "v"(pw[0].x), "v"(pw[1].x), "v"(pw[2].x));
+        asm("v_max3_f32 %0, %1, %2, %3" : "=v"(pk_b) : "v"(pw[0].y), "v"(pw[1].y), "v"(pw[2].y));
+        asm("v_max_f32 %0, %0, %1" : "+v"(pk_a) : "v"(pw[3].x));
+        asm("v_max_f32 %0, %0, %1" : "+v"(pk_b) : "v"(pw[3].y));
+    }
+#pragma unroll
+    for (int j = 0; j < 4; ++j) {
+        pbuf[pslot[j]] = make_float2(pw[j].x, pw[j].y);
+        e = e + pw[j];
+    }
+    if (lane == 0) {
+        const cf t = v[4] * 2.f;
+        const cf p = (t * t) * sc;
+        e = e + p;
+        if constexpr (PEAK) {
+            asm("v_max_f32 %0, %0, %1" : "+v"(pk_a) : "v"(p.x));
+            asm("v_max_f32 %0, %0, %1" : "+v"(pk_b) : "v"(p.y));
+        }
+    }
+    ea = e.x;
+    eb = e.y;
+    wave_lds_order();
+}
+
 constexpr float PSF_EPS = 2.220446049250313e-16f;
 
 __device__ __forceinline__ float to_unit(int16_t s) { return (float)s * (1.0f / 32768.0f); }
@@ -328,7 +382,9 @@
         reinterpret_cast<float4*>(scr)[i * 64 + lane] = make_float4(0.f, 0.f, 0.f, 0.f);
 }
 
-__device__ __forceinline__ void segment_suffix_sums(float& a, float& b, float& c, float& d, const MelLane& m) {
+template <bool M4_FROM_TABLE = false>
+__device__ __forceinline__ void segment_suffix_sums(float& a, float& b, float& c, float& d, const MelLane& m,
+                                                    const int* seg_tab = nullptr, int lane = 0) {
     asm("s_nop 1\n\t"
         "v_fmac_f32_dpp %0, %0, %4 row_shl:1 row_mask:0xf bank_mask:0xf bound_ctrl:1\n\t"
         "v_fmac_f32_dpp %1, %1, %4 row_shl:1 row_mask:0xf bank_mask:0xf bound_ctrl:1\n\t"
@@ -340,14 +396,16 @@
         "v_fmac_f32_dpp %3, %3, %5 row_shl:2 row_mask:0xf bank_mask:0xf bound_ctrl:1"
         : "+v"(a), "+v"(b), "+v"(c), "+v"(d)
         : "v"(m.m1), "v"(m.m2));
-    if (m.deep)
+    if (m.deep) {
+        const float m4 = M4_FROM_TABLE ? ((seg_tab[lane] & 4) ? 1.f : 0.f) : m.m4;
         asm("s_nop 1\n\t"
             "v_fmac_f32_dpp %0, %0, %4 row_shl:4 row_mask:0xf bank_mask:0xf bound_ctrl:1\n\t"
             "v_fmac_f32_dpp %1, %1, %4 row_shl:4 row_mask:0xf bank_mask:0xf bound_ctrl:1\n\t"
             "v_fmac_f32_dpp %2, %2, %4 row_shl:4 row_mask:0xf bank_mask:0xf bound_ctrl:1\n\t"
             "v_fmac_f32_dpp %3, %3, %4 row_shl:4 row_mask:0xf bank_mask:0xf bound_ctrl:1"
             : "+v"(a), "+v"(b), "+v"(c), "+v"(d)
-            : "v"(m.m4));
+            : "v"(m4));
+    }
 }
 
 __device__ __forceinline__ void wave_sum2_max2(float& a, float& b, float& ma, float& mb) {
@@ -411,28 +469,60 @@
     over_b = (__ballot(b < lim_b) >> 63) & 1ull;
 }
 
+struct GeomAny {
+    static constexpr bool REF = false;
+    static constexpr bool FLAGS = true;
+    static __device__ __forceinline__ int frame_len(const FrontendParams& p) { return p.frame_len; }
+    static __device__ __forceinline__ int frame_step(const FrontendParams& p) { return p.frame_step; }
+    static __device__ __forceinline__ int nfilt(const FrontendParams& p) { return p.nfilt; }
+    static __device__ __forceinline__ int numcep(const FrontendParams& p) { return p.numcep; }
+    static __device__ __forceinline__ bool append_energy(const FrontendParams& p) { return p.append_energy != 0; }
+    static __device__ __forceinline__ bool refine(const FrontendParams& p) { return p.refine_span > 0.f; }
+};
+constexpr int REF_FRAME_LEN = 400, REF_FRAME_STEP = 160, REF_NFILT = 26, REF_NUMCEP = 10;
+template <bool REFINE>
+struct GeomRef {
+    static constexpr bool REF = true;
+    static constexpr bool FLAGS = REFINE;
+    static __device__ __forceinline__ constexpr int frame_len(const FrontendParams&) { return REF_FRAME_LEN; }
+    static __device__ __forceinline__ constexpr int frame_step(const FrontendParams&) { return REF_FRAME_STEP; }
+    static __device__ __forceinline__ constexpr int nfilt(const FrontendParams&) { return REF_NFILT; }
+    static __device__ __forceinline__ constexpr int numcep(const FrontendParams&) { return REF_NUMCEP; }
+    static __device__ __forceinline__ constexpr bool append_energy(const FrontendParams&) { return true; }
+    static __device__ __forceinline__ constexpr bool refine(const FrontendParams&) { return REFINE; }
+};
+
+template <class G = GeomAny>
 __device__ __forceinline__ uint32_t mfcc_pair(cf (&v)[8], bool nza, bool nzb, bool has_b, const FrontendParams& p,
                                           const PairScratch& sc, const cf (&t1)[8], const MelLane& ml, int lane,
                                           float* __restrict__ out_a, float* __restrict__ out_b,
-                                          float* lds_out_a = nullptr) {
+                                          float* lds_out_a = nullptr, const int* seg_tab = nullptr) {
     cf* xbuf = sc.xbuf;
     float2* pbuf = sc.pbuf;
     float* lbuf = sc.lbuf;
     const float* dctb = sc.dctb;
     const cf* tw2 = sc.tw2;
     const uint32_t gth = ml.gth;
-    const int nfp = sc.nfp;
-    const PairLevel lv = equalise_levels(v);
+    const int nfp = G::REF ? ((REF_NFILT + 3) & ~3) : sc.nfp;
+    const int nfilt = G::nfilt(p);
+    [[maybe_unused]] const int numcep = G::numcep(p);
+    float e_pair[2];
+    const PairLevel lv = G::REF ? equalise_levels<(REF_FRAME_LEN + 63) / 64>(v, e_pair) : equalise_levels(v);
+    if constexpr (G::REF) nza = e_pair[0] != 0.f, nzb = e_pair[1] != 0.f;
 #if !defined(KWS_X_MFCC_STOP) || KWS_X_MFCC_STOP >= 1
     fft512(v, xbuf, t1, tw2, lane);
 #endif
 #if defined(KWS_X_MFCC_STOP) && KWS_X_MFCC_STOP <= 1
-    if (lane < p.numcep) out_a[lane] = v[0].x + v[1].y + v[2].x + v[3].y + v[4].x + v[5].y + v[6].x + v[7].y + lv.pow_a;
+    if (lane < numcep) out_a[lane] = v[0].x + v[1].y + v[2].x + v[3].y + v[4].x + v[5].y + v[6].x + v[7].y + lv.pow_a;
     return 0u;
 #endif
 
     float ea, eb, pka = 0.f, pkb = 0.f;
-    if (p.refine_span > 0.f) {
+    if constexpr (G::REF) {
+        split_power_packed<G::FLAGS>(v, xbuf, pbuf, lane, nza, nzb, ml.pslot, lv, ea, eb, pka, pkb);
+        if constexpr (G::FLAGS) wave_sum2_max2(ea, eb, pka, pkb);
+        else wave_sum2(ea, eb);
+    } else if (G::refine(p)) {
         split_power(v, xbuf, pbuf, lane, 1, nza, nzb, ml.pslot, -1, lv, ea, eb, &pka, &pkb);
         wave_sum2_max2(ea, eb, pka, pkb);
     } else {
@@ -440,12 +530,26 @@
         wave_sum2(ea, eb);
     }
 #if defined(KWS_X_MFCC_STOP) && KWS_X_MFCC_STOP == 2
-    if (lane < p.numcep) out_a[lane] = ea + eb + pbuf[lane].x;
+    if (lane < numcep) out_a[lane] = ea + eb + pbuf[lane].x;
     return 0u;
 #endif
 
     float ra = 0.f, fa_ = 0.f, rb = 0.f, fb_ = 0.f;
-    {
+    if constexpr (G::REF) {
+        const float4* pc = reinterpret_cast<const float4*>(pbuf + lane * MEL_STRIDE);
+        cf accr = {0.f, 0.f}, accf = {0.f, 0.f};
+#pragma unroll
+        for (int h = 0; h < MEL_CHUNK / 2; ++h) {
+            const float4 pw = pc[h];
+            const cf p0 = {pw.x, pw.y}, p1 = {pw.z, pw.w};
+            const cf rw2 = {ml.rw[2 * h], ml.rw[2 * h + 1]}, fw2 = {ml.fw[2 * h], ml.fw[2 * h + 1]};
+            asm("v_pk_fma_f32 %0, %1, %2, %0 op_sel_hi:[0,1,1]" : "+v"(accr) : "v"(rw2), "v"(p0));
+            asm("v_pk_fma_f32 %0, %1, %2, %0 op_sel_hi:[0,1,1]" : "+v"(accf) : "v"(fw2), "v"(p0));
+            asm("v_pk_fma_f32 %0, %1, %2, %0 op_sel:[1,0,0]" : "+v"(accr) : "v"(rw2), "v"(p1));
+            asm("v_pk_fma_f32 %0, %1, %2, %0 op_sel:[1,0,0]" : "+v"(accf) : "v"(fw2), "v"(p1));
+        }
+        ra = accr.x, rb = accr.y, fa_ = accf.x, fb_ = accf.y;
+    } else {
         const float4* pc = reinterpret_cast<const float4*>(pbuf + lane * MEL_STRIDE);
 #pragma unroll
         for (int h = 0; h < MEL_CHUNK / 2; ++h) {
@@ -460,7 +564,8 @@
             fb_ = fmaf(ml.fw[2 * h + 1], pw.w, fb_);
         }
     }
-    segment_suffix_sums(ra, fa_, rb, fb_, ml);
+    if constexpr (G::REF) segment_suffix_sums<true>(ra, fa_, rb, fb_, ml, seg_tab, lane);
+    else segment_suffix_sums(ra, fa_, rb, fb_, ml);
     float ma, mb;
     uint32_t flags = 0u;
     {
@@ -469,22 +574,35 @@
         const float grb = __builtin_bit_cast(float, __builtin_amdgcn_ds_bpermute(4 * r0, __builtin_bit_cast(int, rb)));
         const float gfa = __builtin_bit_cast(float, __builtin_amdgcn_ds_bpermute(4 * q0, __builtin_bit_cast(int, fa_)));
         const float gfb = __builtin_bit_cast(float, __builtin_amdgcn_ds_bpermute(4 * q0, __builtin_bit_cast(int, fb_)));
+#ifdef KWS_X_MFCC_NO_BOOKKEEPING
+        const float sa = G::REF ? gra + gfa : (nr ? gra : 0.f) + (nq ? gfa : 0.f);
+        const float sb = G::REF ? grb + gfb : (nr ? grb : 0.f) + (nq ? gfb : 0.f);
+#else
         const float sa = (nr ? gra : 0.f) + (nq ? gfa : 0.f);
         const float sb = (nr ? grb : 0.f) + (nq ? gfb : 0.f);
-        if (p.nfilt <= 32) {
+#endif
+        if (nfilt <= 32) {
             const auto sw = __builtin_amdgcn_permlane32_swap(__builtin_bit_cast(unsigned, sa), __builtin_bit_cast(unsigned, sb), false, false);
             const float s = __builtin_bit_cast(float, (unsigned)sw[0]);
+#ifdef KWS_X_MFCC_NO_BOOKKEEPING
+            const float l = logf(G::REF ? s : (s == 0.f ? PSF_EPS : s));
+#else
             const float l = logf(s == 0.f ? PSF_EPS : s);
+#endif
             ma = __builtin_bit_cast(float, __builtin_amdgcn_readlane(__builtin_bit_cast(int, l), 0));
             mb = __builtin_bit_cast(float, __builtin_amdgcn_readlane(__builtin_bit_cast(int, l), 32));
 #if defined(KWS_X_MFCC_STOP) && KWS_X_MFCC_STOP == 3
-            if (lane < p.numcep) out_a[lane] = l + ea + eb;
+            if (lane < numcep) out_a[lane] = l + ea + eb;
             return 0u;
 #endif
             const int f = lane >> 5, j = lane & 31;
-            const float cv = j < p.nfilt ? l - (f ? mb : ma) : 0.f;
+#ifdef KWS_X_MFCC_NO_BOOKKEEPING
+            const float cv = G::REF ? l - (f ? mb : ma) : (j < nfilt ? l - (f ? mb : ma) : 0.f);
+#else
+            const float cv = j < nfilt ? l - (f ? mb : ma) : 0.f;
+#endif
             lbuf[64 * f + j] = cv;
-            if (p.refine_span > 0.f) {
+            if (G::refine(p)) {
                 const float lim = 0.6931471806f * __builtin_amdgcn_logf(f ? pkb : pka) - (f ? mb : ma) - p.refine_span;
                 const unsigned long long over = peak_over<false>(cv, lim);
                 flags = (uint32_t)((over >> 31) & 1u) | ((uint32_t)((over >> 63) & 1u) << 1);
@@ -493,10 +611,10 @@
             const float la = logf(sa == 0.f ? PSF_EPS : sa), lb = logf(sb == 0.f ? PSF_EPS : sb);
             ma = __builtin_bit_cast(float, __builtin_amdgcn_readfirstlane(__builtin_bit_cast(int, la)));
             mb = __builtin_bit_cast(float, __builtin_amdgcn_readfirstlane(__builtin_bit_cast(int, lb)));
-            const float cva = lane < p.nfilt ? la - ma : 0.f, cvb = lane < p.nfilt ? lb - mb : 0.f;
+            const float cva = lane < nfilt ? la - ma : 0.f, cvb = lane < nfilt ? lb - mb : 0.f;
             lbuf[lane] = cva;
             lbuf[64 + lane] = cvb;
-            if (p.refine_span > 0.f) {
+            if (G::refine(p)) {
                 bool oa, ob;
                 peak_over2(cva, cvb, 0.6931471806f * __builtin_amdgcn_logf(pka) - ma - p.refine_span, 0.6931471806f * __builtin_amdgcn_logf(pkb) - mb - p.refine_span, oa, ob);
                 flags = (uint32_t)oa | ((uint32_t)ob << 1);
@@ -505,7 +623,39 @@
     }
     wave_lds_order();
 
-    {
+    if constexpr (G::REF) {
+        const int f = lane >> 5, i = lane & 31;
+        const int row = i < REF_NUMCEP ? i : REF_NUMCEP - 1;
+        const float4* L4 = reinterpret_cast<const float4*>(lbuf + 64 * f);
+        const float4* D4 = reinterpret_cast<const float4*>(dctb + row * nfp);
+        float acc = 0.f;
+        if (i < REF_NUMCEP)
+#pragma unroll
+        for (int j0 = 0; j0 < 7; j0 += 4) {
+            float4 d[4], l[4];
+#pragma unroll
+            for (int j = 0; j < 4; ++j)
+                if (j0 + j < 7) d[j] = D4[j0 + j], l[j] = L4[j0 + j];
+#pragma unroll
+            for (int j = 0; j < 4; ++j)
+                if (j0 + j < 7) {
+                    acc = fmaf(d[j].x, l[j].x, acc);
+                    acc = fmaf(d[j].y, l[j].y, acc);
+                    acc = fmaf(d[j].z, l[j].z, acc);
+                    acc = fmaf(d[j].w, l[j].w, acc);
+                }
+            __builtin_amdgcn_sched_barrier(0);
+        }
+        const float e = f ? eb : ea;
+#ifdef KWS_X_MFCC_NO_BOOKKEEPING
+        acc += logf(e);
+        if (i < REF_NUMCEP && (f == 0 || has_b)) out_a[REF_NUMCEP * f + i] = acc;
+#else
+        const float le = logf(e == 0.f ? PSF_EPS : e);
+        acc = i == 0 ? le : acc;
+        if (i < REF_NUMCEP && (f == 0 || has_b)) out_a[(unsigned)(REF_NUMCEP * f + i)] = acc;
+#endif
+    } else {
         const int f = lane >> 5, i = lane & 31;
         if (i < p.numcep && (f == 0 || has_b)) {
             const float4* L4 = reinterpret_cast<const float4*>(lbuf + 64 * f);
diff --git a/keyword-spotting_amd/kws/_native/__init__.py b/keyword-spotting_amd/kws/_native/__init__.py
--- a/keyword-spotting_amd/kws/_native/__init__.py
+++ b/keyword-spotting_amd/kws/_native/__init__.py
@@ -16,6 +16,7 @@
 KWS_K_DSCNN_LOAD_STATS, KWS_K_DSCNN_LOAD_PACK, KWS_K_DSCNN_LOAD_FILL = 7, 8, 9
 KWS_K_RESAMPLE = 10
 FE_REFINE_SPAN_DEFAULT = 10.2
+FE_ROUTE_AUTO, FE_ROUTE_GENERIC = 0, 1
 FE_F32, FE_F64 = 0, 1
 ACT_FLOATS_PER_CLIP = 64 * (141 + 141 + 245 + 357) + 64 + 64 * 477
 PW_F32 = 1
@@ -36,6 +37,7 @@
     "kws_set_frontend": (C.c_int, [_c_ctx] + [C.c_int] * 7 + [C.c_float, C.c_int]),
     "kws_set_frontend_math": (C.c_int, [_c_ctx, C.c_int]),
     "kws_frontend_math": (C.c_int, [_c_ctx]),
+    "kws_set_frontend_route": (C.c_int, [_c_ctx, C.c_int]),
     "kws_set_frontend_refine": (C.c_int, [_c_ctx, C.c_float]),
     "kws_frontend_stats": (C.c_int, [_c_ctx, C.POINTER(C.c_uint64), C.POINTER(C.c_uint64), C.POINTER(C.c_int)]),
     "kws_spec_f32": (C.c_int, [_c_ctx, _f32p, C.c_int, C.c_int, C.c_int, C.c_int, _f32p]),
@@ -220,6 +222,9 @@
     def set_frontend_math(self, math: int):
         self._check(self._lib.kws_set_frontend_math(self._h, int(math)), AudioProcessingError)
 
+    def set_frontend_route(self, route: int = FE_ROUTE_AUTO):
+        self._check(self._lib.kws_set_frontend_route(self._h, int(route)), AudioProcessingError)
+
     def frontend_math(self) -> int:
         return int(self._lib.kws_frontend_math(self._h))
 
```

Result: faster. 7.198 million (median of 6 runs) (+2.3%).
